# WeeFav/Visual-Odometry-GPU

Measured on AMD Instinct MI355X. Metric: ORB detect+describe frames/sec (1241x376, 8 lvls), higher is better.
Workload: dtype u8; 1 GPU; KITTI-shaped 1241x376 u8, 8 levels s=1.2, 1000 features, FAST-9 t=20, NMS 3x3, Harris top-N, blur5 all levels, BRIEF-256; batch=1024 frames/step/GPU resident in HBM (stream A); distinct_resident_batches=2, fast_early_exit=True, pyramid_blur_fused=True, pyramid_top_rows_first=True, pipelined_batches=True

## Files before the change

visual-odometry-gpu_amd/csrc/orbx_adapt.h:

```cpp
#pragma once
#include <cstdio>
#include <cstdlib>

#include "orbx_plan.h"

struct OrbxAdapt {
  int top_mode = 2;
  bool top_on = true;
  int top_single_batches = 0;
  uint32_t feedback_seen[2] = {0, 0};
  uint32_t need_cur[ORBX_MAX_LEVELS] = {}, need_prev[ORBX_MAX_LEVELS] = {};
  int tile_h_pref[ORBX_MAX_LEVELS] = {};
  int need_batches = 0, need_window = 2, retiles = 0, learn_w = 0, learn_h = 0;
  bool prefs_applied = false;
  uint32_t fill_cur[ORBX_MAX_LEVELS][ORBX_FILL_BUCKETS] = {}, fill_prev[ORBX_MAX_LEVELS][ORBX_FILL_BUCKETS] = {};
  int cut_pref[ORBX_MAX_LEVELS] = {}, cut_force[ORBX_MAX_LEVELS] = {};
  bool first_split = true, split_trace = false;
  uint32_t fill_last[ORBX_MAX_LEVELS][ORBX_FILL_BUCKETS] = {};
  int early_rows[ORBX_MAX_LEVELS] = {};
  bool early_band = true;
};

struct OrbxAdaptGeom {
  const OrbxPlan& plan;
  const OrbxBandMap& bm;
  int nms_radius, fast_impl, top_rows;
};

namespace orbx_adapt {

using namespace orbx_geom;

inline int fast_unit_rows_max(int fast_impl, int nms_radius) {
  return fast_impl == 4 ? ORBX_FAST_UNIT_ROWS_MAX : orbx_fast3_tile_h(nms_radius);
}

inline void first_split_fields(OrbxAdapt& a, const char* e) {
  e = e ? std::strchr(e, ':') : nullptr;
  while (e && *e == ':') {
    e++;
    if (!std::strncmp(e, "equal", 5)) {
      a.first_split = false;
    } else if (!std::strncmp(e, "trace", 5)) {
      a.split_trace = true;
    } else if (!std::strncmp(e, "late", 4)) {
      a.early_band = false;
    } else {
      for (int l = 0; l < ORBX_MAX_LEVELS; l++) {
        char* end = nullptr;
        const long v = std::strtol(e, &end, 10);
        if (end == e) break;
        a.cut_force[l] = (int)std::min<long>(std::max<long>(v, 0), 0xffff);
        e = end;
        if (*e != ',') break;
        e++;
      }
    }
    e = std::strchr(e, ':');
  }
}

inline void new_frame_size(OrbxAdapt& a, int w, int h, uint32_t* feedback) {
  a.learn_w = w;
  a.learn_h = h;
  for (int l = 0; l < ORBX_MAX_LEVELS; l++) a.need_cur[l] = a.need_prev[l] = 0, a.tile_h_pref[l] = a.cut_pref[l] = 0;
  std::memset(a.fill_cur, 0, sizeof(a.fill_cur));
  std::memset(a.fill_prev, 0, sizeof(a.fill_prev));
  std::memset(a.fill_last, 0, sizeof(a.fill_last));
  for (int i = 2; i < ORBX_FEEDBACK_WORDS; i++) feedback[i] = 0;
  a.need_batches = 0;
  a.need_window = 2;
  a.retiles = 0;
}

inline bool top_rows_wanted(const OrbxAdapt& a, int top_rows) {
  if (top_rows <= 0 || a.top_mode == 0) return false;
  return a.top_mode == 1 || a.top_on;
}
inline void top_rows_update(OrbxAdapt& a, uint64_t both) {
  if (a.top_mode != 2) return;
  const uint32_t sk = (uint32_t)both, pr = (uint32_t)(both >> 32);
  const uint32_t dsk = sk - a.feedback_seen[0], dpr = pr - a.feedback_seen[1];
  if (dsk + dpr > 0) {
    a.feedback_seen[0] = sk;
    a.feedback_seen[1] = pr;
    const bool pays = 4ull * dsk >= (unsigned long long)(dsk + dpr);
    if (!pays && a.top_on) a.top_single_batches = 0;
    a.top_on = pays;
  }
  if (!a.top_on && ++a.top_single_batches >= 128) {
    a.top_on = true;
    a.top_single_batches = 0;
  }
}

inline bool adapt_tile_rows(OrbxAdapt& a, const OrbxAdaptGeom& g, const uint32_t* words, bool prefs_apply,
                            long long batch_serial, FILE* trace) {
  if (!prefs_apply) return false;
  const int top = g.top_rows, nl = g.plan.nlevels;
  bool any = false;
  for (int l = 0; l < nl; l++) {
    const uint32_t v = words[2 + l];
    if (v) {
      a.need_cur[l] = std::max(a.need_cur[l], std::min<uint32_t>(v, (uint32_t)g.plan.L[l].h));
      any = true;
      for (int b = 0; b < ORBX_FILL_BUCKETS; b++) {
        const uint32_t cnt = words[ORBX_FEEDBACK_HIST + l * ORBX_FILL_BUCKETS + b];
        a.fill_cur[l][b] += std::min<uint32_t>(cnt, 1u << 20);
      }
    }
  }
  if (!any || ++a.need_batches < a.need_window) return false;
  a.need_batches = 0;
  a.need_window = std::min(2 * a.need_window, 32);
  bool change = false, grow = false;
  int want[ORBX_MAX_LEVELS] = {};
  for (int l = 0; l < nl; l++) {
    const uint32_t need = std::max(a.need_cur[l], a.need_prev[l]);
    a.need_prev[l] = a.need_cur[l];
    a.need_cur[l] = 0;
    if (need == 0) {
      want[l] = a.tile_h_pref[l];
      continue;
    }
    const int rows = (int)need + std::max(4, (int)need / 10);
    const int dflt = orbx_fast3_tile_h(g.nms_radius), lh = g.plan.L[l].h;
    const int bal = (lh + (lh + dflt - 1) / dflt - 1) / ((lh + dflt - 1) / dflt);
    int hh = (rows + top - 1) / top;
    if (g.fast_impl == 4) {
      const int over = (hh + 2 * g.nms_radius) % 7;
      if ((over == 1 || over == 2) && top * (hh - over) >= (int)need + 3) hh -= over;
    }
    if (hh >= bal || lh <= top * hh) hh = 0;
    const int eff = hh ? hh : bal, cur = g.bm.tile_h[l], asked = a.tile_h_pref[l] ? a.tile_h_pref[l] : bal;
    want[l] = ((eff > cur && (int)need > top * cur) || eff + 2 < std::min(cur, asked)) ? hh : a.tile_h_pref[l];
    if (eff > cur && (int)need > top * cur) grow = true;
    else if (eff + 2 < std::min(cur, asked)) change = true;
  }
  const bool heights_change = grow || change;
  const bool split = a.first_split && top == 2 && g.fast_impl == 4;
  const int R = g.nms_radius;
  int cut_want[ORBX_MAX_LEVELS] = {};
  bool cut_change = false;
  for (int l = 0; l < nl; l++) {
    uint32_t hist[ORBX_FILL_BUCKETS];
    uint64_t total = 0;
    for (int b = 0; b < ORBX_FILL_BUCKETS; b++) {
      hist[b] = a.fill_cur[l][b] + a.fill_prev[l][b];
      a.fill_last[l][b] = hist[b];
      a.fill_prev[l][b] = a.fill_cur[l][b];
      a.fill_cur[l][b] = 0;
      total += hist[b];
    }
    if (!split || a.cut_force[l] > 0 || g.bm.tiles_y[l] < 2) continue;
    const int dflt = orbx_fast3_tile_h(R), lh = g.plan.L[l].h;
    const int bal = (lh + (lh + dflt - 1) / dflt - 1) / ((lh + dflt - 1) / dflt);
    const int th_after = heights_change ? (want[l] ? want[l] : bal) : g.bm.tile_h[l];
    const int depth = 2 * th_after;
    const int in_force = !heights_change && g.bm.first_h[l][0] > 0 ? g.bm.first_h[l][0] : 0;
    int cost_new = 0;
    const int cut_new = total && lh > depth ? choose_first_cut(hist, depth, R, ORBX_FAST_UNIT_ROWS_MAX, &cost_new) : 0;
    const int cost_now = first_pass_cost_milli(hist, depth, in_force ? in_force : depth / 2, R);
    if (!total || lh <= depth) cost_new = cost_now;
    const bool pays = cost_now - cost_new >= 1000, stopped = in_force && !cut_new && cost_now > cost_new;
    cut_want[l] = heights_change || pays || stopped ? cut_new : a.cut_pref[l];
    if (cut_want[l] != in_force && (pays || stopped)) cut_change = true;
    if (trace) {
      fprintf(trace, "orbx split: batch %lld level %d need %u depth %d cut %d -> %d (%d -> %d milli-groups) fill rows:",
              batch_serial, l, a.need_prev[l], depth, in_force, cut_want[l], cost_now, cost_new);
      for (int b = 0; b < ORBX_FILL_BUCKETS; b++)
        if (hist[b]) fprintf(trace, " %d:%u", ORBX_FILL_BUCKET_ROWS * (b + 1), hist[b]);
      fprintf(trace, "\n");
    }
  }
  if (!grow && !change && !cut_change) return false;
  if (!grow && a.retiles >= 4 && a.need_window < 32) return false;
  for (int l = 0; l < nl; l++) a.tile_h_pref[l] = want[l], a.cut_pref[l] = cut_want[l];
  a.retiles++;
  if (trace) fprintf(trace, "orbx split: batch %lld re-tile %d\n", batch_serial, a.retiles);
  return true;
}

inline void forget_tile_rows(OrbxAdapt& a) {
  for (int l = 0; l < ORBX_MAX_LEVELS; l++) a.tile_h_pref[l] = 0;
  a.prefs_applied = false;
}

inline bool first_pass_heights(const OrbxAdapt& a, const OrbxAdaptGeom& g, int (*first)[2]) {
  bool any = false;
  if (a.prefs_applied && a.first_split && g.top_rows == 2) {
    for (int l = 0; l < g.plan.nlevels; l++) {
      int h0 = a.cut_force[l] > 0 ? a.cut_force[l] : a.cut_pref[l];
      if (h0 <= 0 || g.bm.tiles_y[l] < 2) continue;
      const int depth = 2 * g.bm.tile_h[l], umax = fast_unit_rows_max(g.fast_impl, g.nms_radius);
      if (a.cut_force[l] > 0)
        h0 = std::max(std::max(1, depth - umax), std::min(h0, std::min(umax, std::min(depth, g.plan.L[l].h) - 1)));
      first[l][0] = h0;
      first[l][1] = depth - h0;
      any = true;
    }
  }
  return any;
}

inline void choose_early_bands(OrbxAdapt& a, const OrbxAdaptGeom& g, FILE* trace) {
  const int top = g.top_rows;
  for (int l = 0; l < ORBX_MAX_LEVELS; l++) a.early_rows[l] = 0;
  for (int l = 0; l < g.plan.nlevels; l++) {
    const int late = pyrblur_first_pass_rows(g.plan, g.bm, l, top);
    const int P = a.early_band ? pyrblur_early_rows(g.plan, g.bm, l, top, g.nms_radius) : late;
    const bool forced = a.cut_force[l] > 0;
    const bool pays = P < late && (forced ? late - P >= ORBX_PYRBLUR_EARLY_MIN_ROWS
                                          : early_band_pays(a.fill_last[l], g.bm.first_h[l][0], late - P,
                                                            pyrblur_row_cost(l, g.plan.L[l].win8)));
    a.early_rows[l] = pays ? P : late;
    if (trace && g.bm.first_h[l][0] > 0)
      fprintf(trace, "orbx early band: level %d cut %d first pass ended at %d, now ends at %d, band %d rows: %s\n", l,
              g.bm.first_h[l][0], late, a.early_rows[l], late - P,
              pays ? (forced ? "split (forced cut)" : "split") : !a.early_band ? "late" : "kept");
  }
}

}
```

visual-odometry-gpu_amd/csrc/orbx_api.cpp:

```cpp
#include <algorithm>
#include <array>
#include <cmath>
#include <cstdlib>
#include <cstring>
#include <new>

#include "orbx_host.h"

using namespace orbx_host;
using namespace orbx_tables;

namespace {
thread_local std::string g_create_error;
}

namespace orbx_host {

int fail(orbx_ctx* c, int status, const std::string& msg) {
  if (c)
    c->err = msg;
  else
    g_create_error = msg;
  return status;
}

int ensure(orbx_ctx* c, DevBuf& b, size_t bytes) {
  if (b.bytes >= bytes && b.p) return ORBX_OK;
  if (b.p) {
    HIPCHK(c, hipStreamSynchronize(c->stream));
    for (const Lane& L : c->lanes)
      if (L.stream && L.stream != c->stream) HIPCHK(c, hipStreamSynchronize(L.stream));
    if (c->last_stream && c->last_stream != c->stream) HIPCHK(c, hipStreamSynchronize(c->last_stream));
    HIPCHK(c, hipFree(b.p));
    b.p = nullptr;
    b.bytes = 0;
  }
  bytes = align_up_sz(std::max<size_t>(bytes, 256), 256);
  HIPCHK(c, hipMalloc(&b.p, bytes));
  b.bytes = bytes;
  return ORBX_OK;
}

hipStream_t batch_stream(const orbx_ctx* c) { return c->last_stream ? c->last_stream : c->stream; }
const Lane& cur_lane(const orbx_ctx* c) { return c->lanes[c->lane]; }
const Block& last_block(const orbx_ctx* c) { return c->blocks[c->blk]; }
hipError_t lanes_sync(orbx_ctx* c) {
  for (const Lane& L : c->lanes)
    if (L.stream) {
      const hipError_t e = hipStreamSynchronize(L.stream);
      if (e != hipSuccess) return e;
    }
  return hipSuccess;
}

int check_image(orbx_ctx* c, const void* img, int w, int h, int stride) {
  if (!c) return ORBX_ERR_INVALID_ARG;
  if (!img) return fail(c, ORBX_ERR_INVALID_ARG, "image is NULL");
  if (w < 8 || h < 8 || w > c->p.max_width || h > c->p.max_height)
    return fail(c, ORBX_ERR_INVALID_ARG, "image size outside [8, max_width] x [8, max_height]");
  if (stride < w) return fail(c, ORBX_ERR_INVALID_ARG, "stride < width");
  return ORBX_OK;
}

bool finite_all(const double* v, int n) {
  for (int i = 0; i < n; i++)
    if (!std::isfinite(v[i])) return false;
  return true;
}

int gaussian_kernel(int K, float sigma, float* kernel) {
  if (K <= 0 || (K % 2) == 0 || !kernel) return ORBX_ERR_INVALID_ARG;
  if (sigma <= 0.0f) sigma = 0.3f * ((K - 1) * 0.5f) + 0.8f;
  const int half = K / 2;
  float sum = 0.0f;
  for (int y = -half; y <= half; ++y)
    for (int x = -half; x <= half; ++x) {
      const float value = std::exp(-(float)(x * x + y * y) / (2 * sigma * sigma));
      kernel[(y + half) * K + (x + half)] = value;
      sum += value;
    }
  for (int i = 0; i < K * K; ++i) kernel[i] /= sum;
  return ORBX_OK;
}

hipError_t launch_blur_auto(int impl, hipStream_t s, const OrbxPlan& P, const OrbxTileMap& tm1, const OrbxTileDesc* tiles2,
                            int ntiles2, int n, const uint8_t* src, uint8_t* dst, int first_level, int kind) {
  if (kind == ORBX_BLUR_SEP16 && impl == 3)
    return orbx_launch_blur4(s, tiles2, ntiles2, P.frame_bytes, n, src, dst, first_level);
  if (kind == ORBX_BLUR_SEP16 && impl != 1)
    return orbx_launch_blur3(s, tiles2, ntiles2, P.frame_bytes, n, src, dst, first_level);
  return orbx_launch_blur(s, P, tm1, n, src, dst, first_level, kind);
}

int SideWork::wait(orbx_ctx* c) {
  if (ev) HIPCHK(c, hipEventSynchronize(ev));
  return ORBX_OK;
}

int SideWork::enter(orbx_ctx* c, hipStream_t s) {
  if (!ev) HIPCHK(c, hipEventCreateWithFlags(&ev, hipEventDisableTiming));
  if (stream != s) {
    const int st = wait(c);
    if (st != ORBX_OK) return st;
  }
  stream = s;
  return ORBX_OK;
}

int SideWork::after(orbx_ctx* c, const SideWork& producer, hipStream_t s) {
  if (producer.ev && producer.stream != s) HIPCHK(c, hipStreamWaitEvent(s, producer.ev, 0));
  return ORBX_OK;
}

int SideWork::grow(orbx_ctx* c, DevBuf& b, size_t bytes) {
  if (b.p && b.bytes >= bytes) return ORBX_OK;
  const int st = wait(c);
  if (st != ORBX_OK) return st;
  bytes = align_up_sz(std::max<size_t>(bytes, 256), 256);
  void* p = nullptr;
  HIPCHK(c, hipMalloc(&p, bytes));
  if (b.p) (void)hipFree(b.p);
  b.p = p;
  b.bytes = bytes;
  return ORBX_OK;
}

int PinnedUpload::send(orbx_ctx* c, void* d_dst, const void* src, size_t n, hipStream_t s) {
  if (!ev) HIPCHK(c, hipEventCreateWithFlags(&ev, hipEventDisableTiming));
  HIPCHK(c, hipEventSynchronize(ev));
  if (bytes < n) {
    if (host) (void)hipHostFree(host);
    host = nullptr;
    bytes = 0;
    HIPCHK(c, hipHostMalloc(&host, align_up_sz(n, 4096), hipHostMallocDefault));
    bytes = align_up_sz(n, 4096);
  }
  std::memcpy(host, src, n);
  HIPCHK(c, hipMemcpyAsync(d_dst, host, n, hipMemcpyHostToDevice, s));
  HIPCHK(c, hipEventRecord(ev, s));
  return ORBX_OK;
}

int set_workspace_limit(orbx_ctx* c, SideWork& side, std::initializer_list<DevBuf*> ws, size_t* limit, size_t bytes,
                        size_t dflt) {
  const int st = side.wait(c);
  if (st != ORBX_OK) return st;
  for (DevBuf* b : ws)
    if (b->p) {
      HIPCHK(c, hipFree(b->p));
      *b = DevBuf{};
    }
  *limit = bytes ? bytes : dflt;
  return ORBX_OK;
}

int stage_tracks(orbx_ctx* c, SideWork& side, DevBuf& stage, const float* tracks_xy, const int32_t* seen, int n_slots,
                 int window_len, const float** d_tracks, const int32_t** d_seen) {
  int st = side.enter(c, c->stream);
  if (st != ORBX_OK) return st;
  const SideWork::Mark mark{side, c->stream};
  const size_t tb = sizeof(float) * 2 * (size_t)n_slots * window_len, sb = sizeof(int32_t) * (size_t)n_slots;
  const size_t o_seen = align_up_sz(tb, 256);
  if ((st = side.grow(c, stage, o_seen + sb)) != ORBX_OK) return st;
  uint8_t* d = (uint8_t*)stage.p;
  HIPCHK(c, hipMemcpyAsync(d, tracks_xy, tb, hipMemcpyHostToDevice, c->stream));
  HIPCHK(c, hipMemcpyAsync(d + o_seen, seen, sb, hipMemcpyHostToDevice, c->stream));
  *d_tracks = (const float*)d;
  *d_seen = (const int32_t*)(d + o_seen);
  return ORBX_OK;
}

int check_device_frames(orbx_ctx* c, const void* d_frames, int n, int n_min, int n_max, int w, int h, int row_stride,
                        size_t frame_stride, const FramesWhat& what) {
  if (!d_frames) return fail(c, ORBX_ERR_INVALID_ARG, what.null_msg);
  if (n < n_min || n > n_max) return fail(c, ORBX_ERR_INVALID_ARG, what.range_msg);
  if (w < 8 || h < 8 || w > c->p.max_width || h > c->p.max_height)
    return fail(c, ORBX_ERR_INVALID_ARG, "image size outside [8, max_width] x [8, max_height]");
  if (row_stride < w) return fail(c, ORBX_ERR_INVALID_ARG, "row_stride < width");
  if (frame_stride < (size_t)row_stride * (size_t)(h - 1) + (size_t)w)
    return fail(c, ORBX_ERR_INVALID_ARG, "frame_stride smaller than a frame");
  if ((unsigned long long)row_stride * (unsigned long long)(h - 1) + (unsigned long long)w > 0x7fffffffull)
    return fail(c, ORBX_ERR_INVALID_ARG, "row_stride * (height - 1) + width exceeds 2^31 - 1");
  return ORBX_OK;
}

}

namespace {

int env_int(const char* name, int dflt) {
  const char* e = getenv(name);
  return e ? atoi(e) : dflt;
}

int pyr_group_env() {
  static const int v = env_int("ORBX_PYR_GROUP", 32);
  return v;
}

int top_rows_env() {
  static const int v = std::max(env_int("ORBX_TOP_ROWS", 2), 0);
  return v;
}

int fast_impl_env() { return env_int("ORBX_FAST_IMPL", 4) == 3 ? 3 : 4; }

int blur_impl_env() {
  const int v = env_int("ORBX_BLUR_IMPL", 2);
  return v >= 1 && v <= 3 ? v : 2;
}

int fast_early_env() {
  static const int v = env_int("ORBX_FAST_EARLY", 1);
  return v;
}

int fuse_env() {
  static const int v = env_int("ORBX_FUSE", 1);
  return v;
}

int graph_env() {
  static const int v = env_int("ORBX_GRAPH", 1);
  return v;
}

int select_spread_env() {
  static const int v = env_int("ORBX_SELECT_SPREAD", -1);
  return v;
}

bool fused_pyrblur(const orbx_ctx* c) {
  return fuse_env() && c->fuse && c->p.blur_levels == ORBX_BLUR_ALL && c->p.blur_kind == ORBX_BLUR_SEP16;
}
bool fast_early_on(const orbx_ctx* c) { return fast_early_env() && c->fast_early; }
bool blur_enabled(const orbx_ctx* c) { return c->p.blur_levels != ORBX_BLUR_NONE; }
const uint8_t* final_pyr(const orbx_ctx* c) { return blur_enabled(c) ? cur_lane(c).d_pyr_blur : cur_lane(c).d_pyr; }

int slots_per_frame(const OrbxPlan& P) { return P.out_cap > 0 ? P.out_cap : 1; }

int validate_params(const orbx_params& p, std::string* why) {
  auto bad = [&](const char* m) {
    *why = m;
    return (int)ORBX_ERR_INVALID_ARG;
  };
  if (p.nfeatures < 0) return bad("nfeatures < 0");
  if (!(p.scale_factor > 1.0f) || !(p.scale_factor <= 4.0f)) return bad("scale_factor must be in (1, 4]");
  if (p.nlevels < 1 || p.nlevels > ORBX_MAX_LEVELS) return bad("nlevels must be in [1, 16]");
  if (p.n < 1 || p.n > 16) return bad("n must be in [1, 16]");
  if (p.threshold < 0 || p.threshold > 255) return bad("threshold must be in [0, 255]");
  if (p.nms_window < 0 || p.nms_window / 2 > 3) return bad("nms_window must be in [0, 7]");
  if (p.patch_size < 1 || p.patch_size / 2 > 20) return bad("patch_size must be in [1, 41]");
  if (p.harris_window < 1 || (p.harris_window % 2) == 0 || p.harris_window > 15)
    return bad("harris_window must be odd, in [1, 15]");
  if (p.select_mode != ORBX_SELECT_HARRIS && p.select_mode != ORBX_SELECT_ROWMAJOR) return bad("select_mode");
  if (p.blur_levels < 0 || p.blur_levels > 2) return bad("blur_levels");
  if (p.blur_kind < 0 || p.blur_kind > 1) return bad("blur_kind");
  if (p.max_width < 8 || p.max_height < 8 || p.max_width > 16384 || p.max_height > 16384)
    return bad("max_width/max_height must be in [8, 16384]");
  if (p.max_batch < 1 || p.max_batch > 65535) return bad("max_batch must be in [1, 65535]");
  return ORBX_OK;
}

struct PoolRef {
  void** p;
  size_t bytes;
  bool zero;
};
std::array<PoolRef, 11> lane_pools(const orbx_ctx* c, Lane& L) {
  const OrbxPlan& M = c->plan_max;
  const size_t B = (size_t)c->p.max_batch, nc = B * (size_t)std::max(M.cand_total, 1);
  const size_t frames = B * (size_t)M.frame_bytes, levels = B * ORBX_MAX_LEVELS * sizeof(int32_t);
  return {{
      {(void**)&L.d_pyr, frames, false},
      {(void**)&L.d_pyr_blur, c->p.blur_levels != ORBX_BLUR_NONE ? frames : 0, true},
      {(void**)&L.d_mask, B * (size_t)M.mask_words * 8, true},
      {(void**)&L.d_row_stat, B * ORBX_FAST_STAT_WORDS * 8, false},
      {(void**)&L.d_cand, nc * sizeof(orbx_keypoint), false},
      {(void**)&L.d_cand_count, levels, false},
      {(void**)&L.d_cand_total, levels, false},
      {(void**)&L.d_resp, nc * sizeof(float), false},
      {(void**)&L.d_lcand, nc * sizeof(uint32_t), false},
      {(void**)&L.d_lresp, nc * sizeof(float), false},
      {(void**)&L.d_lcount, levels, false},
  }};
}
hipError_t alloc_lane_pools(orbx_ctx* c, Lane& L) {
  for (const PoolRef& r : lane_pools(c, L)) {
    if (r.bytes == 0) continue;
    hipError_t e = hipMalloc(r.p, r.bytes + 256);
    if (e == hipSuccess && r.zero) e = hipMemset(*r.p, 0, r.bytes);
    if (e != hipSuccess) return e;
  }
  return hipSuccess;
}
void free_lane(orbx_ctx* c, Lane& L) {
  for (const PoolRef& r : lane_pools(c, L)) {
    if (*r.p) (void)hipFree(*r.p);
    *r.p = nullptr;
  }
  if (L.stream != c->stream) {
    if (L.stream) (void)hipStreamDestroy(L.stream);
    L.stream = nullptr;
  }
  L.pool_stream = nullptr;
}

bool tile_prefs_apply(const orbx_ctx* c) {
  return c->adapt.top_mode == 2 && top_rows_env() > 0 && fast_early_on(c) && fused_pyrblur(c);
}
OrbxAdaptGeom adapt_geom(const orbx_ctx* c) {
  return OrbxAdaptGeom{c->plan, c->bm_fast, c->p.nms_window / 2, c->fast_impl, top_rows_env()};
}
FILE* adapt_trace(const orbx_ctx* c) { return c->adapt.split_trace ? stderr : nullptr; }

int set_plan(orbx_ctx* c, int w, int h) {
  if (w == c->plan_w && h == c->plan_h) return ORBX_OK;
  if (w < 8 || h < 8 || w > c->p.max_width || h > c->p.max_height)
    return fail(c, ORBX_ERR_INVALID_ARG, "frame size outside [8, max_width] x [8, max_height]");
  OrbxPlan plan;
  std::string why;
  int st = plan_with_taps(c->p, w, h, c->fast_impl, &plan, &c->h_taps, &why);
  if (st != ORBX_OK) return fail(c, st, why);
  if (c->h_taps.size() > c->table_cap.taps) return fail(c, ORBX_ERR_UNSUPPORTED, "resize table exceeds pool");
  c->plan_w = c->plan_h = 0;
  OrbxPlanTables& T = c->scratch;
  const OrbxTableSwitches sw{c->fast_impl, c->blur_impl, top_rows_env(), pyr_group_env() > 0, tile_prefs_apply(c)};
  st = build_tile_tables(plan, c->p.nms_window / 2, sw, c->table_cap, c->adapt, adapt_trace(c), &T, &why);
  if (st != ORBX_OK) return fail(c, st, why);
  HIPCHK(c, hipStreamSynchronize(batch_stream(c)));
  HIPCHK(c, lanes_sync(c));
  HIPCHK(c, hipMemcpy(c->d_taps, c->h_taps.data(), c->h_taps.size() * sizeof(OrbxResizeTap),
                      hipMemcpyHostToDevice));
  for (const Lane& L : c->lanes)
    if (L.d_pyr_blur)
      HIPCHK(c, hipMemsetAsync(L.d_pyr_blur, 0, (size_t)c->p.max_batch * (size_t)c->plan_max.frame_bytes, c->stream));
  HIPCHK(c, hipStreamSynchronize(c->stream));
  for (int i = 0; i < kTileTables; i++) {
    const std::vector<OrbxTileDesc>& t = T.tiles[i];
    if (!t.empty())
      HIPCHK(c, hipMemcpy(c->tiles[i].d, t.data(), t.size() * sizeof(OrbxTileDesc), hipMemcpyHostToDevice));
    c->tiles[i].count = (int)t.size();
  }
  c->plan = plan;
  c->tm_blur = T.tm_blur;
  c->bm_fast = T.bm_fast;
  c->top_levels = T.top_levels;
  c->plan_serial++;
  c->plan_w = w;
  c->plan_h = h;
  return ORBX_OK;
}

hipError_t launch_pyramid_auto(orbx_ctx* c, hipStream_t s, int n, const uint8_t* d_in, int in_stride,
                               size_t in_frame_stride) {
  return orbx_launch_pyramid2(s, c->tiles[T_PYR2].d, c->tiles[T_PYR2].count, c->plan.frame_bytes, c->plan.w0, c->plan.h0, n,
                              d_in, in_stride, in_frame_stride, c->d_taps, cur_lane(c).d_pyr);
}

hipError_t launch_fast_tiles(orbx_ctx* c, hipStream_t s, int first, int count, int n, OrbxFastParams fp,
                             unsigned long long* stat, int chunk_scale = 1) {
  const OrbxTileDesc* tiles = c->tiles[T_FAST].d + first;
  unsigned long long* mask = cur_lane(c).d_mask;
  if (c->fast_impl == 4)
    return orbx_launch_fast4(s, tiles, count, n, final_pyr(c), c->plan.frame_bytes, c->plan.mask_words, fp, mask, stat);
  return orbx_launch_fast_nms(s, tiles, count, n, final_pyr(c), c->plan.frame_bytes, c->plan.mask_words, fp, mask, nullptr,
                              stat, chunk_scale);
}

hipError_t launch_fast_whole(orbx_ctx* c, hipStream_t s, int n, OrbxFastParams fp, bool stats_zeroed = false) {
  unsigned long long* stat = fast_early_on(c) ? cur_lane(c).d_row_stat : nullptr;
  if (stat && !stats_zeroed) {
    hipError_t e = hipMemsetAsync(stat, 0, (size_t)n * ORBX_FAST_STAT_WORDS * 8, s);
    if (e != hipSuccess) return e;
  }
  return launch_fast_tiles(c, s, 0, c->tiles[T_FAST].count, n, fp, stat);
}

int enqueue_batch(orbx_ctx* c, Block& B, const uint8_t* d_frames, int n, int row_stride, size_t frame_stride, hipStream_t s) {
  const OrbxPlan& P = c->plan;
  const Lane& L = cur_lane(c);
  const TileTable &whole = c->tiles[T_PYRBLUR], &shortb = c->tiles[T_PYRBLUR_SMALL], &top = c->tiles[T_PYRBLUR_TOP],
                  &rest = c->tiles[T_PYRBLUR_REST];
  const int tm = c->timing;
  TimingSet& ts = c->evr[c->ev_calls % ORBX_EVENT_SETS];
  auto mark = [&](int slot, bool roofline_edge) -> hipError_t {
    if (tm == 1 || (tm == 2 && roofline_edge)) return hipEventRecord(ts.ev[slot], s);
    return hipSuccess;
  };
  const bool fused = fused_pyrblur(c);
  const bool small = (long long)n * whole.count < 4096;
  const bool two_pass = fused && !small && fast_early_on(c) && top_rows_wanted(c->adapt, top_rows_env()) && rest.count > 0 &&
                        c->bm_fast.nbands > top_rows_env();
  if (!two_pass) HIPCHK(c, hipMemsetAsync(L.d_row_stat, 0, (size_t)n * ORBX_FAST_STAT_WORDS * 8, s));
  HIPCHK(c, mark(0, false));
  OrbxFastParams fp{c->p.threshold, c->p.n, c->p.nms_window / 2};
  if (fused) {
    HIPCHK(c, mark(1, true));
    if (!two_pass) {
      const TileTable& T = small ? shortb : whole;
      HIPCHK(c, orbx_launch_pyrblur(s, T.d, T.count, P.frame_bytes, P.w0, P.h0, n, d_frames, row_stride, frame_stride,
                                    c->d_taps, L.d_pyr_blur, small ? 0 : pyr_group_env()));
    } else {
      const int first_tiles = c->bm_fast.band_begin[top_rows_env()];
      HIPCHK(c, orbx_launch_pyrblur(s, top.d, top.count, P.frame_bytes, P.w0, P.h0, n, d_frames, row_stride, frame_stride,
                                    c->d_taps, L.d_pyr_blur, pyr_group_env(), nullptr, c->d_feedback, nullptr,
                                    L.d_row_stat));
      HIPCHK(c, mark(ORBX_NUM_STAGE_TIMES + 1, true));
      HIPCHK(c, launch_fast_tiles(c, s, 0, first_tiles, n, fp, L.d_row_stat));
      HIPCHK(c, mark(ORBX_NUM_STAGE_TIMES + 2, true));
      HIPCHK(c, orbx_launch_pyrblur(s, rest.d, rest.count, P.frame_bytes, P.w0, P.h0, n, d_frames, row_stride,
                                    frame_stride, c->d_taps, L.d_pyr_blur, pyr_group_env(), L.d_row_stat, c->d_feedback,
                                    &c->top_levels));
      HIPCHK(c, mark(2, true));
      HIPCHK(c, launch_fast_tiles(c, s, first_tiles, c->tiles[T_FAST].count - first_tiles, n, fp, L.d_row_stat, 4));
    }
  } else {
    HIPCHK(c, launch_pyramid_auto(c, s, n, d_frames, row_stride, frame_stride));
    HIPCHK(c, mark(1, true));
    if (blur_enabled(c))
      HIPCHK(c, launch_blur_auto(c->blur_impl, s, P, c->tm_blur, c->tiles[T_BLUR].d, c->tiles[T_BLUR].count, n, L.d_pyr,
                                 L.d_pyr_blur, c->p.blur_levels == ORBX_BLUR_UPPER ? 1 : 0, c->p.blur_kind));
  }
  if (!two_pass) {
    HIPCHK(c, mark(2, true));
    HIPCHK(c, launch_fast_whole(c, s, n, fp, true));
  }
  ts.split = two_pass;
  c->last_two_pass = two_pass;
  HIPCHK(c, mark(3, true));
  HIPCHK(c, mark(4, false));
  HIPCHK(c, mark(5, false));
  const OutLayout& o = B.layout;
  HIPCHK(c, orbx_launch_level_select_auto(s, P, n, c->p.select_mode, select_spread_env(), L.d_mask, final_pyr(c), c->d_gauss,
                                          c->p.harris_window, c->p.harris_k, L.d_lcand, L.d_lcount, L.d_lresp,
                                          L.d_cand, L.d_resp, L.d_cand_count, two_pass ? c->d_feedback + 2 : nullptr));
  HIPCHK(c, mark(6, false));
  if (P.out_cap <= 0)
    HIPCHK(c, hipMemsetAsync(B.d + o.counts, 0, sizeof(int32_t) * (size_t)n, s));
  OrbxHostRecord hr{};
  if (c->host_results && P.out_cap > 0 && B.h_dev)
    hr = OrbxHostRecord{(int32_t*)(B.h_dev + o.counts), (uint32_t*)(B.h_dev + o.kp16), (float*)(B.h_dev + o.angle),
                        (orbx_descriptor*)(B.h_dev + o.desc)};
  HIPCHK(c, orbx_launch_describe(s, P, n, final_pyr(c), c->p.patch_size, L.d_cand_count, L.d_cand, L.d_resp,
                                 (int32_t*)(B.d + o.counts), (orbx_keypoint*)(B.d + o.lkp),
                                 (float*)(B.d + o.resp), (int32_t*)(B.d + o.level),
                                 (orbx_keypoint*)(B.d + o.kp), (uint32_t*)(B.d + o.kp16),
                                 (float*)(B.d + o.angle),
                                 (orbx_descriptor*)(B.d + o.desc), two_pass ? c->d_feedback : nullptr,
                                 two_pass ? const_cast<uint32_t*>(c->h_feedback) : nullptr, &hr));
  HIPCHK(c, mark(7, false));
  return ORBX_OK;
}

void drop_graph(orbx_ctx* c, int i) {
  if (c->g_exec[i]) (void)hipGraphExecDestroy(c->g_exec[i]);
  c->g_exec[i] = nullptr;
}

int run_batch(orbx_ctx* c, const uint8_t* d_frames, int n, int w, int h, int row_stride, size_t frame_stride,
              hipStream_t s, bool may_pipeline = false) {
  OrbxAdapt& a = c->adapt;
  if (w != a.learn_w || h != a.learn_h) {
    new_frame_size(a, w, h, const_cast<uint32_t*>(c->h_feedback));
  } else if (w == c->plan_w && h == c->plan_h) {
    bool any_pref = false;
    for (int l = 0; l < ORBX_MAX_LEVELS; l++) any_pref |= a.tile_h_pref[l] != 0 || a.cut_pref[l] != 0 || a.cut_force[l] != 0;
    const bool apply = tile_prefs_apply(c);
    const int used = ORBX_FEEDBACK_HIST + c->plan.nlevels * ORBX_FILL_BUCKETS;
    uint32_t words[ORBX_FEEDBACK_WORDS];
    for (int i = 0; apply && i < used; i++) words[i] = c->h_feedback[i];
    if (adapt_tile_rows(a, adapt_geom(c), words, apply, c->batch_serial, adapt_trace(c)) || (any_pref && apply != a.prefs_applied))
      c->plan_w = 0;
  }
  const bool lanes = may_pipeline && c->pipelined && s == c->stream && w == c->plan_w && h == c->plan_h;
  c->lane = lanes ? c->next_lane : 0;
  Lane& L = c->lanes[c->lane];
  if (lanes) {
    s = L.stream;
  } else {
    if (c->lanes[1].stream) HIPCHK(c, lanes_sync(c));
    if (c->last_stream && c->last_stream != s) HIPCHK(c, hipStreamSynchronize(c->last_stream));
  }
  int st = set_plan(c, w, h);
  if (st != ORBX_OK) return st;
  top_rows_update(a, *reinterpret_cast<const volatile uint64_t*>(c->h_feedback));
  const int blk = (c->blk + 1) % orbx_ctx::kBlocks;
  Block& B = c->blocks[blk];
  if (B.copy_pending) HIPCHK(c, hipStreamWaitEvent(s, B.ev_copied, 0));
  if (L.pool_stream && L.pool_stream != s) HIPCHK(c, hipStreamWaitEvent(s, L.ev_pool, 0));
  if (B.stream && B.stream != s) HIPCHK(c, hipStreamWaitEvent(s, B.ev_done, 0));
  B.n = 0;
  B.copy_pending = false;
  B.copy_compact = false;
  B.cap = slots_per_frame(c->plan);
  B.layout = OutLayout(n, B.cap);
  const int tm = c->timing;
  if (graph_env() && tm == 0) {
    const OrbxGraphKey key{d_frames, frame_stride, n, w, h, row_stride, (fast_early_on(c) ? 1 : 0) | (fused_pyrblur(c) ? 2 : 0) | (top_rows_wanted(a, top_rows_env()) ? 4 : 0) | (lanes ? 8 : 0) | (c->lane << 4) | (c->host_results ? 64 : 0),
                           c->plan_serial, blk};
    int gi = -1;
    for (int i = 0; i < orbx_ctx::kGraphs; i++)
      if (c->g_exec[i] && key == c->g_key[i]) gi = i;
    if (gi < 0) {
      gi = c->g_next;
      c->g_next = (c->g_next + 1) % orbx_ctx::kGraphs;
      drop_graph(c, gi);
      hipGraph_t g = nullptr;
      const hipError_t be = hipStreamBeginCapture(s, hipStreamCaptureModeThreadLocal);
      if (be != hipSuccess) return fail(c, ORBX_ERR_HIP, std::string("hipStreamBeginCapture: ") + hipGetErrorString(be));
      st = enqueue_batch(c, B, d_frames, n, row_stride, frame_stride, s);
      const hipError_t ee = hipStreamEndCapture(s, &g);
      if (st != ORBX_OK) {
        if (g) (void)hipGraphDestroy(g);
        return st;
      }
      if (ee != hipSuccess) return fail(c, ORBX_ERR_HIP, std::string("hipStreamEndCapture: ") + hipGetErrorString(ee));
      const hipError_t ie = hipGraphInstantiate(&c->g_exec[gi], g, nullptr, nullptr, 0);
      (void)hipGraphDestroy(g);
      if (ie != hipSuccess) {
        c->g_exec[gi] = nullptr;
        return fail(c, ORBX_ERR_HIP, std::string("hipGraphInstantiate: ") + hipGetErrorString(ie));
      }
      c->g_key[gi] = key;
    }
    const hipError_t le = hipGraphLaunch(c->g_exec[gi], s);
    if (le != hipSuccess) return fail(c, ORBX_ERR_HIP, std::string("hipGraphLaunch: ") + hipGetErrorString(le));
  } else {
    if ((st = enqueue_batch(c, B, d_frames, n, row_stride, frame_stride, s)) != ORBX_OK) return st;
  }
  c->blk = blk;
  if (lanes) c->next_lane ^= 1;
  c->batch_serial++;
  c->last_stream = s;
  B.n = n;
  B.host_written = c->host_results && c->plan.out_cap > 0;
  HIPCHK(c, hipEventRecord(B.ev_done, s));
  if (B.host_written) {
    HIPCHK(c, hipEventRecord(B.ev_copied, s));
    B.copy_pending = true;
    B.copy_compact = true;
  }
  HIPCHK(c, hipEventRecord(L.ev_pool, s));
  L.pool_stream = s;
  B.stream = s;
  if (tm != 0) {
    c->evr[c->ev_calls % ORBX_EVENT_SETS].mode = tm;
    c->ev_calls++;
  }
  return ORBX_OK;
}


}

extern "C" {

int orbx_params_default_gpu(orbx_params* p) {
  if (!p) return ORBX_ERR_INVALID_ARG;
  std::memset(p, 0, sizeof(*p));
  p->nfeatures = 500;
  p->scale_factor = 1.2f;
  p->nlevels = 8;
  p->threshold = 20;
  p->n = 9;
  p->nms_window = 3;
  p->patch_size = 31;
  p->harris_window = 7;
  p->harris_k = 0.04f;
  p->select_mode = ORBX_SELECT_HARRIS;
  p->blur_levels = ORBX_BLUR_NONE;
  p->blur_kind = ORBX_BLUR_SEP16;
  p->max_width = 1920;
  p->max_height = 1080;
  p->max_batch = 1;
  p->device = -1;
  return ORBX_OK;
}

int orbx_params_default_cpu(orbx_params* p) {
  int st = orbx_params_default_gpu(p);
  if (st != ORBX_OK) return st;
  p->nfeatures = 3000;
  p->threshold = 50;
  p->n = 9;
  p->nms_window = 3;
  p->patch_size = 9;
  p->nlevels = 1;
  p->select_mode = ORBX_SELECT_ROWMAJOR;
  return ORBX_OK;
}

const char* orbx_status_string(int status) {
  switch (status) {
    case ORBX_OK:
      return "ok";
    case ORBX_ERR_INVALID_ARG:
      return "invalid argument";
    case ORBX_ERR_CAPACITY:
      return "output capacity exceeded";
    case ORBX_ERR_HIP:
      return "HIP runtime error";
    case ORBX_ERR_NO_DEVICE:
      return "no usable gfx950 device";
    case ORBX_ERR_UNSUPPORTED:
      return "unsupported parameter combination";
    default:
      return "unknown status";
  }
}

const char* orbx_version(void) { return "liborbx 0.1.0 gfx950"; }

const char* orbx_last_error_string(const orbx_ctx* ctx) { return ctx ? ctx->err.c_str() : g_create_error.c_str(); }

void orbx_destroy(orbx_ctx* c) {
  DeviceGuard _dg(c);
  if (!c) return;
  if (c->stream) (void)hipStreamSynchronize(c->stream);
  if (c->lanes[1].stream) (void)hipStreamSynchronize(c->lanes[1].stream);
  for (int i = 0; i < orbx_ctx::kGraphs; i++) drop_graph(c, i);
  for (Lane& L : c->lanes) {
    free_lane(c, L);
    if (L.ev_pool) (void)hipEventDestroy(L.ev_pool);
  }
  for (TileTable& T : c->tiles)
    if (T.d) (void)hipFree(T.d);
  void* bufs[] = {c->d_in, c->d_taps, c->d_gauss, c->d_feedback};
  for (void* b : bufs)
    if (b) (void)hipFree(b);
  if (c->h_feedback) (void)hipHostFree(const_cast<uint32_t*>(c->h_feedback));
  for (Block& B : c->blocks) {
    if (B.h) (void)hipHostFree(B.h);
    if (B.d) (void)hipFree(B.d);
    if (B.ev_done) (void)hipEventDestroy(B.ev_done);
    if (B.ev_copied) (void)hipEventDestroy(B.ev_copied);
  }
  if (c->cstream) {
    (void)hipStreamSynchronize(c->cstream);
    (void)hipStreamDestroy(c->cstream);
  }
  c->carry.release();
  c->reloc.release();
  c->pnp.release();
  c->st.release();
  c->wp.release();
  c->tp.release();
  c->lm.release();
  c->lkw.release();
  c->gf.release();
  c->s.release();
  c->m.release();
  c->lk.release();
  c->pose.release();
  c->scale.release();
  c->ba.release();
  for (auto& e : c->ev)
    if (e) (void)hipEventDestroy(e);
  for (TimingSet& set : c->evr)
    for (auto& e : set.ev)
      if (e) (void)hipEventDestroy(e);
  if (c->stream) (void)hipStreamDestroy(c->stream);
  delete c;
}

int orbx_create(const orbx_params* p, orbx_ctx** out) {
  if (!p || !out) return fail(nullptr, ORBX_ERR_INVALID_ARG, "params/out is NULL");
  *out = nullptr;
  std::string why;
  int st = validate_params(*p, &why);
  if (st != ORBX_OK) return fail(nullptr, st, why);

  int ndev = 0;
  if (hipGetDeviceCount(&ndev) != hipSuccess || ndev <= 0)
    return fail(nullptr, ORBX_ERR_NO_DEVICE, "hipGetDeviceCount found no device (liborbx has no CPU fallback)");
  int dev = p->device;
  if (dev < 0) {
    if (hipGetDevice(&dev) != hipSuccess) dev = 0;
  }
  if (dev >= ndev) return fail(nullptr, ORBX_ERR_INVALID_ARG, "device ordinal out of range");
  DeviceGuard dg(dev);
  {
    int cur = -1;
    if (hipGetDevice(&cur) != hipSuccess || cur != dev) return fail(nullptr, ORBX_ERR_NO_DEVICE, "hipSetDevice failed");
  }
  hipDeviceProp_t prop;
  if (hipGetDeviceProperties(&prop, dev) != hipSuccess)
    return fail(nullptr, ORBX_ERR_NO_DEVICE, "hipGetDeviceProperties failed");
  if (std::strncmp(prop.gcnArchName, "gfx950", 6) != 0)
    return fail(nullptr, ORBX_ERR_NO_DEVICE,
                std::string("device is ") + prop.gcnArchName + ", liborbx is built for gfx950 only");

  orbx_ctx* c = new (std::nothrow) orbx_ctx();
  if (!c) return fail(nullptr, ORBX_ERR_HIP, "out of host memory");
  c->p = *p;
  c->device = dev;

  c->fast_impl = fast_impl_env();
  c->blur_impl = blur_impl_env();
  first_split_fields(c->adapt, getenv("ORBX_TOP_ROWS"));
  st = build_plan(c->p, p->max_width, p->max_height, &c->plan_max, &why, c->fast_impl);
  if (st != ORBX_OK) {
    delete c;
    return fail(nullptr, st, why);
  }
  const OrbxPlan& M = c->plan_max;
  const size_t B = (size_t)p->max_batch;

#define CREATE_CHK(expr)                                                                     \
  do {                                                                                       \
    hipError_t _e = (expr);                                                                  \
    if (_e != hipSuccess) {                                                                  \
      std::string m = std::string(#expr) + ": " + hipGetErrorString(_e);                     \
      orbx_destroy(c);                                                                       \
      return fail(nullptr, ORBX_ERR_HIP, m);                                                 \
    }                                                                                        \
  } while (0)

  CREATE_CHK(hipStreamCreateWithFlags(&c->stream, hipStreamNonBlocking));
  c->lanes[0].stream = c->stream;
  for (auto& e : c->ev) CREATE_CHK(hipEventCreate(&e));
  for (TimingSet& set : c->evr)
    for (auto& e : set.ev) CREATE_CHK(hipEventCreate(&e));
  CREATE_CHK(hipMalloc((void**)&c->d_in, B * (size_t)p->max_width * p->max_height + 256));
  CREATE_CHK(alloc_lane_pools(c, c->lanes[0]));
  CREATE_CHK(hipMalloc((void**)&c->d_feedback, ORBX_FEEDBACK_WORDS * 4));
  CREATE_CHK(hipMemset(c->d_feedback, 0, ORBX_FEEDBACK_WORDS * 4));
  CREATE_CHK(hipHostMalloc((void**)&c->h_feedback, ORBX_FEEDBACK_WORDS * 4, hipHostMallocDefault));
  for (int i = 0; i < ORBX_FEEDBACK_WORDS; i++) c->h_feedback[i] = 0;
  OrbxTableCapacity tcap{};
  if ((st = table_capacity(*p, M, c->fast_impl, c->blur_impl, &tcap, &why)) != ORBX_OK) {
    orbx_destroy(c);
    return fail(nullptr, st, why);
  }
  c->table_cap = tcap;
  for (int i = 0; i < kTileTables; i++)
    CREATE_CHK(hipMalloc((void**)&c->tiles[i].d, std::max<size_t>(tile_table_capacity(tcap, i), 1) * sizeof(OrbxTileDesc)));
  CREATE_CHK(hipMalloc((void**)&c->d_taps, tcap.taps * sizeof(OrbxResizeTap)));
  {
    const int K = p->harris_window;
    std::vector<float> g((size_t)K * K);
    gaussian_kernel(K, -1.0f, g.data());
    CREATE_CHK(hipMalloc((void**)&c->d_gauss, g.size() * sizeof(float)));
    CREATE_CHK(hipMemcpy(c->d_gauss, g.data(), g.size() * sizeof(float), hipMemcpyHostToDevice));
  }
  {
    const OutLayout o((int)B, slots_per_frame(M));
    {
      int least = 0, greatest = 0;
      CREATE_CHK(hipDeviceGetStreamPriorityRange(&least, &greatest));
      CREATE_CHK(hipStreamCreateWithPriority(&c->cstream, hipStreamNonBlocking, greatest));
    }
    for (Block& blk : c->blocks) {
      CREATE_CHK(hipMalloc((void**)&blk.d, o.total));
      CREATE_CHK(hipHostMalloc((void**)&blk.h, o.total, hipHostMallocDefault));
      CREATE_CHK(hipHostGetDevicePointer((void**)&blk.h_dev, blk.h, 0));
      CREATE_CHK(hipEventCreateWithFlags(&blk.ev_done, hipEventDisableTiming));
      CREATE_CHK(hipEventCreateWithFlags(&blk.ev_copied, hipEventDisableTiming));
    }
    for (Lane& L : c->lanes) CREATE_CHK(hipEventCreateWithFlags(&L.ev_pool, hipEventDisableTiming));
  }
#undef CREATE_CHK
  *out = c;
  return ORBX_OK;
}

int orbx_get_plan(orbx_ctx* c, int width, int height, int32_t* level_w, int32_t* level_h, int32_t* quota,
                  int32_t* fast_cap, float* level_scale_out, int32_t* out_capacity) {
  DeviceGuard _dg(c);
  if (!c) return ORBX_ERR_INVALID_ARG;
  OrbxPlan plan;
  std::string why;
  int st = build_plan(c->p, width, height, &plan, &why, c->fast_impl);
  if (st != ORBX_OK) return fail(c, st, why);
  for (int l = 0; l < plan.nlevels; l++) {
    if (level_w) level_w[l] = plan.L[l].w;
    if (level_h) level_h[l] = plan.L[l].h;
    if (quota) quota[l] = plan.L[l].quota;
    if (fast_cap) fast_cap[l] = plan.L[l].cap;
    if (level_scale_out) level_scale_out[l] = plan.L[l].scale;
  }
  if (out_capacity) *out_capacity = plan.out_cap;
  return ORBX_OK;
}

int orbx_detect_and_compute_batch_device(orbx_ctx* c, const void* d_frames, int n, int width, int height,
                                         int row_stride, size_t frame_stride, void* stream) {
  DeviceGuard _dg(c);
  if (!c) return ORBX_ERR_INVALID_ARG;
  if (!d_frames) return fail(c, ORBX_ERR_INVALID_ARG, "d_frames is NULL");
  if (n < 1 || n > c->p.max_batch) return fail(c, ORBX_ERR_INVALID_ARG, "n outside [1, max_batch]");
  if (row_stride < width) return fail(c, ORBX_ERR_INVALID_ARG, "row_stride < width");
  if (frame_stride < (size_t)row_stride * (size_t)(height - 1) + (size_t)width)
    return fail(c, ORBX_ERR_INVALID_ARG, "frame_stride smaller than a frame");
  if ((unsigned long long)row_stride * (unsigned long long)(height - 1) + (unsigned long long)width > 0x7fffffffull)
    return fail(c, ORBX_ERR_INVALID_ARG, "row_stride * (height - 1) + width exceeds 2^31 - 1");
  return run_batch(c, (const uint8_t*)d_frames, n, width, height, row_stride, frame_stride, stream_of(c, stream), true);
}

int orbx_detect_and_compute_batch_host(orbx_ctx* c, const uint8_t* frames, int n, int width, int height,
                                       int row_stride, size_t frame_stride) {
  DeviceGuard _dg(c);
  if (!c) return ORBX_ERR_INVALID_ARG;
  if (n < 1 || n > c->p.max_batch) return fail(c, ORBX_ERR_INVALID_ARG, "n outside [1, max_batch]");
  int st = check_image(c, frames, width, height, row_stride);
  if (st != ORBX_OK) return st;
  if (n > 1 && frame_stride < (size_t)row_stride * (size_t)(height - 1) + (size_t)width)
    return fail(c, ORBX_ERR_INVALID_ARG, "frame_stride smaller than a frame");
  const size_t tight = (size_t)width * height;
  if (row_stride == width && (n == 1 || frame_stride == tight)) {
    HIPCHK(c, hipMemcpyAsync(c->d_in, frames, tight * n, hipMemcpyHostToDevice, c->stream));
  } else {
    for (int i = 0; i < n; i++)
      HIPCHK(c, hipMemcpy2DAsync(c->d_in + tight * i, width, frames + frame_stride * i, row_stride, width, height,
                                 hipMemcpyHostToDevice, c->stream));
  }
  return run_batch(c, c->d_in, n, width, height, width, tight, c->stream);
}

int orbx_wait(orbx_ctx* c) {
  DeviceGuard _dg(c);
  if (!c) return ORBX_ERR_INVALID_ARG;
  HIPCHK(c, hipStreamSynchronize(batch_stream(c)));
  HIPCHK(c, lanes_sync(c));
  return ORBX_OK;
}

int orbx_set_host_results(orbx_ctx* c, int enable) {
  DeviceGuard _dg(c);
  if (!c) return ORBX_ERR_INVALID_ARG;
  c->host_results = enable ? 1 : 0;
  return ORBX_OK;
}

int orbx_set_pipelined_batches(orbx_ctx* c, int enable) {
  DeviceGuard _dg(c);
  if (!c) return ORBX_ERR_INVALID_ARG;
  if (c->last_stream) HIPCHK(c, hipStreamSynchronize(c->last_stream));
  HIPCHK(c, lanes_sync(c));
  Lane& L = c->lanes[1];
  if (enable && !L.stream) {
    hipError_t e = alloc_lane_pools(c, L);
    if (e == hipSuccess) e = hipStreamCreateWithFlags(&L.stream, hipStreamNonBlocking);
    if (e != hipSuccess) {
      free_lane(c, L);
      c->pipelined = false;
      return fail(c, ORBX_ERR_HIP, std::string("second lane of the pipelined mode: ") + hipGetErrorString(e));
    }
  }
  c->pipelined = enable != 0;
  return ORBX_OK;
}

int orbx_debug_fill_pools(orbx_ctx* c, int byte) {
  DeviceGuard _dg(c);
  if (!c) return ORBX_ERR_INVALID_ARG;
  if (byte < 0 || byte > 255) return fail(c, ORBX_ERR_INVALID_ARG, "byte must be in [0, 255]");
  if (c->last_stream) HIPCHK(c, hipStreamSynchronize(c->last_stream));
  HIPCHK(c, hipStreamSynchronize(c->stream));
  HIPCHK(c, lanes_sync(c));
  for (Lane& L : c->lanes) {
    if (!L.d_mask) continue;
    for (const PoolRef& r : lane_pools(c, L))
      if (*r.p && *r.p != L.d_pyr_blur) HIPCHK(c, hipMemsetAsync(*r.p, byte, r.bytes, c->stream));
    if (L.d_pyr_blur && c->plan_w > 0)
      for (size_t f = 0; f < (size_t)c->p.max_batch; f++)
        for (int l = 0; l < c->plan.nlevels; l++) {
          const OrbxLevel& V = c->plan.L[l];
          HIPCHK(c, hipMemset2DAsync(L.d_pyr_blur + f * (size_t)c->plan.frame_bytes + (size_t)V.img_off, (size_t)V.pitch, byte,
                                     (size_t)V.w, (size_t)V.h, c->stream));
        }
  }
  HIPCHK(c, hipStreamSynchronize(c->stream));
  return ORBX_OK;
}

int orbx_debug_read_pyramid_level(orbx_ctx* c, int frame, int level, uint8_t* out, size_t out_bytes) {
  DeviceGuard _dg(c);
  if (!c || !out) return ORBX_ERR_INVALID_ARG;
  if (c->plan_w == 0 || !cur_lane(c).d_pyr_blur) return fail(c, ORBX_ERR_INVALID_ARG, "run a batch first");
  if (frame < 0 || frame >= c->p.max_batch || level < 0 || level >= c->plan.nlevels)
    return fail(c, ORBX_ERR_INVALID_ARG, "frame or level out of range");
  const OrbxLevel& V = c->plan.L[level];
  if (out_bytes < (size_t)V.w * (size_t)V.h) return fail(c, ORBX_ERR_INVALID_ARG, "out_bytes below level_w * level_h");
  if (c->last_stream) HIPCHK(c, hipStreamSynchronize(c->last_stream));
  HIPCHK(c, hipStreamSynchronize(c->stream));
  HIPCHK(c, lanes_sync(c));
  HIPCHK(c, hipMemcpy2D(out, (size_t)V.w, cur_lane(c).d_pyr_blur + (size_t)frame * (size_t)c->plan.frame_bytes + (size_t)V.img_off,
                        (size_t)V.pitch, (size_t)V.w, (size_t)V.h, hipMemcpyDeviceToHost));
  return ORBX_OK;
}

int orbx_set_fast_early_exit(orbx_ctx* c, int enable) {
  DeviceGuard _dg(c);
  if (!c) return ORBX_ERR_INVALID_ARG;
  c->fast_early = enable != 0;
  return ORBX_OK;
}

int orbx_set_fused_pyramid_blur(orbx_ctx* c, int enable) {
  DeviceGuard _dg(c);
  if (!c) return ORBX_ERR_INVALID_ARG;
  c->fuse = enable != 0;
  return ORBX_OK;
}

int orbx_set_top_rows_first(orbx_ctx* c, int mode) {
  DeviceGuard _dg(c);
  if (!c || mode < 0 || mode > 2) return ORBX_ERR_INVALID_ARG;
  c->adapt.top_mode = mode;
  c->adapt.top_on = true;
  c->adapt.top_single_batches = 0;
  return ORBX_OK;
}

int orbx_fast_tile_counts(orbx_ctx* c, long long* worked, long long* total) {
  DeviceGuard _dg(c);
  if (!c || !worked || !total) return ORBX_ERR_INVALID_ARG;
  if (c->plan_w == 0 || last_block(c).n < 1) return fail(c, ORBX_ERR_INVALID_ARG, "run a batch first");
  const int n = last_block(c).n;
  std::vector<unsigned long long> h((size_t)n * ORBX_FAST_STAT_WORDS);
  HIPCHK(c, hipStreamSynchronize(c->last_stream));
  HIPCHK(c, hipMemcpy(h.data(), cur_lane(c).d_row_stat, h.size() * 8, hipMemcpyDeviceToHost));
  long long w = 0;
  for (int f = 0; f < n; f++)
    for (int l = 0; l < c->plan.nlevels; l++)
      for (int b = 0; b < c->bm_fast.tiles_y[l]; b++)
        w += (long long)(h[(size_t)f * ORBX_FAST_STAT_WORDS + (size_t)l * ORBX_MAX_BANDS + b] >> 32);
  *total = (long long)c->bm_fast.band_begin[c->bm_fast.nbands] * n;
  *worked = fast_early_on(c) ? w : *total;
  return ORBX_OK;
}

int orbx_pyramid_pixel_counts(orbx_ctx* c, long long* produced, long long* total) {
  DeviceGuard _dg(c);
  if (!c || !produced || !total) return ORBX_ERR_INVALID_ARG;
  if (c->plan_w == 0 || last_block(c).n < 1) return fail(c, ORBX_ERR_INVALID_ARG, "run a batch first");
  const int n = last_block(c).n, top = top_rows_env();
  long long per_frame = 0;
  for (int l = 0; l < c->plan.nlevels; l++) per_frame += (long long)c->plan.L[l].w * c->plan.L[l].h;
  *total = per_frame * n;
  *produced = *total;
  if (!c->last_two_pass) return ORBX_OK;
  std::vector<unsigned long long> h((size_t)n * ORBX_FAST_STAT_WORDS);
  HIPCHK(c, hipStreamSynchronize(c->last_stream));
  HIPCHK(c, hipMemcpy(h.data(), cur_lane(c).d_row_stat, h.size() * 8, hipMemcpyDeviceToHost));
  long long done = 0;
  for (int f = 0; f < n; f++)
    for (int l = 0; l < c->plan.nlevels; l++) {
      const OrbxLevel& L = c->plan.L[l];
      const int first = pyrblur_first_pass_rows(c->plan, c->bm_fast, l, top);
      long long surv = 0, surv0 = 0;
      for (int b = 0; b < std::min(top, c->bm_fast.tiles_y[l]); b++) {
        surv += (long long)(uint32_t)h[(size_t)f * ORBX_FAST_STAT_WORDS + (size_t)l * ORBX_MAX_BANDS + b];
        if (b == 0) surv0 = surv;
      }
      const int early_l = c->adapt.early_rows[l], early = early_l > 0 && early_l < first ? early_l : first;
      const int band = surv0 >= L.cap ? 0 : first - early;
      done += (long long)L.w * (first < L.h && surv >= L.cap ? early + band : L.h);
    }
  *produced = done;
  return ORBX_OK;
}

int orbx_enable_stage_timing(orbx_ctx* c, int enable) {
  DeviceGuard _dg(c);
  if (!c) return ORBX_ERR_INVALID_ARG;
  c->timing = enable < 0 || enable > 2 ? 1 : enable;
  return ORBX_OK;
}

int orbx_stage_times_history(orbx_ctx* c, int back, float* ms) {
  DeviceGuard _dg(c);
  if (!c || !ms) return ORBX_ERR_INVALID_ARG;
  if (back < 0 || back >= ORBX_EVENT_SETS || back >= c->ev_calls)
    return fail(c, ORBX_ERR_INVALID_ARG, "no timed batched call that far back");
  const long long call = c->ev_calls - 1 - back;
  const TimingSet& ts = c->evr[call % ORBX_EVENT_SETS];
  const hipEvent_t* evs = ts.ev;
  const int mode = ts.mode;
  std::memset(ms, 0, sizeof(float) * ORBX_NUM_STAGE_TIMES);
  if (mode == 1) {
    for (int i = 0; i < ORBX_NUM_STAGE_TIMES - 1; i++) HIPCHK(c, hipEventElapsedTime(&ms[i], evs[i], evs[i + 1]));
    HIPCHK(c, hipEventElapsedTime(&ms[ORBX_NUM_STAGE_TIMES - 1], evs[0], evs[ORBX_NUM_STAGE_TIMES - 1]));
  } else {
    HIPCHK(c, hipEventElapsedTime(&ms[1], evs[1], evs[2]));
    HIPCHK(c, hipEventElapsedTime(&ms[2], evs[2], evs[3]));
  }
  if (ts.split) {
    float a = 0, b = 0, d = 0, e = 0;
    HIPCHK(c, hipEventElapsedTime(&a, evs[1], evs[ORBX_NUM_STAGE_TIMES + 1]));
    HIPCHK(c, hipEventElapsedTime(&b, evs[ORBX_NUM_STAGE_TIMES + 1], evs[ORBX_NUM_STAGE_TIMES + 2]));
    HIPCHK(c, hipEventElapsedTime(&d, evs[ORBX_NUM_STAGE_TIMES + 2], evs[2]));
    HIPCHK(c, hipEventElapsedTime(&e, evs[2], evs[3]));
    ms[1] = a + d;
    ms[2] = b + e;
  }
  return ORBX_OK;
}

int orbx_last_stage_times(orbx_ctx* c, float* ms) { return orbx_stage_times_history(c, 0, ms); }

int orbx_batch_results_device(orbx_ctx* c, orbx_batch_view* v) {
  DeviceGuard _dg(c);
  if (!c || !v) return ORBX_ERR_INVALID_ARG;
  const Block& B = last_block(c);
  if (B.n <= 0) return fail(c, ORBX_ERR_INVALID_ARG, "no batch has been run");
  const OutLayout& o = B.layout;
  v->counts = (const int32_t*)(B.d + o.counts);
  v->keypoints = (const orbx_keypoint*)(B.d + o.kp);
  v->keypoints16 = (const uint32_t*)(B.d + o.kp16);
  v->level_kps = (const orbx_keypoint*)(B.d + o.lkp);
  v->orientations = (const float*)(B.d + o.angle);
  v->responses = (const float*)(B.d + o.resp);
  v->levels = (const int32_t*)(B.d + o.level);
  v->descriptors = (const orbx_descriptor*)(B.d + o.desc);
  v->slot_capacity = B.cap;
  v->n = B.n;
  return ORBX_OK;
}

namespace {
int fetch_block(orbx_ctx* c, int b, int first, int n, int32_t* counts, orbx_keypoint* keypoints, float* orientations,
                orbx_descriptor* descriptors, float* responses, int32_t* levels, orbx_keypoint* level_kps,
                int capacity) {
  Block& B = c->blocks[b];
  if (!counts) return fail(c, ORBX_ERR_INVALID_ARG, "counts is NULL");
  if (first < 0 || n < 1 || first + n > B.n) return fail(c, ORBX_ERR_INVALID_ARG, "frame range outside batch");
  if (capacity < 0) return fail(c, ORBX_ERR_INVALID_ARG, "capacity < 0");
  const OutLayout& o = B.layout;
  const int cap = B.cap;
  const uint8_t* h = B.h;
  if (B.copy_pending && B.copy_compact && (responses || levels || level_kps)) {
    HIPCHK(c, hipEventSynchronize(B.ev_copied));
    HIPCHK(c, hipMemcpyAsync(B.h + o.compact, B.d + o.compact, o.total - o.compact, hipMemcpyDeviceToHost,
                             c->cstream));
    HIPCHK(c, hipStreamSynchronize(c->cstream));
    B.copy_compact = false;
  } else if (B.copy_pending) {
    HIPCHK(c, hipEventSynchronize(B.ev_copied));
  } else if (b == c->blk) {
    hipStream_t s = batch_stream(c);
    HIPCHK(c, hipMemcpyAsync(B.h, B.d, o.total, hipMemcpyDeviceToHost, s));
    HIPCHK(c, hipStreamSynchronize(s));
  } else {
    HIPCHK(c, hipStreamWaitEvent(c->cstream, B.ev_done, 0));
    HIPCHK(c, hipMemcpyAsync(B.h, B.d, o.total, hipMemcpyDeviceToHost, c->cstream));
    HIPCHK(c, hipStreamSynchronize(c->cstream));
  }
  const int32_t* hc = (const int32_t*)(h + o.counts);
  bool truncated = false;
  for (int i = 0; i < n; i++) {
    const int f = first + i;
    const int cnt = hc[f];
    counts[i] = cnt;
    const int m = std::min(cnt, capacity);
    if (cnt > capacity) truncated = true;
    const size_t so = (size_t)f * cap, dst = (size_t)i * capacity;
    if (keypoints) {
      const uint32_t* k16 = (const uint32_t*)(h + o.kp16) + so;
      for (int j = 0; j < m; j++) keypoints[dst + j] = orbx_keypoint{(int32_t)(k16[j] & 0xffffu), (int32_t)(k16[j] >> 16)};
    }
    if (level_kps) std::memcpy(level_kps + dst, (const orbx_keypoint*)(h + o.lkp) + so, sizeof(orbx_keypoint) * m);
    if (orientations) std::memcpy(orientations + dst, (const float*)(h + o.angle) + so, sizeof(float) * m);
    if (responses) std::memcpy(responses + dst, (const float*)(h + o.resp) + so, sizeof(float) * m);
    if (levels) std::memcpy(levels + dst, (const int32_t*)(h + o.level) + so, sizeof(int32_t) * m);
    if (descriptors)
      std::memcpy(descriptors + dst, (const orbx_descriptor*)(h + o.desc) + so, sizeof(orbx_descriptor) * m);
  }
  if (truncated) return fail(c, ORBX_ERR_CAPACITY, "capacity smaller than keypoint count");
  return ORBX_OK;
}
}

int orbx_batch_fetch(orbx_ctx* c, int first, int n, int32_t* counts, orbx_keypoint* keypoints,
                     float* orientations, orbx_descriptor* descriptors, float* responses, int32_t* levels,
                     orbx_keypoint* level_kps, int capacity) {
  DeviceGuard _dg(c);
  if (!c) return ORBX_ERR_INVALID_ARG;
  return fetch_block(c, c->blk, first, n, counts, keypoints, orientations, descriptors, responses, levels, level_kps,
                     capacity);
}

int orbx_batch_results_host(orbx_ctx* c, int previous, orbx_batch_view* v) {
  DeviceGuard _dg(c);
  if (!c || !v) return ORBX_ERR_INVALID_ARG;
  if (previous < 0 || previous >= orbx_ctx::kBlocks) return fail(c, ORBX_ERR_INVALID_ARG, "previous must be 0..3 (a ring of four result blocks)");
  Block& B = c->blocks[(c->blk + orbx_ctx::kBlocks - previous) % orbx_ctx::kBlocks];
  if (B.n <= 0) return fail(c, ORBX_ERR_INVALID_ARG, previous ? "there is no batch that far back" : "no batch has been run");
  const OutLayout& o = B.layout;
  if (B.copy_pending) {
    HIPCHK(c, hipEventSynchronize(B.ev_copied));
  } else {
    HIPCHK(c, hipStreamWaitEvent(c->cstream, B.ev_done, 0));
    HIPCHK(c, hipMemcpyAsync(B.h, B.d, o.total, hipMemcpyDeviceToHost, c->cstream));
    HIPCHK(c, hipEventRecord(B.ev_copied, c->cstream));
    B.copy_pending = true;
    HIPCHK(c, hipEventSynchronize(B.ev_copied));
  }
  const uint8_t* h = B.h;
  const bool compact = B.copy_compact;
  v->counts = (const int32_t*)(h + o.counts);
  v->keypoints = compact ? nullptr : (const orbx_keypoint*)(h + o.kp);
  v->keypoints16 = (const uint32_t*)(h + o.kp16);
  v->level_kps = compact ? nullptr : (const orbx_keypoint*)(h + o.lkp);
  v->orientations = (const float*)(h + o.angle);
  v->responses = compact ? nullptr : (const float*)(h + o.resp);
  v->levels = compact ? nullptr : (const int32_t*)(h + o.level);
  v->descriptors = (const orbx_descriptor*)(h + o.desc);
  v->slot_capacity = B.cap;
  v->n = B.n;
  return ORBX_OK;
}

namespace {
int prefetch_block(orbx_ctx* c, bool compact) {
  Block& B = c->blocks[c->blk];
  if (B.n <= 0) return fail(c, ORBX_ERR_INVALID_ARG, "no batch has been run");
  const OutLayout& o = B.layout;
  if (B.copy_pending) {
    if (compact || !B.copy_compact) return ORBX_OK;
    HIPCHK(c, hipStreamWaitEvent(c->cstream, B.ev_done, 0));
    HIPCHK(c, hipMemcpyAsync(B.h + o.compact, B.d + o.compact, o.total - o.compact, hipMemcpyDeviceToHost,
                             c->cstream));
    HIPCHK(c, hipEventRecord(B.ev_copied, c->cstream));
    B.copy_compact = false;
    return ORBX_OK;
  }
  HIPCHK(c, hipStreamWaitEvent(c->cstream, B.ev_done, 0));
  HIPCHK(c, hipMemcpyAsync(B.h, B.d, compact ? o.compact : o.total, hipMemcpyDeviceToHost, c->cstream));
  HIPCHK(c, hipEventRecord(B.ev_copied, c->cstream));
  B.copy_pending = true;
  B.copy_compact = compact;
  return ORBX_OK;
}
}

int orbx_batch_prefetch(orbx_ctx* c) {
  DeviceGuard _dg(c);
  if (!c) return ORBX_ERR_INVALID_ARG;
  return prefetch_block(c, false);
}

int orbx_batch_prefetch_compact(orbx_ctx* c) {
  DeviceGuard _dg(c);
  if (!c) return ORBX_ERR_INVALID_ARG;
  return prefetch_block(c, true);
}

int orbx_batch_fetch_previous(orbx_ctx* c, int first, int n, int32_t* counts, orbx_keypoint* keypoints,
                              float* orientations, orbx_descriptor* descriptors, float* responses, int32_t* levels,
                              orbx_keypoint* level_kps, int capacity) {
  DeviceGuard _dg(c);
  if (!c) return ORBX_ERR_INVALID_ARG;
  const int b = (c->blk + orbx_ctx::kBlocks - 1) % orbx_ctx::kBlocks;
  if (c->blocks[b].n <= 0) return fail(c, ORBX_ERR_INVALID_ARG, "there is no batch before the last one");
  return fetch_block(c, b, first, n, counts, keypoints, orientations, descriptors, responses, levels, level_kps,
                     capacity);
}

int orbx_detect_and_compute(orbx_ctx* c, const uint8_t* image, int width, int height, int stride,
                            orbx_keypoint* keypoints, float* orientations, orbx_descriptor* descriptors,
                            float* responses, int32_t* levels, orbx_keypoint* level_kps, int capacity,
                            int* count) {
  DeviceGuard _dg(c);
  if (!c) return ORBX_ERR_INVALID_ARG;
  if (!count) return fail(c, ORBX_ERR_INVALID_ARG, "count is NULL");
  int st = orbx_detect_and_compute_batch_host(c, image, 1, width, height, stride, (size_t)stride * height);
  if (st != ORBX_OK) return st;
  int32_t cnt = 0;
  st = orbx_batch_fetch(c, 0, 1, &cnt, keypoints, orientations, descriptors, responses, levels, level_kps,
                        capacity);
  *count = cnt;
  return st;
}

int orbx_bench_stage(orbx_ctx* c, int n_frames, int stage, int reps, float* avg_ms) {
  DeviceGuard _dg(c);
  if (!c || !avg_ms) return ORBX_ERR_INVALID_ARG;
  if (c->plan_w == 0) return fail(c, ORBX_ERR_INVALID_ARG, "run a batch first (no pyramid built)");
  if (n_frames < 1 || n_frames > last_block(c).n || reps < 1) return fail(c, ORBX_ERR_INVALID_ARG, "n_frames/reps");
  const OrbxPlan& P = c->plan;
  const Lane& L = cur_lane(c);
  hipStream_t s = c->stream;
  OrbxFastParams fp{c->p.threshold, c->p.n, c->p.nms_window / 2};
  HIPCHK(c, hipStreamSynchronize(s));
  HIPCHK(c, lanes_sync(c));
  HIPCHK(c, hipEventRecord(c->ev[0], s));
  for (int i = 0; i < reps; i++) {
    switch (stage) {
      case ORBX_STAGE_BLUR:
        if (!blur_enabled(c)) return fail(c, ORBX_ERR_INVALID_ARG, "blur is disabled in this context");
        HIPCHK(c, launch_blur_auto(c->blur_impl, s, P, c->tm_blur, c->tiles[T_BLUR].d, c->tiles[T_BLUR].count, n_frames,
                                   L.d_pyr, L.d_pyr_blur, c->p.blur_levels == ORBX_BLUR_UPPER ? 1 : 0, c->p.blur_kind));
        break;
      case ORBX_STAGE_FAST:
        HIPCHK(c, launch_fast_whole(c, s, n_frames, fp));
        break;
      case ORBX_STAGE_COMPACT:
        HIPCHK(c, orbx_launch_compact(s, P, n_frames, L.d_mask, L.d_cand, L.d_cand_count, L.d_cand_total, 0));
        break;
      default:
        return fail(c, ORBX_ERR_INVALID_ARG, "stage not benchmarkable in isolation");
    }
  }
  HIPCHK(c, hipEventRecord(c->ev[1], s));
  HIPCHK(c, hipEventSynchronize(c->ev[1]));
  float ms = 0;
  HIPCHK(c, hipEventElapsedTime(&ms, c->ev[0], c->ev[1]));
  *avg_ms = ms / reps;
  return ORBX_OK;
}

int orbx_build_pyramid_level(orbx_ctx* c, const uint8_t* image, int width, int height, int stride, int level,
                             uint8_t* dst, int* level_w, int* level_h) {
  DeviceGuard _dg(c);
  int st = check_image(c, image, width, height, stride);
  if (st != ORBX_OK) return st;
  if (level < 0 || level >= c->p.nlevels || !dst) return fail(c, ORBX_ERR_INVALID_ARG, "level out of range / dst NULL");
  if ((st = set_plan(c, width, height)) != ORBX_OK) return st;
  const OrbxPlan& P = c->plan;
  HIPCHK(c, lanes_sync(c));
  HIPCHK(c, hipMemcpy2DAsync(c->d_in, width, image, stride, width, height, hipMemcpyHostToDevice, c->stream));
  HIPCHK(c, launch_pyramid_auto(c, c->stream, 1, c->d_in, width, (size_t)width * height));
  if (blur_enabled(c))
    HIPCHK(c, launch_blur_auto(c->blur_impl, c->stream, P, c->tm_blur, c->tiles[T_BLUR].d, c->tiles[T_BLUR].count, 1,
                               cur_lane(c).d_pyr, cur_lane(c).d_pyr_blur, c->p.blur_levels == ORBX_BLUR_UPPER ? 1 : 0,
                               c->p.blur_kind));
  const OrbxLevel& L = P.L[level];
  HIPCHK(c, hipMemcpy2DAsync(dst, L.w, final_pyr(c) + L.img_off, L.pitch, L.w, L.h, hipMemcpyDeviceToHost,
                             c->stream));
  HIPCHK(c, hipStreamSynchronize(c->stream));
  if (level_w) *level_w = L.w;
  if (level_h) *level_h = L.h;
  return ORBX_OK;
}

}
```

visual-odometry-gpu_amd/csrc/orbx_fast4.hip:

```cpp
#include <hip/hip_runtime.h>

#include <algorithm>

#include "orbx_fast_common.h"
#include "orbx_internal.h"
#include "orbx_wave.h"

namespace {

template <int R>
struct F4 {
  static constexpr int HD = orbx_fast4_halo(R);
  static constexpr int S = 64 - 2 * HD;
  static constexpr int G = 7;
  static constexpr int IMG_SLOTS = 2 * G + 6;
  static constexpr int IMG_PITCH = 256;
  static constexpr int NS = R > 0 ? G + 2 * R : 1;
  static constexpr int SC_PITCH = 256;
  static constexpr int QCAP = 256;
};

__device__ __forceinline__ uint32_t f4_colmask(int x0, int lo, int hi) {
  const int a = min(max(lo - x0, 0), 4), b = min(max(hi - x0, 0), 4);
  if (b <= a) return 0u;
  const uint32_t upto_b = b >= 4 ? 0xffffffffu : ((1u << (8 * b)) - 1u);
  const uint32_t below_a = a >= 4 ? 0xffffffffu : ((1u << (8 * a)) - 1u);
  return (upto_b & ~below_a) & 0x7f7f7f7fu;
}
__device__ __forceinline__ uint32_t f4_rowmask(int y0, int lo, int hi) {
  const int a = min(max(lo - y0, 0), 7), b = min(max(hi - y0, 0), 7);
  if (b <= a) return 0u;
  return (((1u << b) - 1u) & ~((1u << a) - 1u)) * 0x01010101u;
}

template <int R, bool ZT>
__global__ __launch_bounds__(64) void k_fast4(const OrbxTileDesc* __restrict__ tiles, int n_tiles, int n_frames,
                                              const uint8_t* __restrict__ pyr, int frame_bytes, int mask_words,
                                              OrbxFastParams fp, u64* __restrict__ mask, u64* __restrict__ row_stat) {
  typedef F4<R> C;
  typedef F3Ring<C::IMG_PITCH> RG;
  __shared__ __attribute__((aligned(16))) uint32_t s_img32[C::IMG_SLOTS * 64];
  __shared__ __attribute__((aligned(16))) uint16_t s_sc[C::NS * C::SC_PITCH];
  __shared__ __attribute__((aligned(16))) uint16_t s_queue[C::QCAP];
  __shared__ __attribute__((aligned(16))) uint32_t s_cflag[64];
  __shared__ __attribute__((aligned(16))) uint32_t s_mask32[C::G * 8];
  __shared__ __attribute__((aligned(16))) uint32_t s_lut32[128];
  __shared__ int s_qn;
  const uint8_t* s_img = reinterpret_cast<const uint8_t*>(s_img32);
  const uint8_t* s_lut = reinterpret_cast<const uint8_t*>(s_lut32);

  const int lane = threadIdx.x;
  const int lin = blockIdx.x;
  const int tile = lin / n_frames, f = lin - tile * n_frames;
  const OrbxTileDesc d = f3_tile(tiles, tile);
  if (row_stat && d.ty > 0) {
    u64* st = row_stat + (size_t)f * ORBX_FAST_STAT_WORDS;
    u64* dead = st + ORBX_MAX_LEVELS * ORBX_MAX_BANDS + d.l;
    const u64 pv = f3_probe_issue(st + d.stat_index, dead, d.ty, lane);
    if (f3_probe_decide(pv, dead, d.ty, d.u2, d.u0, lane)) return;
  }
  const int w = d.w, h = d.h, pitch = d.pitch, th = (int)(d.pad >> 16);
  const int y0 = (int)(d.pad & 0xffffu), y1 = min(y0 + th, h);
  const int thr = fp.threshold, narc_any = fp.n;
  const bool first = d.tx == 0, last = d.tx + 1 == d.u2;
  const int dw0 = d.tx * C::S;
  const int x_lane = 4 * (dw0 + lane);
  const int P0 = first ? 0 : 4 * (dw0 + C::HD), P1 = last ? 4 * (dw0 + 64) : 4 * (dw0 + 64 - C::HD);
  const uint32_t scol = f4_colmask(x_lane, max(P0 - R, 3), min(P1 + R, w - 3));
  const uint32_t pcol = f4_colmask(x_lane, max(P0, 3), min(P1, w - 3));
  const int sy_lo = max(y0 - R, 3), sy_hi = min(y1 + R, h - 3);

  const __amdgpu_buffer_rsrc_t rsrc = __builtin_amdgcn_make_buffer_rsrc(
      const_cast<uint8_t*>(pyr) + ((size_t)f * (size_t)frame_bytes + d.img_off), 0, pitch * h, 0x00020000);
  const uint32_t voff = x_lane < pitch ? (uint32_t)x_lane : 0xffffffffu;
  const int rbase = y0 - R - 3;
  auto issue = [&](int t, uint32_t& r) {
    const int ry = min(max(rbase + t, 0), h - 1);
    r = __builtin_amdgcn_raw_buffer_load_b32(rsrc, voff, ry * pitch, 0);
  };

  {
    uint32_t wlo = 0, whi = 0;
#pragma unroll
    for (int b = 0; b < 4; b++) {
      const int d0 = 8 * lane + b - 255, d1 = d0 + 4;
      wlo |= (uint32_t)((d0 >= thr ? 1 : 0) | (d0 <= -thr ? 2 : 0)) << (8 * b);
      whi |= (uint32_t)((d1 >= thr ? 1 : 0) | (d1 <= -thr ? 2 : 0)) << (8 * b);
    }
    reinterpret_cast<uint2*>(s_lut32)[lane] = make_uint2(wlo, whi);
    if (lane == 0) s_qn = 0;
  }
  if (R > 0) {
    for (int i = lane; i < C::NS * C::SC_PITCH / 8; i += 64) reinterpret_cast<uint4*>(s_sc)[i] = make_uint4(0u, 0u, 0u, 0u);
    s_cflag[lane] = 0u;
  }
  if (lane < C::G * 8) s_mask32[lane] = 0u;

  uint32_t E[7], O[7], raw[7];
#pragma unroll
  for (int k = 0; k < 7; k++) issue(k, raw[k]);
  int slot = 0;
  const uint32_t lds_lane = (uint32_t)lane * 4u;
  auto store_row = [&](uint32_t c) {
    s_img32[slot * 64 + lane] = c;
    if (slot < 6) s_img32[(14 + slot) * 64 + lane] = c;
    slot = slot == 13 ? 0 : slot + 1;
  };
  (void)lds_lane;
#pragma unroll
  for (int k = 0; k < 6; k++) {
    const uint32_t c = raw[k];
    issue(7 + k, raw[k]);
    store_row(c);
    E[k] = __builtin_amdgcn_perm(c, c, 0x0c020c00u);
    O[k] = __builtin_amdgcn_perm(c, c, 0x0c030c01u);
  }

  const uint32_t T = (uint32_t)thr * 0x00010001u;
  const int ngroups = (y1 - y0 + 2 * R + C::G - 1) / C::G;
  uint32_t prev_c = 0u;
  int sm0 = 0;
  int surv = 0;
  u64* const mask_base = mask + ((size_t)f * (size_t)mask_words + d.mask_off) + (size_t)(4 * d.tx);
  const int wpr = d.u1;

  for (int g = 0; g < ngroups; g++) {
    const int gpar = (g & 1) * 7;
    const int cy0 = y0 - R + 7 * g;
    uint32_t acc = 0u;
#pragma unroll
    for (int k = 0; k < 7; k++) {
      const int jn = (6 + k) % 7, jc = (3 + k) % 7, jo = k;
      const uint32_t c = raw[jn];
      issue(7 * g + 13 + k, raw[jn]);
      store_row(c);
      E[jn] = __builtin_amdgcn_perm(c, c, 0x0c020c00u);
      O[jn] = __builtin_amdgcn_perm(c, c, 0x0c030c01u);
      const uint32_t Ec = E[jc], Oc = O[jc];
      const uint32_t En = __builtin_amdgcn_update_dpp(0u, Ec, 0x130, 0xf, 0xf, true);
      const uint32_t On = __builtin_amdgcn_update_dpp(0u, Oc, 0x130, 0xf, 0xf, true);
      const uint32_t Ep = __builtin_amdgcn_update_dpp(0u, Ec, 0x138, 0xf, 0xf, true);
      const uint32_t Op = __builtin_amdgcn_update_dpp(0u, Oc, 0x138, 0xf, 0xf, true);
      const uint32_t ee = __builtin_amdgcn_alignbit(On, Oc, 16), eo = En;
      const uint32_t we = Op, wo = __builtin_amdgcn_alignbit(Ec, Ep, 16);
      const uint32_t ze = f3_pretest<ZT>(Ec, E[jo], ee, E[jn], we, T);
      const uint32_t zo = f3_pretest<ZT>(Oc, O[jo], eo, O[jn], wo, T);
      const uint32_t F = __builtin_amdgcn_perm(zo, ze, 0x07030501u);
      acc = (F & 0x80808080u) | (acc >> 1);
    }
    uint32_t cand = (~acc >> 1) & scol & f4_rowmask(cy0, sy_lo, sy_hi);
    if (R == 0) cand &= pcol & f4_rowmask(cy0, y0, y1);

    auto for_each = [&](uint32_t bits, auto&& fn) {
      if (__ballot(bits != 0u) == 0ull) return;
      const uint32_t ebase = (uint32_t)lane << 5;
      auto pass = [&](uint32_t b) -> int {
        const int cnt = __popc(b);
        int pos = 0;
        if (cnt) pos = atomicAdd(&s_qn, cnt);
        wave_lds_sync();
        const int total = __builtin_amdgcn_readfirstlane(s_qn);
        wave_lds_sync();
        if (lane == 0) s_qn = 0;
        if (total <= C::QCAP) {
          while (b) {
            const int bp = __ffs(b) - 1;
            b &= b - 1;
            s_queue[pos++] = (uint16_t)(ebase | (uint32_t)bp);
          }
        }
        return total;
      };
      auto drain = [&](int n) {
        wave_lds_sync();
        for (int q0 = 0; q0 < n; q0 += 64) {
          const int q = q0 + lane;
          const bool active = q < n;
          fn(active, active ? (uint32_t)s_queue[q] : 0u);
        }
        wave_lds_sync();
      };
      const int total = pass(bits);
      if (total <= C::QCAP) {
        drain(total);
      } else {
        for (int r = 0; r < C::G; r++) {
          const uint32_t rb = bits & (0x01010101u << r);
          if (__ballot(rb != 0u) == 0ull) continue;
          drain(pass(rb));
        }
      }
    };

    auto eval = [&](bool active, uint32_t e) {
      const int xs = (int)(e >> 3), k = (int)(e & 7u);
      const uint8_t* p0 = s_img + (gpar + k) * C::IMG_PITCH + xs - 3;
      if (!active) p0 = s_img + 3 * C::IMG_PITCH;
      const int Ip = p0[3 * C::IMG_PITCH + 3];
      int v[16];
#pragma unroll
      for (int i = 0; i < 16; i++) v[i] = p0[RG::off(i)];
      const uint8_t* lut = s_lut + (255 - Ip);
      uint32_t M = 0;
#pragma unroll
      for (int i = 0; i < 16; i++) M = (M << 2) | (uint32_t)lut[v[i]];
      auto rot = [](uint32_t x, int sh) { return __builtin_amdgcn_alignbit(x, x, sh); };
      uint32_t a = M;
      if (narc_any == 9) {
        a &= rot(a, 2);
        a &= rot(a, 4);
        a &= rot(a, 8);
        a &= rot(a, 2);
      } else if (narc_any == 12) {
        a &= rot(a, 2);
        a &= rot(a, 4);
        a &= rot(a, 8);
        a &= rot(a, 8);
      } else {
        int kk = 1;
        while (2 * kk <= narc_any) {
          a &= rot(a, 2 * kk);
          kk *= 2;
        }
        if (kk < narc_any) a &= rot(a, 2 * (narc_any - kk));
      }
      const bool corner = a != 0u;
      uint32_t score = 0;
#pragma unroll
      for (int i = 0; i < 16; i++) score = __builtin_amdgcn_sad_u16((uint32_t)Ip, (uint32_t)v[i], score);
      if (active && corner && score > 0u) {
        if (R > 0) {
          int s = sm0 + k;
          s = s >= C::NS ? s - C::NS : s;
          s_sc[s * C::SC_PITCH + xs] = (uint16_t)(score | ((uint32_t)((7 * g + k) & 15) << 12));
          atomicOr(&s_cflag[e >> 5], 1u << (e & 31u));
        } else {
          atomicOr(&s_mask32[k * 8 + (xs >> 5)], 1u << (xs & 31));
        }
      }
    };
    for_each(cand, eval);

    if (R > 0) {
      const uint32_t cur_c = s_cflag[lane];
      s_cflag[lane] = 0u;
      constexpr uint32_t LOWR = ((1u << R) - 1u) * 0x01010101u;
      uint32_t nbits = ((prev_c >> (7 - R)) & LOWR) | ((cur_c << R) & (0x7f7f7f7fu & ~LOWR));
      prev_c = cur_c;
      nbits &= pcol & f4_rowmask(cy0 - R, y0, y1);
      auto nms = [&](bool active, uint32_t e) {
        const int xs = (int)(e >> 3), n = (int)(e & 7u);
        int sr = sm0 - R + n;
        sr = sr < 0 ? sr + C::NS : sr;
        sr = sr >= C::NS ? sr - C::NS : sr;
        const int xq = active ? xs : R;
        const int mrow = 7 * g - R + n;
        const uint32_t s = (uint32_t)s_sc[sr * C::SC_PITCH + xq] & 0xfffu;
        bool keep = true;
#pragma unroll
        for (int dy = -R; dy <= R; dy++) {
          int rr = sr + dy;
          rr = rr < 0 ? rr + C::NS : rr;
          rr = rr >= C::NS ? rr - C::NS : rr;
          const uint16_t* row = s_sc + rr * C::SC_PITCH + xq - R;
          const uint32_t base = ((uint32_t)((mrow + dy) & 15) << 12) + s + 1u, lim = 4095u - s;
#pragma unroll
          for (int dx = 0; dx <= 2 * R; dx++)
            if (dy != 0 || dx != R) keep = keep & !((uint32_t)row[dx] - base < lim);
        }
        if (active && keep) atomicOr(&s_mask32[n * 8 + (xs >> 5)], 1u << (xs & 31));
      };
      for_each(nbits, nms);
    }

    wave_lds_sync();
    {
      const int r = lane >> 2, wq = lane & 3;
      const int y = cy0 - R + r;
      if (lane < C::G * 4) {
        const uint2 m = reinterpret_cast<const uint2*>(s_mask32)[lane];
        reinterpret_cast<uint2*>(s_mask32)[lane] = make_uint2(0u, 0u);
        if (y >= y0 && y < y1) {
          mask_base[(size_t)y * wpr + wq] = (u64)m.x | ((u64)m.y << 32);
          surv += __popc(m.x) + __popc(m.y);
        }
      }
    }
    wave_lds_sync();
    sm0 += C::G;
    sm0 = sm0 >= C::NS ? sm0 - C::NS : sm0;
  }
  if (row_stat) {
    const int ws = wave_sum(surv);
    if (lane == 0)
      __hip_atomic_fetch_add(row_stat + (size_t)f * ORBX_FAST_STAT_WORDS + d.stat_index + d.ty,
                             (1ull << 32) | (u64)(uint32_t)ws, __ATOMIC_RELAXED, __HIP_MEMORY_SCOPE_AGENT);
  }
}

template <int R>
void launch_fast4(unsigned wgs, hipStream_t s, const OrbxTileDesc* d_tiles, int n_tiles, int n_frames, const uint8_t* d_pyr,
                  int frame_bytes, int mask_words, OrbxFastParams fp, unsigned long long* d_mask,
                  unsigned long long* d_row_stat) {
  if (fp.threshold == 0)
    hipLaunchKernelGGL((k_fast4<R, true>), dim3(wgs), dim3(64), 0, s, d_tiles, n_tiles, n_frames, d_pyr, frame_bytes,
                       mask_words, fp, d_mask, d_row_stat);
  else
    hipLaunchKernelGGL((k_fast4<R, false>), dim3(wgs), dim3(64), 0, s, d_tiles, n_tiles, n_frames, d_pyr, frame_bytes,
                       mask_words, fp, d_mask, d_row_stat);
}

}

hipError_t orbx_launch_fast4(hipStream_t s, const OrbxTileDesc* d_tiles, int n_tiles, int n_frames, const uint8_t* d_pyr,
                             int frame_bytes, int mask_words, OrbxFastParams fp, unsigned long long* d_mask,
                             unsigned long long* d_row_stat) {
  if (n_tiles <= 0 || n_frames <= 0) return hipSuccess;
  const long long total = (long long)n_tiles * n_frames;
  if (total > 0x7fffffffll) return hipErrorInvalidValue;
  switch (fp.nms_radius) {
    case 0:
      launch_fast4<0>((unsigned)total, s, d_tiles, n_tiles, n_frames, d_pyr, frame_bytes, mask_words, fp, d_mask, d_row_stat);
      break;
    case 1:
      launch_fast4<1>((unsigned)total, s, d_tiles, n_tiles, n_frames, d_pyr, frame_bytes, mask_words, fp, d_mask, d_row_stat);
      break;
    case 2:
      launch_fast4<2>((unsigned)total, s, d_tiles, n_tiles, n_frames, d_pyr, frame_bytes, mask_words, fp, d_mask, d_row_stat);
      break;
    default:
      launch_fast4<3>((unsigned)total, s, d_tiles, n_tiles, n_frames, d_pyr, frame_bytes, mask_words, fp, d_mask, d_row_stat);
      break;
  }
  return hipGetLastError();
}
```

visual-odometry-gpu_amd/csrc/orbx_host.h:

```cpp
#pragma once
#include <hip/hip_runtime.h>

#include <cmath>
#include <cstring>
#include <initializer_list>
#include <string>
#include <vector>

#include "../../include/orbx_reloc.h"
#include "orbx_internal.h"
#include "orbx_layout.h"
#include "orbx_tables.h"

namespace orbx_host {

using namespace orbx_geom;
using namespace orbx_layout;

struct DevBuf {
  void* p = nullptr;
  size_t bytes = 0;
};
template <class T>
T* at(const DevBuf& b, size_t off) { return reinterpret_cast<T*>(static_cast<uint8_t*>(b.p) + off); }
inline void free_bufs(std::initializer_list<DevBuf*> bufs) {
  for (DevBuf* b : bufs)
    if (b->p) (void)hipFree(b->p);
}

struct Block {
  uint8_t* d = nullptr;
  uint8_t* h = nullptr;
  uint8_t* h_dev = nullptr;
  OutLayout layout{};
  int n = 0;
  int cap = 1;
  bool copy_pending = false;
  bool copy_compact = false;
  bool host_written = false;
  hipEvent_t ev_done = nullptr, ev_copied = nullptr;
  hipStream_t stream = nullptr;
};

struct Lane {
  uint8_t *d_pyr = nullptr, *d_pyr_blur = nullptr;
  unsigned long long *d_mask = nullptr, *d_row_stat = nullptr;
  orbx_keypoint* d_cand = nullptr;
  int32_t *d_cand_count = nullptr, *d_cand_total = nullptr;
  float* d_resp = nullptr;
  uint32_t* d_lcand = nullptr;
  float* d_lresp = nullptr;
  int32_t* d_lcount = nullptr;
  hipStream_t stream = nullptr;
  hipEvent_t ev_pool = nullptr;
  hipStream_t pool_stream = nullptr;
};

struct TileTable {
  OrbxTileDesc* d = nullptr;
  int count = 0;
};

struct TimingSet {
  hipEvent_t ev[ORBX_NUM_STAGE_TIMES + 3] = {};
  int mode = 0;
  bool split = false;
};

int fail(orbx_ctx* c, int status, const std::string& msg);

#define HIPCHK(c, expr)                                                                              \
  do {                                                                                               \
    hipError_t _e = (expr);                                                                          \
    if (_e != hipSuccess)                                                                            \
      return fail((c), ORBX_ERR_HIP, std::string(#expr) + ": " + hipGetErrorString(_e));             \
  } while (0)

struct SideWork {
  hipStream_t stream = nullptr;
  hipEvent_t ev = nullptr;
  int wait(orbx_ctx* c);
  int enter(orbx_ctx* c, hipStream_t s);
  int after(orbx_ctx* c, const SideWork& producer, hipStream_t s);
  int grow(orbx_ctx* c, DevBuf& b, size_t bytes);
  struct Mark {
    SideWork& w;
    hipStream_t s;
    ~Mark() {
      if (w.ev) (void)hipEventRecord(w.ev, s);
    }
  };
  void release() {
    if (!ev) return;
    (void)hipEventSynchronize(ev);
    (void)hipEventDestroy(ev);
  }
};

struct PinnedUpload {
  void* host = nullptr;
  size_t bytes = 0;
  hipEvent_t ev = nullptr;
  int send(orbx_ctx* c, void* d_dst, const void* src, size_t n, hipStream_t s);
  void release() {
    if (ev) (void)hipEventDestroy(ev);
    if (host) (void)hipHostFree(host);
  }
};


struct StageScratch {
  DevBuf img_a, img_b, f32, u16, mask, kps, f32b, desc, i32, kern;
  DevBuf tiles;
  void release() { free_bufs({&img_a, &img_b, &f32, &u16, &mask, &kps, &f32b, &desc, &i32, &kern, &tiles}); }
};

struct Matcher {
  DevBuf res, in;
  int pairs = 0, cap = 0;
  long long serial = -1;
  long long gen = 0;
  void release() { free_bufs({&res, &in}); }
};

struct LkPair {
  DevBuf img[2], deriv, io;
  void* host = nullptr;
  size_t host_bytes = 0;
  int w = 0, h = 0, top = -1, win = 0, last = -1;
  void release() {
    if (host) (void)hipHostFree(host);
    free_bufs({&img[0], &img[1], &deriv, &io});
  }
};

struct LkWindows {
  DevBuf ws, first, img, pts, res, fbres;
  size_t ws_limit = ORBX_LK_WORKSPACE_DEFAULT;
  int n = 0, cap = 0, len = 0;
  bool fb = false;
  SideWork side;
  PinnedUpload first_up;
  void release() {
    side.release();
    first_up.release();
    free_bufs({&ws, &first, &img, &pts, &res, &fbres});
  }
};

struct Pose {
  DevBuf blk, hblk, hin;
  int pairs = 0, cap = 0;
  hipStream_t stream = nullptr;
  long long serial = -1;
  long long match_gen = -1;
  void release() { free_bufs({&blk, &hblk, &hin}); }
};

struct Scale {
  DevBuf blk, host;
  int pairs = 0, cap = 0;
  hipStream_t stream = nullptr;
  void release() { free_bufs({&blk, &host}); }
};

struct BundleAdjust {
  DevBuf stage, ws;
  void release() { free_bufs({&stage, &ws}); }
};

struct Landmarks {
  DevBuf scr, blk, sol, ws, stage, views;
  double K[9] = {};
  int n = 0, cap = 0, len = 0;
  bool has_views = false;
  bool solved = false;
  long long gen = 0;
  SideWork side;
  PinnedUpload poses_up;
  void release() {
    side.release();
    poses_up.release();
    free_bufs({&scr, &blk, &sol, &ws, &stage, &views});
  }
};

struct TracksPose {
  DevBuf scr, blk, stage;
  int n = 0, cap = 0, len = 0;
  SideWork side;
  void release() {
    side.release();
    free_bufs({&scr, &blk, &stage});
  }
};

struct WindowPoses {
  DevBuf in, blk, wb, stage;
  int n = 0, len = 0;
  int wb_n = 0, wb_len = 0;
  SideWork side;
  PinnedUpload up;
  void release() {
    side.release();
    up.release();
    free_bufs({&in, &blk, &wb, &stage});
  }
};

struct StreamStitch {
  DevBuf in, blk, stage;
  int n = 0, len = 0, stride = 0;
  SideWork side;
  PinnedUpload up;
  void release() {
    side.release();
    up.release();
    free_bufs({&in, &blk, &stage});
  }
};

struct Pnp {
  DevBuf scr, blk, hscr, hblk;
  int n = 0, cap = 0, len = 0;
  long long lm_gen = -1;
  SideWork side;
  void release() {
    side.release();
    free_bufs({&scr, &blk, &hscr, &hblk});
  }
};

struct Carry {
  DevBuf blk, pscr, pblk, stage;
  int n = 0, cap = 0;
  int pn = 0, pcap = 0, plen = 0;
  SideWork side;
  void release() {
    side.release();
    free_bufs({&blk, &pscr, &pblk, &stage});
  }
};

struct Reloc {
  DevBuf ws, list, bank[2], stage, best, rblk, rstage;
  size_t ws_limit = ORBX_PD_WORKSPACE_DEFAULT;
  int n[2] = {0, 0}, cap[2] = {0, 0};
  int rn = 0, rq = 0, rt = 0;
  SideWork side;
  void release() {
    side.release();
    free_bufs({&ws, &list, &bank[0], &bank[1], &stage, &best, &rblk, &rstage});
  }
};

struct GoodFeatures {
  DevBuf ws, img, res, bm, stage, tres;
  size_t ws_limit = ORBX_GFTT_WORKSPACE_DEFAULT;
  int n = 0, cap = 0;
  int tn = 0, tcap = 0;
  SideWork side;
  void release() {
    side.release();
    free_bufs({&ws, &img, &res, &bm, &stage, &tres});
  }
};

}

struct OrbxGraphKey {
  const uint8_t* d_frames;
  size_t frame_stride;
  int n, w, h, row_stride, early, plan_serial, block;
  bool operator==(const OrbxGraphKey& o) const {
    return d_frames == o.d_frames && frame_stride == o.frame_stride && n == o.n && w == o.w && h == o.h &&
           row_stride == o.row_stride && early == o.early && plan_serial == o.plan_serial && block == o.block;
  }
};

struct orbx_ctx {
  orbx_params p{};
  int device = 0;
  hipStream_t stream = nullptr;
  std::string err;

  OrbxPlan plan{};
  OrbxPlan plan_max{};
  OrbxTileMap tm_blur{};
  OrbxBandMap bm_fast{};
  orbx_host::TileTable tiles[kTileTables];
  OrbxTopLevels top_levels{};
  std::vector<OrbxResizeTap> h_taps;
  OrbxPlanTables scratch;
  orbx_geom::OrbxTableCapacity table_cap{};
  int plan_w = 0, plan_h = 0;

  uint8_t* d_in = nullptr;
  static constexpr int kGraphs = 16;
  hipGraphExec_t g_exec[kGraphs] = {};
  OrbxGraphKey g_key[kGraphs] = {};
  int g_next = 0;
  int plan_serial = 0;
  OrbxResizeTap* d_taps = nullptr;
  float* d_gauss = nullptr;
  static constexpr int kBlocks = 4;
  orbx_host::Block blocks[kBlocks];
  int blk = 0;
  int host_results = 0;
  int next_lane = 1;
  hipStream_t cstream = nullptr;
  orbx_host::Lane lanes[2];
  int lane = 0;
  bool pipelined = false;
  bool last_two_pass = false;
  hipStream_t last_stream = nullptr;

  long long batch_serial = 0;
  orbx_host::StageScratch s;
  orbx_host::Matcher m;
  orbx_host::LkPair lk;
  orbx_host::LkWindows lkw;
  orbx_host::Pose pose;
  orbx_host::Scale scale;
  orbx_host::BundleAdjust ba;
  orbx_host::GoodFeatures gf;
  orbx_host::Landmarks lm;
  orbx_host::TracksPose tp;
  orbx_host::WindowPoses wp;
  orbx_host::StreamStitch st;
  orbx_host::Pnp pnp;
  orbx_host::Carry carry;
  orbx_host::Reloc reloc;

  int timing = 0;
  int fast_early = 1;
  int blur_impl = 2;
  int fast_impl = 4;
  int fuse = 1;
  OrbxAdapt adapt;
  uint32_t* d_feedback = nullptr;
  volatile uint32_t* h_feedback = nullptr;
  orbx_host::TimingSet evr[ORBX_EVENT_SETS];
  long long ev_calls = 0;
  hipEvent_t ev[2] = {};
};

namespace orbx_host {

struct DeviceGuard {
  int prev = -1;
  bool switched = false;
  explicit DeviceGuard(const orbx_ctx* c) {
    if (!c) return;
    enter(c->device);
  }
  explicit DeviceGuard(int dev) { enter(dev); }
  void enter(int dev) {
    if (hipGetDevice(&prev) == hipSuccess && prev != dev) switched = hipSetDevice(dev) == hipSuccess;
  }
  ~DeviceGuard() {
    if (switched) (void)hipSetDevice(prev);
  }
  DeviceGuard(const DeviceGuard&) = delete;
  DeviceGuard& operator=(const DeviceGuard&) = delete;
};

int ensure(orbx_ctx* c, DevBuf& b, size_t bytes);
#define ENSURE(c, buf, bytes)                        \
  do {                                               \
    const int _st = ensure((c), (buf), (bytes));     \
    if (_st != ORBX_OK) return _st;                  \
  } while (0)

hipStream_t batch_stream(const orbx_ctx* c);
const Lane& cur_lane(const orbx_ctx* c);
const Block& last_block(const orbx_ctx* c);
hipError_t lanes_sync(orbx_ctx* c);

int check_image(orbx_ctx* c, const void* img, int w, int h, int stride);
struct FramesWhat {
  const char* null_msg;
  std::string range_msg;
};
int check_device_frames(orbx_ctx* c, const void* d_frames, int n, int n_min, int n_max, int w, int h, int row_stride,
                        size_t frame_stride, const FramesWhat& what);
bool finite_all(const double* v, int n);
inline bool pose_args_ok(const double* K, double prob, double threshold, int max_iters) {
  return K && K[0] > 0 && K[4] > 0 && std::isfinite(K[0]) && std::isfinite(K[4]) && std::isfinite(K[2]) &&
         std::isfinite(K[5]) && std::isfinite(prob) && std::isfinite(threshold) && threshold >= 0 && max_iters >= 0 &&
         max_iters <= ORBX_POSE_MAX_ITERS;
}
inline void pose_unpack(const OrbxPoseOut& r, double* E, double* R, double* t, int32_t* inliers, int32_t* good,
                        int32_t* iters) {
  if (E) memcpy(E, r.E, sizeof r.E);
  if (R) memcpy(R, r.R, sizeof r.R);
  if (t) memcpy(t, r.t, sizeof r.t);
  if (inliers) *inliers = r.inliers;
  if (good) *good = r.good;
  if (iters) *iters = r.iters;
}
int gaussian_kernel(int K, float sigma, float* kernel);
hipError_t launch_blur_auto(int impl, hipStream_t s, const OrbxPlan& P, const OrbxTileMap& tm1, const OrbxTileDesc* tiles2,
                            int ntiles2, int n, const uint8_t* src, uint8_t* dst, int first_level, int kind);
int set_workspace_limit(orbx_ctx* c, SideWork& side, std::initializer_list<DevBuf*> ws, size_t* limit, size_t bytes,
                        size_t dflt);
inline hipStream_t stream_of(const orbx_ctx* c, void* stream) { return stream ? (hipStream_t)stream : c->stream; }
inline bool range_ok(int first, int n, int total, int n_min = 1) {
  return first >= 0 && n >= n_min && n <= total - first;
}
int stage_tracks(orbx_ctx* c, SideWork& side, DevBuf& stage, const float* tracks_xy, const int32_t* seen, int n_slots,
                 int window_len, const float** d_tracks, const int32_t** d_seen);
struct LmViewsOptions {
  int tri_mode;
  double max_reproj_px;
};
bool lm_views_ok(const LmViewsOptions& o);
bool ba_params_ok(double huber_delta, int max_iters);
int lm_check_build(orbx_ctx* c, const double* K, const void* tracks, const void* seen, int n, int cap, int len,
                   const double* poses6);
int lm_run(orbx_ctx* c, const double* K, const float* d_tracks, const int32_t* d_seen, int n, int cap, int len,
           const double* poses6, const double* d_poses6, const int32_t* d_pose_status, hipStream_t s,
           const LmViewsOptions* views = nullptr, const SideWork* producer = nullptr);
int tp_check(orbx_ctx* c, const double* K, const void* tracks, const void* seen, int n, int cap, int len, double prob,
             double threshold, int max_iters);
struct WpStreamOptions {
  int stride;
  double scale0_first;
};
int wp_check(orbx_ctx* c, const double* T0, const double* scale0, const WpStreamOptions* stream_of_windows);
int wp_run(orbx_ctx* c, const double* T0, const double* scale0, hipStream_t s,
           const WpStreamOptions* stream_of_windows = nullptr);
bool gate_params_ok(double max_rot, double max_trans);
int lm_solve(orbx_ctx* c, double huber_delta, int max_iters, hipStream_t s, const double* d_poses6,
             const SideWork* producer);

}
```

visual-odometry-gpu_amd/csrc/orbx_internal.h:

```cpp
#pragma once
#include <hip/hip_runtime.h>
#include <stdint.h>

#include "../../include/orbx.h"

#include "orbx_plan.h"

__host__ __device__ inline int orbx_mask_x(const OrbxLevel& L, int xw, int b) {
  return L.mask_strip_px ? (xw >> 2) * L.mask_strip_px + (xw & 3) * 64 + b : xw * 64 + b;
}

#define ORBX_FAST_STAT_WORDS (ORBX_MAX_LEVELS * ORBX_MAX_BANDS + ORBX_MAX_LEVELS)
struct OrbxFastParams {
  int32_t threshold, n, nms_radius;
};

#define ORBX_LK_MAX_LEVELS 8
struct OrbxLkLevel {
  const uint8_t* img;
  const int16_t* deriv;
  int32_t w, h, pitch, pad;
};
struct OrbxLkPyr {
  OrbxLkLevel L[ORBX_LK_MAX_LEVELS];
  int32_t top;
  int32_t pad;
};
hipError_t orbx_launch_lk_pyrdown(hipStream_t s, const uint8_t* d_src, int sw, int sh, int spitch, uint8_t* d_dst,
                                  int dw, int dh, int dpitch);
hipError_t orbx_launch_lk_scharr(hipStream_t s, const uint8_t* d_img, int w, int h, int pitch, int16_t* d_deriv);
hipError_t orbx_launch_lk_track(hipStream_t s, const OrbxLkPyr& prev, const OrbxLkPyr& next, int n,
                                const float* d_prev_pts, float* d_next_pts, uint8_t* d_status, float* d_err, int win,
                                int max_iters, double eps2);
struct OrbxLkFrames {
  OrbxLkLevel L[ORBX_LK_MAX_LEVELS];
  size_t frame_stride, img_stride, der_stride;
  int32_t top, first;
};
hipError_t orbx_launch_lk_pyrdown_frames(hipStream_t s, int frames, const uint8_t* d_src, int sw, int sh, int spitch,
                                         size_t src_frame_stride, uint8_t* d_dst, int dw, int dh, int dpitch,
                                         size_t dst_frame_stride);
hipError_t orbx_launch_lk_scharr_frames(hipStream_t s, int frames, const uint8_t* d_img, int w, int h, int pitch,
                                        size_t img_frame_stride, int16_t* d_deriv, size_t deriv_frame_bytes);
hipError_t orbx_launch_lk_track_windows(hipStream_t s, const OrbxLkFrames& frames, const int32_t* d_window_first,
                                        int n_windows, int window_len, const float* d_points, const int32_t* d_counts,
                                        int slot_capacity, float* d_tracks, int32_t* d_seen, float* d_err, int win,
                                        int max_iters, double eps2);
hipError_t orbx_launch_lk_track_windows_fb(hipStream_t s, const OrbxLkFrames& frames, const int32_t* d_window_first,
                                           int n_windows, int window_len, const float* d_points,
                                           const int32_t* d_counts, int slot_capacity, float* d_tracks, int32_t* d_seen,
                                           float* d_err, float* d_fb_d2, int32_t* d_lost, int win, int max_iters,
                                           double eps2, double thr2);

hipError_t orbx_launch_pyramid2(hipStream_t s, const OrbxTileDesc* d_tiles, int n_tiles, int frame_bytes, int w0,
                                int h0, int n_frames, const uint8_t* d_in, int in_stride, size_t in_frame_stride,
                                const OrbxResizeTap* d_taps, uint8_t* d_pyr);
hipError_t orbx_launch_blur(hipStream_t s, const OrbxPlan& plan, const OrbxTileMap& tm, int n_frames,
                            const uint8_t* d_src, uint8_t* d_dst, int first_level, int kind);
hipError_t orbx_launch_blur3(hipStream_t s, const OrbxTileDesc* d_tiles, int n_tiles, int frame_bytes, int n_frames,
                             const uint8_t* d_src, uint8_t* d_dst, int first_level);
hipError_t orbx_launch_blur4(hipStream_t s, const OrbxTileDesc* d_tiles, int n_tiles, int frame_bytes, int n_frames,
                             const uint8_t* d_src, uint8_t* d_dst, int first_level);
hipError_t orbx_launch_pyrblur(hipStream_t s, const OrbxTileDesc* d_tiles, int n_tiles, int frame_bytes, int w0, int h0,
                               int n_frames, const uint8_t* d_in, int in_stride, size_t in_frame_stride,
                               const OrbxResizeTap* d_taps, uint8_t* d_dst, int group = 0,
                               const unsigned long long* d_row_stat = nullptr, uint32_t* d_feedback = nullptr,
                               const OrbxTopLevels* top = nullptr, unsigned long long* d_zero_stat = nullptr);
hipError_t orbx_launch_fast_nms(hipStream_t s, const OrbxTileDesc* d_tiles, int n_tiles, int n_frames,
                                const uint8_t* d_pyr, int frame_bytes, int mask_words, OrbxFastParams fp,
                                unsigned long long* d_mask, uint16_t* d_scores,
                                unsigned long long* d_row_stat, int chunk_scale = 1);
hipError_t orbx_launch_fast4(hipStream_t s, const OrbxTileDesc* d_tiles, int n_tiles, int n_frames, const uint8_t* d_pyr,
                             int frame_bytes, int mask_words, OrbxFastParams fp, unsigned long long* d_mask,
                             unsigned long long* d_row_stat);
hipError_t orbx_launch_compact(hipStream_t s, const OrbxPlan& plan, int n_frames,
                               const unsigned long long* d_mask, orbx_keypoint* d_cand, int32_t* d_cand_count,
                               int32_t* d_cand_total, int need_total);
hipError_t orbx_launch_harris_flat(hipStream_t s, const uint8_t* d_img, int w, int h, int pitch,
                                   const orbx_keypoint* d_kps, int nkp, const float* d_gauss, int K, float kk,
                                   float* d_resp);
hipError_t orbx_launch_level_select(hipStream_t s, const OrbxPlan& plan, int n_frames, int mode,
                                    const unsigned long long* d_mask, const uint8_t* d_pyr, const float* d_gauss,
                                    int window, float k, orbx_keypoint* d_sel_lkp, float* d_sel_resp,
                                    int32_t* d_sel_count, uint32_t* d_need = nullptr);
hipError_t orbx_launch_level_select_auto(hipStream_t s, const OrbxPlan& plan, int n_frames, int mode, int force,
                                         const unsigned long long* d_mask, const uint8_t* d_pyr,
                                         const float* d_gauss, int window, float k, uint32_t* d_cand,
                                         int32_t* d_ncand, float* d_cresp, orbx_keypoint* d_sel_lkp,
                                         float* d_sel_resp, int32_t* d_sel_count, uint32_t* d_need = nullptr);
struct OrbxHostRecord {
  int32_t* counts;
  uint32_t* kp16;
  float* angle;
  orbx_descriptor* desc;
};
hipError_t orbx_launch_describe(hipStream_t s, const OrbxPlan& plan, int n_frames, const uint8_t* d_pyr,
                                int patch_size, const int32_t* d_sel_count, const orbx_keypoint* d_sel_lkp,
                                const float* d_sel_resp, int32_t* d_out_count, orbx_keypoint* d_out_lkp,
                                float* d_out_resp, int32_t* d_out_level, orbx_keypoint* d_out_kp, uint32_t* d_out_kp16,
                                float* d_out_angle, orbx_descriptor* d_out_desc, const uint32_t* d_feedback = nullptr,
                                uint32_t* h_feedback = nullptr, const OrbxHostRecord* host_record = nullptr);

hipError_t orbx_launch_describe_flat(hipStream_t s, const uint8_t* d_img, int w, int h, int pitch,
                                     const orbx_keypoint* d_kps, int nkp, int patch_size, int use_given_angles,
                                     int do_brief, float* d_angles, orbx_descriptor* d_desc);
hipError_t orbx_launch_nms_f32(hipStream_t s, const float* d_scores, int w, int h, int radius, float threshold,
                               unsigned long long* d_mask, int mask_wpr);
hipError_t orbx_launch_conv2d(hipStream_t s, const uint8_t* d_img, int w, int h, int pitch, const float* d_kernel,
                              int K, int reflect_pad, uint8_t* d_dst, int dst_pitch);
hipError_t orbx_launch_select_flat(hipStream_t s, const float* d_resp, int n, int keep, int32_t* d_idx);

hipError_t orbx_launch_knn2(hipStream_t s, int npairs, int max_nq, const orbx_descriptor* d_q, const int32_t* d_qcount,
                            size_t qstride, const orbx_descriptor* d_t, const int32_t* d_tcount, size_t tstride,
                            double ratio, int32_t* d_idx, int32_t* d_dist, int32_t* d_match, size_t ostride);

struct OrbxPosePt {
  double x1, y1, x2, y2;
};
struct OrbxPoseOut {
  double E[9], R[9], t[3];
  int32_t inliers, good, iters, pad;
};
hipError_t orbx_launch_pose_prep_batch(hipStream_t s, int npairs, int cap, const int32_t* d_counts,
                                       const orbx_keypoint* d_kp, const int32_t* d_match, const double* K,
                                       OrbxPosePt* d_pts, int32_t* d_npts);
hipError_t orbx_launch_pose_prep_host(hipStream_t s, int n, const float* d_p1, const float* d_p2, const double* K,
                                      OrbxPosePt* d_pts, int32_t* d_npts);
hipError_t orbx_launch_pose_ransac(hipStream_t s, int npairs, int cap, const OrbxPosePt* d_pts, const int32_t* d_npts,
                                   const double* K, double prob, double threshold, int max_iters, uint64_t seed,
                                   OrbxPoseOut* d_out, uint8_t* d_mask);

struct OrbxScaleOut {
  double scale;
  int32_t triplets, ratios_used;
};
#define ORBX_SCALE_LDS_MAX (160 * 1024 - 256)
hipError_t orbx_launch_triangulate_batch(hipStream_t s, int npairs, int cap, const int32_t* d_counts,
                                         const orbx_keypoint* d_kp, const int32_t* d_match, const OrbxPoseOut* d_pose,
                                         const double* K, float* d_xyz, uint8_t* d_valid, int32_t* d_mq, int32_t* d_mt,
                                         int32_t* d_npts);
hipError_t orbx_launch_triangulate_host(hipStream_t s, int n, const float* d_p1, const float* d_p2, const double* K,
                                        const double* R, const double* t, float* d_xyz, uint8_t* d_valid);
hipError_t orbx_launch_scale_join(hipStream_t s, int npairs, int chain, int cap, const int32_t* d_npts, const int32_t* d_mq,
                                  const int32_t* d_mt, const float* d_xyz, const uint8_t* d_valid,
                                  const OrbxPoseOut* d_pose, OrbxScaleOut* d_out);
hipError_t orbx_launch_scale_aligned(hipStream_t s, int n_prev, int n_cur, const float* d_prev,
                                     const uint8_t* d_prev_valid, const float* d_cur, const uint8_t* d_cur_valid,
                                     OrbxScaleOut* d_out);

#define ORBX_BA_WS_POINT 30
#define ORBX_BA_WS_OBS 18
#define ORBX_BA_MAX_POINTS 65536
#define ORBX_BA_MAX_GROUPS 512
#define ORBX_BA_WS_BUDGET ((size_t)2 << 30)
hipError_t orbx_launch_ba(hipStream_t s, int n_windows, int groups, int max_iters, const double* K4, double delta,
                          const int32_t* d_pose_off, const int32_t* d_pt_off, const int32_t* d_obs_off,
                          double* d_poses, double* d_points, const int32_t* d_rows, const uint8_t* d_obs_pose,
                          const double* d_obs_xy, int cap, int ocap, double* d_ws_pt, double* d_ws_obs,
                          unsigned long long* d_ws_slot, void* d_out);

#define ORBX_LM_THREADS 256
struct OrbxLmBlock {
  int32_t *status, *pose_off, *pt_off, *obs_off;
  double* points3;
  int32_t* rows;
  uint8_t* opose;
  double* oxy;
  int32_t* slot_of_point;
};
inline int orbx_lm_blocks(int cap) { return (cap + ORBX_LM_THREADS - 1) / ORBX_LM_THREADS; }
hipError_t orbx_launch_landmarks(hipStream_t s, const double* K9, const double* d_poses, const float* d_tracks,
                                 const int32_t* d_seen, int n_windows, int cap, int window_len, double* d_cand,
                                 uint8_t* d_keep, int32_t* d_partial, int32_t* d_gate, const OrbxLmBlock& out,
                                 const int32_t* d_pose_status = nullptr);
hipError_t orbx_launch_landmarks_views(hipStream_t s, const double* K9, const double* d_poses, const float* d_tracks,
                                       const int32_t* d_seen, int n_windows, int cap, int window_len, int tri_mode,
                                       double max_reproj_px, double* d_table, uint8_t* d_reason, float* d_reproj_px,
                                       double* d_cand, uint8_t* d_keep, int32_t* d_partial, int32_t* d_gate,
                                       const OrbxLmBlock& out, const int32_t* d_pose_status = nullptr);

hipError_t orbx_launch_window_poses(hipStream_t s, int n_windows, int window_len, const OrbxPoseOut* d_pose,
                                    const OrbxScaleOut* d_scale, const double* d_T0, const double* d_scale0,
                                    double* d_poses6, double* d_poses4x4, int32_t* d_status);
hipError_t orbx_launch_ba_write_back(hipStream_t s, int n_windows, int window_len, const double* d_solved6,
                                     const double* d_built6, const void* d_summaries, double max_rot,
                                     double max_trans, double* d_poses4x4, uint8_t* d_updated);

struct OrbxPnpCorr {
  double X[3], x, y;
};
struct OrbxPnpRecord {
  double pose6[6];
  int32_t inliers, iters, n_corr, status;
  double rms_px;
};
struct OrbxPnpIn {
  const int32_t *status, *pt_off, *obs_off, *rows;
  const double *points3, *oxy, *built6;
};
hipError_t orbx_launch_pnp(hipStream_t s, int n_windows, int window_len, int cap, const OrbxPnpIn& in, int n_pre,
                           const double* K4, double prob, double threshold_px, int max_iters, uint64_t seed,
                           int refine_iters, int min_inliers, OrbxPnpCorr* d_corr, int32_t* d_cidx,
                           OrbxPnpRecord* d_rec, double* d_seeded6, uint8_t* d_mask,
                           const int32_t* d_ncorr = nullptr);

enum { CARRY_OK = 0, CARRY_LOST = 1 };
struct OrbxCarryIn {
  const int32_t *status, *pt_off, *slot;
  const double* src;
  int old_cap;
};
hipError_t orbx_launch_carry_join(hipStream_t s, const OrbxCarryIn& in, const int32_t* d_origin, int n_windows, int cap,
                                  double* d_xyz, int32_t* d_point, int32_t* d_count);
hipError_t orbx_launch_carry_gather(hipStream_t s, const double* d_xyz, const int32_t* d_point, const int32_t* d_count,
                                    const float* d_tracks, const int32_t* d_seen, int n_windows, int cap, int window_len,
                                    OrbxPnpCorr* d_corr, int32_t* d_cidx, int32_t* d_ncorr);
hipError_t orbx_launch_carry_fill(hipStream_t s, const OrbxPnpRecord* d_rec, int n_windows, int window_len,
                                  double* d_poses6, int32_t* d_wstatus);

enum { PD_NONE = 0, PD_BORDER = 1, PD_OK = 2 };
#define PD_R_MIN 20
#define PD_LEVEL0_COPY 2
hipError_t orbx_launch_pd_level0(hipStream_t s, const uint8_t* d_frames, int n, int w, int h, int row_stride,
                                 size_t frame_stride, int kind, uint8_t* d_level0, int pitch, size_t img_stride);
hipError_t orbx_launch_pd_describe(hipStream_t s, const uint8_t* d_level0, int n, int w, int h, int pitch,
                                   size_t img_stride, const float* d_xy, size_t point_stride, size_t xy_frame_stride,
                                   const int32_t* d_seen, int seen_min, const int32_t* d_counts, int cap, int patch_size,
                                   int32_t* d_state, float* d_angle, orbx_descriptor* d_desc, int32_t* d_n_ok,
                                   int32_t* d_list);
hipError_t orbx_launch_reassociate(hipStream_t s, int n_windows, const orbx_descriptor* d_qdesc,
                                   const int32_t* d_qstate, int qcap, const orbx_descriptor* d_tdesc,
                                   const int32_t* d_tstate, int tcap, double ratio, int max_distance, int unique,
                                   uint32_t* d_best, int32_t* d_origin, int32_t* d_dist, int32_t* d_count);

hipError_t orbx_launch_st_scale0(hipStream_t s, int n_windows, int window_len, int stride, double scale0_first,
                                 const OrbxScaleOut* d_scale, double* d_scale0);
hipError_t orbx_launch_stitch(hipStream_t s, int n_windows, int window_len, int stride, const double* d_poses4x4,
                              const double* d_T_start, int align_scale, double* d_links, int32_t* d_broken,
                              double* d_trajectory4x4, int32_t* d_owner, double* d_anchors4x4, double* d_lambda,
                              int32_t* d_status);

hipError_t orbx_launch_tracks_prep(hipStream_t s, int n_windows, int cap, int window_len, const float* d_tracks,
                                   const int32_t* d_seen, const double* K, OrbxPosePt* d_pts, int32_t* d_npts,
                                   int32_t* d_slot_of, uint8_t* d_mask, float* d_xyz, uint8_t* d_valid);
hipError_t orbx_launch_tracks_triangulate(hipStream_t s, int n_windows, int cap, int window_len, const float* d_tracks,
                                          const int32_t* d_npts, const int32_t* d_slot_of, const OrbxPoseOut* d_pose,
                                          const double* K, float* d_xyz, uint8_t* d_valid);

hipError_t orbx_launch_gftt_response(hipStream_t s, const uint8_t* d_frames, int n, int w, int h, int row_stride,
                                     size_t frame_stride, float* d_map, uint32_t* d_max);
hipError_t orbx_launch_gftt_candidates(hipStream_t s, const float* d_map, int n, int w, int h, const uint32_t* d_max,
                                       double quality, unsigned long long* d_keys, size_t pool, int32_t* d_ncand);
hipError_t orbx_launch_gftt_select(hipStream_t s, int n, int w, unsigned long long* d_keys, size_t pool,
                                   const int32_t* d_ncand, double min_distance, int cell, int gw, int gh, int slots,
                                   uint32_t* d_grid, size_t grid_stride, int cap, int32_t* d_counts,
                                   float* d_corners);
hipError_t orbx_launch_gftt_seeds(hipStream_t s, int n, const float* d_seed_xy, size_t point_stride,
                                  size_t frame_stride, const int32_t* d_seed_seen, int seen_min, int seed_cap, int w,
                                  int h, int slot_cap, int32_t* d_carried, float* d_points, int32_t* d_origin);
hipError_t orbx_launch_gftt_block(hipStream_t s, int n, const float* d_points, const int32_t* d_carried, int slot_cap,
                                  int max_seeds, int w, int h, double min_distance, uint32_t* d_bits);
hipError_t orbx_launch_gftt_mask_bits(hipStream_t s, const uint8_t* d_mask, int w, int h, int mask_stride,
                                      uint32_t* d_bits);
hipError_t orbx_launch_gftt_masked_max(hipStream_t s, const float* d_map, int n, int w, int h, const uint32_t* d_bits,
                                       uint32_t* d_mmax);
hipError_t orbx_launch_gftt_candidates_blocked(hipStream_t s, const float* d_map, int n, int w, int h,
                                               const uint32_t* d_mmax, double quality, unsigned long long* d_keys,
                                               size_t pool, int32_t* d_ncand, const uint32_t* d_bits);
hipError_t orbx_launch_gftt_select_topup(hipStream_t s, int n, int w, unsigned long long* d_keys, size_t pool,
                                         const int32_t* d_ncand, double min_distance, int cell, int gw, int gh,
                                         int slots, uint32_t* d_grid, size_t grid_stride, int slot_cap,
                                         const int32_t* d_carried, int32_t* d_counts, float* d_points);
```

visual-odometry-gpu_amd/csrc/orbx_plan.h:

```cpp
#pragma once
#include <stddef.h>
#include <stdint.h>

#include <algorithm>
#include <cmath>
#include <cstring>
#include <string>
#include <vector>

#include "../../include/orbx.h"

struct OrbxLevel {
  int32_t w, h, pitch;
  int32_t img_off;
  int32_t mask_wpr;
  int32_t mask_off;
  int32_t cap;
  int32_t quota;
  int32_t cand_off;
  int32_t xtab_off;
  int32_t ytab_off;
  float scale;
  int32_t out_off;
  int32_t win8;
  int32_t mask_strip_px;
};

struct OrbxPlan {
  int32_t nlevels;
  int32_t w0, h0;
  int32_t frame_bytes;
  int32_t mask_words;
  int32_t cand_total;
  int32_t out_cap;
  OrbxLevel L[ORBX_MAX_LEVELS];
};

struct OrbxTileMap {
  int32_t begin[ORBX_MAX_LEVELS + 1];
  int32_t tiles_x[ORBX_MAX_LEVELS];
};

#define ORBX_MAX_BANDS 64
#define ORBX_MIN_TILE_H 16
#define ORBX_FAST_UNIT_ROWS_MAX 128
struct OrbxBandMap {
  int32_t nbands;
  int32_t band_begin[ORBX_MAX_BANDS + 1];
  int32_t tiles_x[ORBX_MAX_LEVELS];
  int32_t tiles_y[ORBX_MAX_LEVELS];
  int32_t tile_h[ORBX_MAX_LEVELS];
  int32_t xprefix[ORBX_MAX_LEVELS + 1];
  int32_t first_h[ORBX_MAX_LEVELS][2];
};

struct OrbxTileDesc {
  int32_t l, tx, ty, f;
  int32_t w, h, pitch;
  int32_t u0;
  int32_t u1;
  int32_t u2;
  uint32_t stat_index;
  uint32_t pad;
  uint64_t img_off;
  uint64_t mask_off;
};
static_assert(sizeof(OrbxTileDesc) == 64, "one 64-byte scalar load per workgroup");

struct OrbxResizeTap {
  int32_t ofs;
  int16_t c0, c1;
};

struct OrbxTopLevels {
  int32_t n;
  int32_t stat_index[ORBX_MAX_LEVELS];
  int32_t rows[ORBX_MAX_LEVELS];
  int32_t cap[ORBX_MAX_LEVELS];
};

#define ORBX_FAST3_TW 128
#define ORBX_FAST3_K 7
constexpr int orbx_fast3_tile_h(int nms_radius) {
  return (256 / (ORBX_FAST3_TW / 4 + 2)) * ORBX_FAST3_K - 2 * nms_radius;
}
constexpr int orbx_fast4_halo(int nms_radius) { return (nms_radius + 3 + 3) / 4; }
constexpr int orbx_fast4_strip_lanes(int nms_radius) { return 64 - 2 * orbx_fast4_halo(nms_radius); }
constexpr int orbx_fast4_strips(int w, int nms_radius) {
  const int ndw = (w + 3) / 4, s = orbx_fast4_strip_lanes(nms_radius), n = (ndw - 2 * orbx_fast4_halo(nms_radius) + s - 1) / s;
  return n < 1 ? 1 : n;
}
#define ORBX_BLUR_TW 64
#define ORBX_BLUR_TH 16
#define ORBX_BLUR3_TW 256
#define ORBX_BLUR3_RH 64
#define ORBX_BLUR4_TW 256
#define ORBX_BLUR4_RH 96
#define ORBX_PYRBLUR_TW 248
#define ORBX_PYR_STAGE_BYTES 832
#define ORBX_PYRBLUR_RH 58
#define ORBX_PYRBLUR_RH_SMALL 12
#define ORBX_PYR2_TW 256
#define ORBX_PYR2_TH 16

#define ORBX_MAX_SELECT 4096

#define ORBX_TOP_MARGIN 21

namespace orbx_geom {

inline int align_up(int v, int a) { return (v + a - 1) / a * a; }
inline size_t align_up_sz(size_t v, size_t a) { return (v + a - 1) / a * a; }


inline float level_scale(float sf, int l) { return (float)std::pow((double)sf, (double)l); }

inline void level_size(int w0, int h0, float sf, int l, int* wl, int* hl) {
  if (l == 0) {
    *wl = w0;
    *hl = h0;
    return;
  }
  const float scale = level_scale(sf, l);
  *wl = (int)std::round((double)((float)w0 / scale));
  *hl = (int)std::round((double)((float)h0 / scale));
}

inline int level_quota(int nfeatures, float sf, int nlevels, int l) {
  const float inv = 1 / sf;
  const float num = 1 - inv;
  const double den = 1 - std::pow((double)inv, (double)nlevels);
  return (int)(nfeatures * ((double)num / den) * std::pow((double)inv, (double)l));
}

inline void make_tilemap(const OrbxPlan& plan, int tw, int th, bool use_pitch, OrbxTileMap* tm) {
  int acc = 0;
  for (int l = 0; l < plan.nlevels; l++) {
    const int wcols = use_pitch ? plan.L[l].pitch : plan.L[l].w;
    const int tx = (wcols + tw - 1) / tw, ty = (plan.L[l].h + th - 1) / th;
    tm->begin[l] = acc;
    tm->tiles_x[l] = tx;
    acc += tx * ty;
  }
  for (int l = plan.nlevels; l <= ORBX_MAX_LEVELS; l++) tm->begin[l] = acc;
}

inline int fast_tiles_x(int w, int nms_radius, bool strips) {
  return strips ? orbx_fast4_strips(w, nms_radius) : (w + ORBX_FAST3_TW - 1) / ORBX_FAST3_TW;
}

inline int make_bandmap(const OrbxPlan& plan, int nms_radius, OrbxBandMap* bm, std::string* why, bool strips = false,
                        const int* pref_h = nullptr, const int (*first_h)[2] = nullptr) {
  std::memset(bm, 0, sizeof(*bm));
  const int th = orbx_fast3_tile_h(nms_radius);
  int nb = 0;
  for (int l = 0; l < plan.nlevels; l++) {
    bm->tiles_x[l] = fast_tiles_x(plan.L[l].w, nms_radius, strips);
    bm->tiles_y[l] = (plan.L[l].h + th - 1) / th;
    bm->tile_h[l] = (plan.L[l].h + bm->tiles_y[l] - 1) / bm->tiles_y[l];
    if (pref_h && pref_h[l] > 0 && pref_h[l] < bm->tile_h[l]) {
      int hh = std::max(pref_h[l], ORBX_MIN_TILE_H);
      const int most = l > 0 ? std::min(bm->tiles_y[l - 1], ORBX_MAX_BANDS) : ORBX_MAX_BANDS;
      while ((plan.L[l].h + hh - 1) / hh > most) hh++;
      if (hh < bm->tile_h[l]) {
        bm->tile_h[l] = hh;
        bm->tiles_y[l] = (plan.L[l].h + hh - 1) / hh;
      }
    }
    if (first_h && first_h[l][0] > 0 && first_h[l][1] > 0) {
      const int a = first_h[l][0], b = first_h[l][1];
      const int unit_max = strips ? ORBX_FAST_UNIT_ROWS_MAX : th;
      if (a + b == 2 * bm->tile_h[l] && bm->tiles_y[l] >= 2 && a < plan.L[l].h && a <= unit_max && b <= unit_max) {
        bm->first_h[l][0] = a;
        bm->first_h[l][1] = b;
      }
    }
    bm->xprefix[l + 1] = bm->xprefix[l] + bm->tiles_x[l];
    if (l > 0 && bm->tiles_y[l] > bm->tiles_y[l - 1]) {
      *why = "pyramid levels must not grow with the level index";
      return ORBX_ERR_UNSUPPORTED;
    }
    nb = std::max(nb, bm->tiles_y[l]);
  }
  if (nb > ORBX_MAX_BANDS) {
    *why = "image taller than ORBX_MAX_BANDS FAST tile rows";
    return ORBX_ERR_UNSUPPORTED;
  }
  bm->nbands = nb;
  int acc = 0;
  for (int b = 0; b < nb; b++) {
    bm->band_begin[b] = acc;
    for (int l = 0; l < plan.nlevels; l++)
      if (bm->tiles_y[l] > b) acc += bm->tiles_x[l];
  }
  for (int b = nb; b <= ORBX_MAX_BANDS; b++) bm->band_begin[b] = acc;
  return ORBX_OK;
}

inline void fast_band_rows(const OrbxBandMap& bm, int l, int b, int* y0, int* rows) {
  const bool cut = bm.first_h[l][0] > 0 && b < 2;
  *y0 = cut ? (b == 0 ? 0 : bm.first_h[l][0]) : b * bm.tile_h[l];
  *rows = cut ? bm.first_h[l][b] : bm.tile_h[l];
}


inline size_t build_fast_tiles(const OrbxPlan& plan, const OrbxBandMap& bm, int first_band, int strip,
                               std::vector<OrbxTileDesc>* out) {
  size_t cnt = 0;
  if (out) out->clear();
  for (int b = first_band; b < bm.nbands; b++)
    for (int l = 0; l < plan.nlevels; l++) {
      if (bm.tiles_y[l] <= b) continue;
      const OrbxLevel& L = plan.L[l];
      int y0, rows;
      fast_band_rows(bm, l, b, &y0, &rows);
      for (int tx = 0; tx < bm.tiles_x[l]; tx += strip) {
        OrbxTileDesc d{};
        d.l = l;
        d.tx = tx;
        d.ty = b;
        d.f = bm.tile_h[l];
        d.pad = (uint32_t)y0 | ((uint32_t)rows << 16);
        d.w = L.w;
        d.h = L.h;
        d.pitch = L.pitch;
        d.u0 = L.cap;
        d.u1 = L.mask_wpr;
        d.u2 = bm.tiles_x[l];
        d.stat_index = (uint32_t)(l * ORBX_MAX_BANDS);
        d.img_off = (uint64_t)L.img_off;
        d.mask_off = (uint64_t)L.mask_off;
        if (out) out->push_back(d);
        cnt++;
      }
    }
  return cnt;
}

inline size_t build_frame_tiles(const OrbxPlan& plan, int tw, int th, bool pyramid_fields, std::vector<OrbxTileDesc>* out) {
  size_t cnt = 0;
  if (out) out->clear();
  for (int l = 0; l < plan.nlevels; l++) {
    const OrbxLevel& L = plan.L[l];
    const int rpw = pyramid_fields ? ((l == 0 || L.win8 == 1) ? 8 : 4) : 0;
    if (pyramid_fields) th = 4 * rpw;
    const int ntx = (L.pitch + tw - 1) / tw, nty = (L.h + th - 1) / th;
    for (int ty = 0; ty < nty; ty++)
      for (int tx = 0; tx < ntx; tx++) {
        OrbxTileDesc d{};
        d.l = l;
        d.tx = tx;
        d.ty = ty;
        d.f = rpw;
        d.w = L.w;
        d.h = L.h;
        d.pitch = L.pitch;
        if (pyramid_fields) {
          d.u0 = L.xtab_off;
          d.u1 = L.ytab_off;
          d.u2 = L.win8 == 1;
        }
        d.img_off = (uint64_t)L.img_off;
        if (out) out->push_back(d);
        cnt++;
      }
  }
  return cnt;
}

inline size_t build_blur_tiles(const OrbxPlan& plan, std::vector<OrbxTileDesc>* out) {
  size_t cnt = 0;
  if (out) out->clear();
  for (int l = 0; l < plan.nlevels; l++) {
    const OrbxLevel& L = plan.L[l];
    const int ntx = (L.pitch + ORBX_BLUR3_TW - 1) / ORBX_BLUR3_TW;
    const int nb = (L.h + ORBX_BLUR3_RH - 1) / ORBX_BLUR3_RH, rows = (L.h + nb - 1) / nb;
    for (int b = 0; b < nb; b++)
      for (int tx = 0; tx < ntx; tx++) {
        OrbxTileDesc d{};
        d.l = l;
        d.tx = tx;
        d.ty = b * rows;
        d.f = std::min(rows, L.h - b * rows);
        d.w = L.w;
        d.h = L.h;
        d.pitch = L.pitch;
        d.img_off = (uint64_t)L.img_off;
        if (d.f > 0) {
          if (out) out->push_back(d);
          cnt++;
        }
      }
  }
  return cnt;
}

inline size_t build_blur4_tiles(const OrbxPlan& plan, std::vector<OrbxTileDesc>* out) {
  size_t cnt = 0;
  if (out) out->clear();
  for (int l = 0; l < plan.nlevels; l++) {
    const OrbxLevel& L = plan.L[l];
    const int ntx = (L.pitch + ORBX_BLUR4_TW - 1) / ORBX_BLUR4_TW;
    const int nwv = (L.h + 4 * ORBX_BLUR4_RH - 1) / (4 * ORBX_BLUR4_RH), rows = (L.h + 4 * nwv - 1) / (4 * nwv);
    for (int wv = 0; wv < nwv; wv++)
      for (int tx = 0; tx < ntx; tx++) {
        OrbxTileDesc d{};
        d.l = l;
        d.tx = tx;
        d.ty = wv * 4 * rows;
        d.f = rows;
        d.w = L.w;
        d.h = L.h;
        d.pitch = L.pitch;
        d.img_off = (uint64_t)L.img_off;
        if (d.ty < L.h) {
          if (out) out->push_back(d);
          cnt++;
        }
      }
  }
  return cnt;
}

inline size_t blur_tiles_for_impl(int impl, const OrbxPlan& plan, std::vector<OrbxTileDesc>* out) {
  return impl == 3 ? build_blur4_tiles(plan, out) : build_blur_tiles(plan, out);
}

inline int pyrblur_first_pass_rows(const OrbxPlan& plan, const OrbxBandMap& bm, int l, int top_rows) {
  if (top_rows <= 0 || bm.tiles_y[l] <= top_rows) return plan.L[l].h;
  int y0, rows;
  fast_band_rows(bm, l, top_rows - 1, &y0, &rows);
  return std::min(plan.L[l].h, y0 + rows + ORBX_TOP_MARGIN);
}
inline int pyrblur_early_rows(const OrbxPlan& plan, const OrbxBandMap& bm, int l, int top_rows, int nms_radius) {
  const int late = pyrblur_first_pass_rows(plan, bm, l, top_rows);
  if (top_rows != 2 || bm.tiles_y[l] <= top_rows || bm.first_h[l][0] <= 0 || late >= plan.L[l].h) return late;
  const int h0 = bm.first_h[l][0], D = h0 + bm.first_h[l][1];
  return std::min(late, std::max(h0 + ORBX_TOP_MARGIN, D + nms_radius + 3));
}
inline int pyrblur_strips_x(int w) {
  const int dw = (w + 3) / 4;
  return dw <= 64 ? 1 : (dw - 2 + 61) / 62;
}
inline int pyrblur_row_cost(int l, int win8) { return l == 0 ? 35 : win8 == 1 ? 80 : 90; }
#define ORBX_PYRBLUR_WARMUP_ROWS 4
inline size_t build_pyrblur_tiles(const OrbxPlan& plan, int max_rows, std::vector<OrbxTileDesc>* out,
                                  bool heavy_first = false, int part = 0, const OrbxBandMap* bm = nullptr,
                                  int top_rows = 0, const int* early_rows = nullptr) {
  size_t cnt = 0;
  if (out) out->clear();
  bool have_reporter = false;
  for (int l = 0; l < plan.nlevels; l++) {
    const OrbxLevel& L = plan.L[l];
    const int ntx = pyrblur_strips_x(L.w);
    const int split = part == 0 ? L.h : pyrblur_first_pass_rows(plan, *bm, l, top_rows);
    const int early = part != 0 && early_rows && early_rows[l] > 0 && early_rows[l] < split ? early_rows[l] : split;
    const int seg[2][3] = {{part == 2 ? early : 0, part == 1 ? early : part == 2 ? split : L.h, 1},
                           {split, part == 2 ? L.h : split, std::min(top_rows, bm ? bm->tiles_y[l] : 0)}};
    for (int s = 0; s < 2; s++) {
      const int r0 = seg[s][0], r1 = seg[s][1];
      if (r1 <= r0) continue;
      const int nb = (r1 - r0 + max_rows - 1) / max_rows, rows = (r1 - r0 + nb - 1) / nb;
      for (int b = 0; b < nb; b++)
        for (int tx = 0; tx < ntx; tx++) {
          OrbxTileDesc d{};
          d.l = l;
          d.tx = tx;
          d.ty = r0 + b * rows;
          d.f = std::min(rows, r1 - d.ty);
          d.w = L.w;
          d.h = L.h;
          d.pitch = L.pitch;
          d.u0 = L.xtab_off;
          d.u1 = L.ytab_off;
          d.u2 = L.win8;
          d.pad = (uint32_t)ntx;
          d.img_off = (uint64_t)L.img_off;
          if (part == 2) {
            d.stat_index = (uint32_t)(l * ORBX_MAX_BANDS);
            d.mask_off = ((uint64_t)(uint32_t)seg[s][2] << 32) | (uint32_t)L.cap;
            if (s == 1 && b == 0 && tx == 0 && !have_reporter) {
              d.mask_off |= 1ull << 62;
              have_reporter = true;
            }
          }
          if (d.f > 0) {
            if (out) out->push_back(d);
            cnt++;
          }
        }
    }
  }
  if (heavy_first && out) {
    auto cost = [](const OrbxTileDesc& d) { return (d.f + ORBX_PYRBLUR_WARMUP_ROWS) * pyrblur_row_cost(d.l, d.u2); };
    std::stable_sort(out->begin(), out->end(),
                     [&](const OrbxTileDesc& a, const OrbxTileDesc& b) { return cost(a) > cost(b); });
  }
  return cnt;
}

inline int build_plan(const orbx_params& p, int w0, int h0, OrbxPlan* plan, std::string* why, int fast_impl = 3) {
  std::memset(plan, 0, sizeof(*plan));
  plan->nlevels = p.nlevels;
  plan->w0 = w0;
  plan->h0 = h0;
  size_t img_off = 0, mask_off = 0;
  int cand_off = 0, out_cap = 0, xt = 0;
  for (int l = 0; l < p.nlevels; l++) {
    OrbxLevel& L = plan->L[l];
    level_size(w0, h0, p.scale_factor, l, &L.w, &L.h);
    if (L.w < 8 || L.h < 8) {
      *why = "pyramid level " + std::to_string(l) + " is smaller than 8x8 (" + std::to_string(L.w) + "x" +
             std::to_string(L.h) + ")";
      return ORBX_ERR_UNSUPPORTED;
    }
    L.pitch = align_up(L.w, 64);
    L.img_off = (int32_t)img_off;
    img_off = align_up_sz(img_off + (size_t)L.pitch * L.h, 256);
    if (fast_impl == 4) {
      L.mask_strip_px = 4 * orbx_fast4_strip_lanes(p.nms_window / 2);
      L.mask_wpr = 4 * orbx_fast4_strips(L.w, p.nms_window / 2);
    } else {
      L.mask_wpr = (L.w + 63) / 64;
    }
    L.mask_off = (int32_t)mask_off;
    mask_off += (size_t)L.mask_wpr * L.h;
    int quota;
    if (p.select_mode == ORBX_SELECT_ROWMAJOR && p.nlevels == 1)
      quota = p.nfeatures;
    else
      quota = level_quota(p.nfeatures, p.scale_factor, p.nlevels, l);
    if (quota < 0) quota = 0;
    L.quota = quota;
    L.cap = p.select_mode == ORBX_SELECT_HARRIS ? 2 * quota : quota;
    if (L.cap > ORBX_MAX_SELECT) {
      *why = "per-level FAST cap " + std::to_string(L.cap) + " exceeds ORBX_MAX_SELECT";
      return ORBX_ERR_UNSUPPORTED;
    }
    L.cand_off = cand_off;
    cand_off += L.cap;
    L.out_off = out_cap;
    out_cap += quota;
    L.scale = level_scale(p.scale_factor, l);
    L.xtab_off = xt;
    L.ytab_off = xt + (l == 0 ? 0 : align_up(L.w, 4));
    xt += (l == 0 ? 0 : align_up(L.w, 4) + align_up(L.h, 4));
    if (img_off > 0x7fffffffull) {
      *why = "pyramid frame exceeds 2 GiB";
      return ORBX_ERR_UNSUPPORTED;
    }
  }
  plan->frame_bytes = (int32_t)img_off;
  plan->mask_words = (int32_t)mask_off;
  plan->cand_total = std::max(cand_off, (out_cap + 15) & ~15);
  plan->out_cap = (out_cap + 15) & ~15;
  return ORBX_OK;
}

inline size_t taps_count(const OrbxPlan& plan) {
  size_t total = 0;
  for (int l = 1; l < plan.nlevels; l++) total += (size_t)align_up(plan.L[l].w, 4) + align_up(plan.L[l].h, 4);
  return total ? total : 1;
}

inline void make_taps(OrbxPlan& plan, std::vector<OrbxResizeTap>* taps) {
  taps->assign(taps_count(plan), OrbxResizeTap{0, 0, 0});
  for (int l = 1; l < plan.nlevels; l++) {
    const OrbxLevel& L = plan.L[l];
    const double scale_x = 1. / ((double)L.w / plan.w0), scale_y = 1. / ((double)L.h / plan.h0);
    for (int dx = 0; dx < L.w; dx++) {
      float fx = (float)((dx + 0.5) * scale_x - 0.5);
      int sx = (int)std::floor(fx);
      fx -= (float)sx;
      if (sx < 0) {
        fx = 0;
        sx = 0;
      }
      if (sx >= plan.w0 - 1) {
        fx = 0;
        sx = plan.w0 - 1;
      }
      OrbxResizeTap& t = (*taps)[L.xtab_off + dx];
      t.ofs = sx;
      t.c0 = (int16_t)std::lrintf((1.f - fx) * 2048.f);
      t.c1 = (int16_t)std::lrintf(fx * 2048.f);
      if (sx == plan.w0 - 1) {
        t.ofs = plan.w0 - 2;
        t.c1 = t.c0;
        t.c0 = 0;
      }
    }
    {
      bool ok = plan.w0 >= 8;
      for (int dx = 0; dx + 3 < L.w && ok; dx += 4)
        ok = (*taps)[L.xtab_off + dx + 3].ofs + 1 - (*taps)[L.xtab_off + dx].ofs <= 7;
      for (int dx = L.w & ~3; dx < L.w && ok; dx++)
        ok = (*taps)[L.xtab_off + dx].ofs + 1 - (*taps)[L.xtab_off + (L.w & ~3)].ofs <= 7;
      plan.L[l].win8 = ok ? 1 : 0;
      if (!ok && plan.w0 >= 8) {
        bool ok3 = true;
        for (int x0 = 0; x0 < L.w && ok3; x0 += ORBX_PYRBLUR_TW) {
          const int ofs_first = (*taps)[L.xtab_off + x0].ofs, ofs_last = (*taps)[L.xtab_off + std::min(x0 + 255, L.w - 1)].ofs;
          const int want = ofs_first - ((ofs_first - plan.w0) & 3), span0 = std::max(want, 0);
          ok3 = ofs_last + 2 - span0 <= ORBX_PYR_STAGE_BYTES;
          if (want < 0 && (plan.w0 & 3) && ofs_last + 2 > (plan.w0 & ~3)) ok3 = false;
        }
        if (ok3) plan.L[l].win8 = 3;
      }
    }
    for (int dy = 0; dy < L.h; dy++) {
      float fy = (float)((dy + 0.5) * scale_y - 0.5);
      int sy = (int)std::floor(fy);
      fy -= (float)sy;
      OrbxResizeTap& t = (*taps)[L.ytab_off + dy];
      t.ofs = sy;
      t.c0 = (int16_t)std::lrintf((1.f - fy) * 2048.f);
      t.c1 = (int16_t)std::lrintf(fy * 2048.f);
    }
  }
}

struct OrbxTableCapacity {
  size_t fast;
  size_t frame;
  size_t small;
  size_t taps;
};
static_assert(ORBX_TOP_MARGIN <= ORBX_PYRBLUR_RH, "an early band is one band");
inline size_t pyrblur_early_strips_bound(const OrbxPlan& M) {
  size_t n = 0;
  for (int l = 0; l < M.nlevels; l++) n += (size_t)pyrblur_strips_x(M.L[l].w);
  return n;
}
inline size_t fast_tiles_upper_bound(const OrbxPlan& M, int nms_radius, bool strips) {
  size_t cap = 0;
  for (int l = 0; l < M.nlevels; l++) {
    const int rows = std::min(ORBX_MAX_BANDS, (M.L[l].h + ORBX_MIN_TILE_H - 1) / ORBX_MIN_TILE_H);
    cap += (size_t)fast_tiles_x(M.L[l].w, nms_radius, strips) * (size_t)rows;
  }
  return cap;
}
inline int table_capacity(const orbx_params& p, const OrbxPlan& M, int fast_impl, int blur_impl, OrbxTableCapacity* cap,
                          std::string* why) {
  OrbxBandMap bm;
  const int st = make_bandmap(M, p.nms_window / 2, &bm, why, fast_impl == 4, nullptr);
  if (st != ORBX_OK) return st;
  cap->fast = fast_tiles_upper_bound(M, p.nms_window / 2, fast_impl == 4);
  const size_t t1 = blur_tiles_for_impl(blur_impl, M, nullptr);
  const size_t t2 = build_frame_tiles(M, ORBX_PYR2_TW, ORBX_PYR2_TH, true, nullptr);
  const size_t t3 = build_pyrblur_tiles(M, ORBX_PYRBLUR_RH, nullptr);
  cap->frame = std::max(std::max(t1, t2), t3) + 256 + pyrblur_early_strips_bound(M);
  cap->small = build_pyrblur_tiles(M, ORBX_PYRBLUR_RH_SMALL, nullptr) + 64;
  cap->taps = taps_count(M) + 16;
  return ORBX_OK;
}

#define ORBX_FILL_BUCKETS 32
#define ORBX_FILL_BUCKET_ROWS 4
inline int fill_bucket(int fill_row) { return std::min(std::max(fill_row - 1, 0) / ORBX_FILL_BUCKET_ROWS, ORBX_FILL_BUCKETS - 1); }
#define ORBX_FEEDBACK_HIST (2 + ORBX_MAX_LEVELS)
#define ORBX_FEEDBACK_WORDS (ORBX_FEEDBACK_HIST + ORBX_MAX_LEVELS * ORBX_FILL_BUCKETS)
inline uint32_t fill_exits(const uint32_t* hist, int cut) {
  uint32_t n = 0;
  for (int b = 0; b < ORBX_FILL_BUCKETS - 1 && ORBX_FILL_BUCKET_ROWS * (b + 1) <= cut; b++) n += hist[b];
  return n;
}
#define ORBX_FAST4_UNIT_SETUP_MILLI 1200
#define ORBX_FAST4_UNIT_EXIT_MILLI 280
struct OrbxUnitCost {
  int setup_milli, exit_milli;
};
inline int fast4_unit_cost_milli(int rows, int nms_radius, const OrbxUnitCost& uc) {
  return uc.setup_milli + 1000 * ((rows + 2 * nms_radius + 6) / 7);
}
inline int first_pass_cost_milli(const uint32_t* hist, int depth, int cut, int nms_radius,
                                 const OrbxUnitCost& uc = OrbxUnitCost{ORBX_FAST4_UNIT_SETUP_MILLI, ORBX_FAST4_UNIT_EXIT_MILLI}) {
  uint64_t total = 0;
  for (int b = 0; b < ORBX_FILL_BUCKETS; b++) total += hist[b];
  const uint64_t out = total ? fill_exits(hist, cut) : 0, on = total ? total - out : 1;
  const uint64_t second = (on * (uint64_t)fast4_unit_cost_milli(depth - cut, nms_radius, uc) + out * (uint64_t)uc.exit_milli) /
                          (total ? total : 1);
  return fast4_unit_cost_milli(cut, nms_radius, uc) + (int)second;
}
inline int choose_first_cut(const uint32_t* hist, int depth, int nms_radius, int unit_max, int* cost_milli,
                            const OrbxUnitCost& uc = OrbxUnitCost{ORBX_FAST4_UNIT_SETUP_MILLI, ORBX_FAST4_UNIT_EXIT_MILLI}) {
  uint64_t total = 0;
  for (int b = 0; b < ORBX_FILL_BUCKETS; b++) total += hist[b];
  int best = 0, best_cost = first_pass_cost_milli(hist, depth, depth / 2, nms_radius, uc);
  if (total)
    for (int cut = 7 - (2 * nms_radius) % 7; cut < depth; cut += 7) {
      if (cut > unit_max || depth - cut > unit_max || cut == depth / 2) continue;
      if (fill_exits(hist, cut) == 0) continue;
      const int c = first_pass_cost_milli(hist, depth, cut, nms_radius, uc);
      if (c < best_cost) {
        best = cut;
        best_cost = c;
      }
    }
  if (cost_milli) *cost_milli = best_cost;
  return best;
}

#define ORBX_PYRBLUR_SKIP_EXIT 100
#define ORBX_PYRBLUR_EARLY_MIN_ROWS 3
inline bool early_band_pays(const uint32_t* hist, int h0, int rows, int row_cost, int exit_cost = ORBX_PYRBLUR_SKIP_EXIT) {
  uint64_t total = 0;
  for (int b = 0; b < ORBX_FILL_BUCKETS; b++) total += hist[b];
  if (!total || rows < ORBX_PYRBLUR_EARLY_MIN_ROWS) return false;
  const uint64_t out = fill_exits(hist, h0), stay = total - out;
  return out * (uint64_t)rows * (uint64_t)row_cost >
         stay * (uint64_t)(ORBX_PYRBLUR_WARMUP_ROWS * row_cost) + out * (uint64_t)exit_cost;
}

}
```

visual-odometry-gpu_amd/csrc/orbx_tables.h:

```cpp
#pragma once
#include <cstdio>
#include <string>
#include <vector>

#include "orbx_adapt.h"

enum {
  T_FAST,
  T_BLUR,
  T_PYR2,
  T_PYRBLUR,
  T_PYRBLUR_SMALL,
  T_PYRBLUR_TOP,
  T_PYRBLUR_REST,
  kTileTables
};

struct OrbxTableSwitches {
  int fast_impl, blur_impl;
  int top_rows;
  bool grouped;
  bool prefs_apply;
};

struct OrbxPlanTables {
  OrbxTileMap tm_blur{};
  OrbxBandMap bm_fast{};
  std::vector<OrbxTileDesc> tiles[kTileTables];
  OrbxTopLevels top_levels{};
};

namespace orbx_tables {

using namespace orbx_adapt;

inline size_t tile_table_capacity(const OrbxTableCapacity& cap, int table) {
  return table == T_FAST ? cap.fast : table == T_PYRBLUR_SMALL ? cap.small : cap.frame;
}

inline int plan_with_taps(const orbx_params& p, int w, int h, int fast_impl, OrbxPlan* plan,
                          std::vector<OrbxResizeTap>* taps, std::string* why) {
  const int st = build_plan(p, w, h, plan, why, fast_impl);
  if (st != ORBX_OK) return st;
  make_taps(*plan, taps);
  return ORBX_OK;
}

inline int build_tile_tables(const OrbxPlan& plan, int nms_radius, const OrbxTableSwitches& sw,
                             const OrbxTableCapacity& cap, OrbxAdapt& a, FILE* trace, OrbxPlanTables* out,
                             std::string* why) {
  OrbxBandMap& bm = out->bm_fast;
  const OrbxAdaptGeom geom{plan, bm, nms_radius, sw.fast_impl, sw.top_rows};
  auto too_large = [&](int table, const char* msg) {
    if (out->tiles[table].size() <= tile_table_capacity(cap, table)) return false;
    *why = msg;
    return true;
  };
  make_tilemap(plan, ORBX_BLUR_TW, ORBX_BLUR_TH, true, &out->tm_blur);
  a.prefs_applied = sw.prefs_apply;
  int st = make_bandmap(plan, nms_radius, &bm, why, sw.fast_impl == 4, a.prefs_applied ? a.tile_h_pref : nullptr);
  if (a.prefs_applied && (st != ORBX_OK || (size_t)bm.band_begin[bm.nbands] > cap.fast)) {
    forget_tile_rows(a);
    st = make_bandmap(plan, nms_radius, &bm, why, sw.fast_impl == 4, nullptr);
  }
  if (st != ORBX_OK) return st;
  int first[ORBX_MAX_LEVELS][2] = {};
  if (first_pass_heights(a, geom, first))
    (void)make_bandmap(plan, nms_radius, &bm, why, sw.fast_impl == 4, a.prefs_applied ? a.tile_h_pref : nullptr, first);
  const bool grouped = sw.grouped;
  const int top = sw.top_rows;
  blur_tiles_for_impl(sw.blur_impl, plan, &out->tiles[T_BLUR]);
  if (too_large(T_BLUR, "blur tile table exceeds pool")) return ORBX_ERR_UNSUPPORTED;
  build_pyrblur_tiles(plan, ORBX_PYRBLUR_RH, &out->tiles[T_PYRBLUR], grouped);
  if (too_large(T_PYRBLUR, "strip table exceeds pool")) return ORBX_ERR_UNSUPPORTED;
  choose_early_bands(a, geom, trace);
  build_pyrblur_tiles(plan, ORBX_PYRBLUR_RH, &out->tiles[T_PYRBLUR_TOP], grouped, 1, &bm, top, a.early_rows);
  if (too_large(T_PYRBLUR_TOP, "strip table exceeds pool")) return ORBX_ERR_UNSUPPORTED;
  build_pyrblur_tiles(plan, ORBX_PYRBLUR_RH, &out->tiles[T_PYRBLUR_REST], grouped, 2, &bm, top, a.early_rows);
  if (too_large(T_PYRBLUR_REST, "strip table exceeds pool")) return ORBX_ERR_UNSUPPORTED;
  out->top_levels = OrbxTopLevels{};
  for (int l = 0; l < plan.nlevels; l++)
    if (pyrblur_first_pass_rows(plan, bm, l, top) < plan.L[l].h) {
      const int i = out->top_levels.n++;
      out->top_levels.stat_index[i] = l * ORBX_MAX_BANDS;
      out->top_levels.rows[i] = std::min(top, bm.tiles_y[l]);
      out->top_levels.cap[i] = plan.L[l].cap;
    }
  build_pyrblur_tiles(plan, ORBX_PYRBLUR_RH_SMALL, &out->tiles[T_PYRBLUR_SMALL]);
  if (too_large(T_PYRBLUR_SMALL, "strip table exceeds pool")) return ORBX_ERR_UNSUPPORTED;
  build_frame_tiles(plan, ORBX_PYR2_TW, ORBX_PYR2_TH, true, &out->tiles[T_PYR2]);
  if (too_large(T_PYR2, "pyramid tile table exceeds pool")) return ORBX_ERR_UNSUPPORTED;
  build_fast_tiles(plan, bm, 0, 1, &out->tiles[T_FAST]);
  if (too_large(T_FAST, "FAST tile table exceeds pool")) return ORBX_ERR_UNSUPPORTED;
  return ORBX_OK;
}

}
```

Baseline: 699,000 frames/s.

## Pack narrow FAST tail strips of several frames into one wave

In the first FAST pass, the last column strip of each level often fills only a few of the 64 lanes. This change packs 2 or 4 frames' tail strips into a single 64-lane workgroup, using a per-frame buffer offset and per-quarter mask and stat writes. A separate pack tile table and a grid prefix are passed to the kernel, and the adaptive first-cut cost model now weights row-0 cost by the packed share. It cuts wasted lanes and workgroup count on narrow levels, but adds lane-index arithmetic, extra LDS syncs and a serialized per-frame stats reduction.

```diff
diff --git a/visual-odometry-gpu_amd/csrc/orbx_adapt.h b/visual-odometry-gpu_amd/csrc/orbx_adapt.h
--- a/visual-odometry-gpu_amd/csrc/orbx_adapt.h
+++ b/visual-odometry-gpu_amd/csrc/orbx_adapt.h
@@ -2,6 +2,7 @@
 #include <cstdio>
 #include <cstdlib>
 
+#include "orbx_pack.h"
 #include "orbx_plan.h"
 
 struct OrbxAdapt {
@@ -19,12 +20,14 @@
   uint32_t fill_last[ORBX_MAX_LEVELS][ORBX_FILL_BUCKETS] = {};
   int early_rows[ORBX_MAX_LEVELS] = {};
   bool early_band = true;
+  bool tail_pack = true, two_pass_small = false;
 };
 
 struct OrbxAdaptGeom {
   const OrbxPlan& plan;
   const OrbxBandMap& bm;
   int nms_radius, fast_impl, top_rows;
+  bool tail_pack = false;
 };
 
 namespace orbx_adapt {
@@ -45,6 +48,10 @@
       a.split_trace = true;
     } else if (!std::strncmp(e, "late", 4)) {
       a.early_band = false;
+    } else if (!std::strncmp(e, "nopack", 6)) {
+      a.tail_pack = false;
+    } else if (!std::strncmp(e, "small", 5)) {
+      a.two_pass_small = true;
     } else {
       for (int l = 0; l < ORBX_MAX_LEVELS; l++) {
         char* end = nullptr;
@@ -159,8 +166,10 @@
     const int depth = 2 * th_after;
     const int in_force = !heights_change && g.bm.first_h[l][0] > 0 ? g.bm.first_h[l][0] : 0;
     int cost_new = 0;
-    const int cut_new = total && lh > depth ? choose_first_cut(hist, depth, R, ORBX_FAST_UNIT_ROWS_MAX, &cost_new) : 0;
-    const int cost_now = first_pass_cost_milli(hist, depth, in_force ? in_force : depth / 2, R);
+    const OrbxUnitCost uc{ORBX_FAST4_UNIT_SETUP_MILLI, ORBX_FAST4_UNIT_EXIT_MILLI};
+    const int share = orbx_pack::fast4_row0_share_milli(g.plan, l, R, g.tail_pack && g.fast_impl == 4);
+    const int cut_new = total && lh > depth ? choose_first_cut(hist, depth, R, ORBX_FAST_UNIT_ROWS_MAX, &cost_new, uc, share) : 0;
+    const int cost_now = first_pass_cost_milli(hist, depth, in_force ? in_force : depth / 2, R, uc, share);
     if (!total || lh <= depth) cost_new = cost_now;
     const bool pays = cost_now - cost_new >= 1000, stopped = in_force && !cut_new && cost_now > cost_new;
     cut_want[l] = heights_change || pays || stopped ? cut_new : a.cut_pref[l];
diff --git a/visual-odometry-gpu_amd/csrc/orbx_api.cpp b/visual-odometry-gpu_amd/csrc/orbx_api.cpp
--- a/visual-odometry-gpu_amd/csrc/orbx_api.cpp
+++ b/visual-odometry-gpu_amd/csrc/orbx_api.cpp
@@ -310,7 +310,7 @@
   return c->adapt.top_mode == 2 && top_rows_env() > 0 && fast_early_on(c) && fused_pyrblur(c);
 }
 OrbxAdaptGeom adapt_geom(const orbx_ctx* c) {
-  return OrbxAdaptGeom{c->plan, c->bm_fast, c->p.nms_window / 2, c->fast_impl, top_rows_env()};
+  return OrbxAdaptGeom{c->plan, c->bm_fast, c->p.nms_window / 2, c->fast_impl, top_rows_env(), c->adapt.tail_pack};
 }
 FILE* adapt_trace(const orbx_ctx* c) { return c->adapt.split_trace ? stderr : nullptr; }
 
@@ -325,7 +325,7 @@
   if (c->h_taps.size() > c->table_cap.taps) return fail(c, ORBX_ERR_UNSUPPORTED, "resize table exceeds pool");
   c->plan_w = c->plan_h = 0;
   OrbxPlanTables& T = c->scratch;
-  const OrbxTableSwitches sw{c->fast_impl, c->blur_impl, top_rows_env(), pyr_group_env() > 0, tile_prefs_apply(c)};
+  const OrbxTableSwitches sw{c->fast_impl, c->blur_impl, top_rows_env(), pyr_group_env() > 0, tile_prefs_apply(c), c->adapt.tail_pack};
   st = build_tile_tables(plan, c->p.nms_window / 2, sw, c->table_cap, c->adapt, adapt_trace(c), &T, &why);
   if (st != ORBX_OK) return fail(c, st, why);
   HIPCHK(c, hipStreamSynchronize(batch_stream(c)));
@@ -342,6 +342,11 @@
       HIPCHK(c, hipMemcpy(c->tiles[i].d, t.data(), t.size() * sizeof(OrbxTileDesc), hipMemcpyHostToDevice));
     c->tiles[i].count = (int)t.size();
   }
+  if (!T.fast_pack.empty())
+    HIPCHK(c, hipMemcpy(c->fast_pack.d, T.fast_pack.data(), T.fast_pack.size() * sizeof(OrbxTileDesc), hipMemcpyHostToDevice));
+  c->fast_pack.count = (int)T.fast_pack.size();
+  c->fast_pack_units = std::min(T.fast_pack_units, ORBX_MAX_LEVELS);
+  for (int i = 0; i < c->fast_pack_units; i++) c->fast_pack_head[i] = T.fast_pack[i];
   c->plan = plan;
   c->tm_blur = T.tm_blur;
   c->bm_fast = T.bm_fast;
@@ -366,6 +371,18 @@
     return orbx_launch_fast4(s, tiles, count, n, final_pyr(c), c->plan.frame_bytes, c->plan.mask_words, fp, mask, stat);
   return orbx_launch_fast_nms(s, tiles, count, n, final_pyr(c), c->plan.frame_bytes, c->plan.mask_words, fp, mask, nullptr,
                               stat, chunk_scale);
+}
+
+hipError_t launch_fast_first(orbx_ctx* c, hipStream_t s, int first_tiles, int n, OrbxFastParams fp, unsigned long long* stat) {
+  OrbxPackGrid pg;
+  c->last_pack_units = c->last_pack_waves = 0;
+  if (c->fast_impl != 4 || c->fast_pack_units <= 0 || c->fast_pack.count != first_tiles ||
+      !orbx_pack::fast4_pack_grid(c->fast_pack_head, c->fast_pack_units, n, &pg))
+    return launch_fast_tiles(c, s, 0, first_tiles, n, fp, stat);
+  c->last_pack_units = pg.n_units;
+  c->last_pack_waves = pg.blocks;
+  return orbx_launch_fast4(s, c->fast_pack.d, c->fast_pack.count, n, final_pyr(c), c->plan.frame_bytes, c->plan.mask_words, fp,
+                           cur_lane(c).d_mask, stat, &pg);
 }
 
 hipError_t launch_fast_whole(orbx_ctx* c, hipStream_t s, int n, OrbxFastParams fp, bool stats_zeroed = false) {
@@ -389,8 +406,10 @@
     return hipSuccess;
   };
   const bool fused = fused_pyrblur(c);
+  c->last_pack_units = c->last_pack_waves = 0;
   const bool small = (long long)n * whole.count < 4096;
-  const bool two_pass = fused && !small && fast_early_on(c) && top_rows_wanted(c->adapt, top_rows_env()) && rest.count > 0 &&
+  const bool few = small && !c->adapt.two_pass_small;
+  const bool two_pass = fused && !few && fast_early_on(c) && top_rows_wanted(c->adapt, top_rows_env()) && rest.count > 0 &&
                         c->bm_fast.nbands > top_rows_env();
   if (!two_pass) HIPCHK(c, hipMemsetAsync(L.d_row_stat, 0, (size_t)n * ORBX_FAST_STAT_WORDS * 8, s));
   HIPCHK(c, mark(0, false));
@@ -407,7 +426,7 @@
                                     c->d_taps, L.d_pyr_blur, pyr_group_env(), nullptr, c->d_feedback, nullptr,
                                     L.d_row_stat));
       HIPCHK(c, mark(ORBX_NUM_STAGE_TIMES + 1, true));
-      HIPCHK(c, launch_fast_tiles(c, s, 0, first_tiles, n, fp, L.d_row_stat));
+      HIPCHK(c, launch_fast_first(c, s, first_tiles, n, fp, L.d_row_stat));
       HIPCHK(c, mark(ORBX_NUM_STAGE_TIMES + 2, true));
       HIPCHK(c, orbx_launch_pyrblur(s, rest.d, rest.count, P.frame_bytes, P.w0, P.h0, n, d_frames, row_stride,
                                     frame_stride, c->d_taps, L.d_pyr_blur, pyr_group_env(), L.d_row_stat, c->d_feedback,
@@ -626,6 +645,7 @@
   }
   for (TileTable& T : c->tiles)
     if (T.d) (void)hipFree(T.d);
+  if (c->fast_pack.d) (void)hipFree(c->fast_pack.d);
   void* bufs[] = {c->d_in, c->d_taps, c->d_gauss, c->d_feedback};
   for (void* b : bufs)
     if (b) (void)hipFree(b);
@@ -736,6 +756,7 @@
   c->table_cap = tcap;
   for (int i = 0; i < kTileTables; i++)
     CREATE_CHK(hipMalloc((void**)&c->tiles[i].d, std::max<size_t>(tile_table_capacity(tcap, i), 1) * sizeof(OrbxTileDesc)));
+  CREATE_CHK(hipMalloc((void**)&c->fast_pack.d, std::max<size_t>(tcap.fast, 1) * sizeof(OrbxTileDesc)));
   CREATE_CHK(hipMalloc((void**)&c->d_taps, tcap.taps * sizeof(OrbxResizeTap)));
   {
     const int K = p->harris_window;
@@ -929,6 +950,15 @@
         w += (long long)(h[(size_t)f * ORBX_FAST_STAT_WORDS + (size_t)l * ORBX_MAX_BANDS + b] >> 32);
   *total = (long long)c->bm_fast.band_begin[c->bm_fast.nbands] * n;
   *worked = fast_early_on(c) ? w : *total;
+  return ORBX_OK;
+}
+
+int orbx_debug_tail_packs(orbx_ctx* c, int* units, int* waves) {
+  DeviceGuard _dg(c);
+  if (!c || !units || !waves) return ORBX_ERR_INVALID_ARG;
+  if (c->plan_w == 0 || last_block(c).n < 1) return fail(c, ORBX_ERR_INVALID_ARG, "run a batch first");
+  *units = c->last_pack_units;
+  *waves = c->last_pack_waves;
   return ORBX_OK;
 }
 
diff --git a/visual-odometry-gpu_amd/csrc/orbx_fast4.hip b/visual-odometry-gpu_amd/csrc/orbx_fast4.hip
--- a/visual-odometry-gpu_amd/csrc/orbx_fast4.hip
+++ b/visual-odometry-gpu_amd/csrc/orbx_fast4.hip
@@ -33,46 +33,54 @@
   return (((1u << b) - 1u) & ~((1u << a) - 1u)) * 0x01010101u;
 }
 
-template <int R, bool ZT>
-__global__ __launch_bounds__(64) void k_fast4(const OrbxTileDesc* __restrict__ tiles, int n_tiles, int n_frames,
-                                              const uint8_t* __restrict__ pyr, int frame_bytes, int mask_words,
-                                              OrbxFastParams fp, u64* __restrict__ mask, u64* __restrict__ row_stat) {
+template <int R>
+struct F4Lds {
+  uint32_t* img32;
+  uint16_t* sc;
+  uint16_t* queue;
+  uint32_t* cflag;
+  uint32_t* mask32;
+  uint32_t* lut32;
+  int* qn;
+};
+
+template <int R, bool ZT, bool PK>
+__device__ __forceinline__ void f4_unit(const F4Lds<R>& S, const OrbxTileDesc& d, int f0, int n_frames,
+                                        const uint8_t* __restrict__ pyr, int frame_bytes, int mask_words,
+                                        OrbxFastParams fp, u64* __restrict__ mask, u64* __restrict__ row_stat) {
   typedef F4<R> C;
   typedef F3Ring<C::IMG_PITCH> RG;
-  __shared__ __attribute__((aligned(16))) uint32_t s_img32[C::IMG_SLOTS * 64];
-  __shared__ __attribute__((aligned(16))) uint16_t s_sc[C::NS * C::SC_PITCH];
-  __shared__ __attribute__((aligned(16))) uint16_t s_queue[C::QCAP];
-  __shared__ __attribute__((aligned(16))) uint32_t s_cflag[64];
-  __shared__ __attribute__((aligned(16))) uint32_t s_mask32[C::G * 8];
-  __shared__ __attribute__((aligned(16))) uint32_t s_lut32[128];
-  __shared__ int s_qn;
+  uint32_t* const s_img32 = S.img32;
+  uint16_t* const s_sc = S.sc;
+  uint16_t* const s_queue = S.queue;
+  uint32_t* const s_cflag = S.cflag;
+  uint32_t* const s_mask32 = S.mask32;
+  uint32_t* const s_lut32 = S.lut32;
+  int& s_qn = *S.qn;
   const uint8_t* s_img = reinterpret_cast<const uint8_t*>(s_img32);
   const uint8_t* s_lut = reinterpret_cast<const uint8_t*>(s_lut32);
 
   const int lane = threadIdx.x;
-  const int lin = blockIdx.x;
-  const int tile = lin / n_frames, f = lin - tile * n_frames;
-  const OrbxTileDesc d = f3_tile(tiles, tile);
-  if (row_stat && d.ty > 0) {
-    u64* st = row_stat + (size_t)f * ORBX_FAST_STAT_WORDS;
-    u64* dead = st + ORBX_MAX_LEVELS * ORBX_MAX_BANDS + d.l;
-    const u64 pv = f3_probe_issue(st + d.stat_index, dead, d.ty, lane);
-    if (f3_probe_decide(pv, dead, d.ty, d.u2, d.u0, lane)) return;
-  }
+  const int f = f0;
+  const int Q = PK ? d.f : 1, wsh = PK ? (Q == 4 ? 4 : 5) : 6;
+  const int q = PK ? lane >> wsh : 0, lq = PK ? lane & ((1 << wsh) - 1) : lane;
+  const int nq = PK ? min(Q, n_frames - f0) : 1;
+  const bool on = !PK || q < nq;
   const int w = d.w, h = d.h, pitch = d.pitch, th = (int)(d.pad >> 16);
   const int y0 = (int)(d.pad & 0xffffu), y1 = min(y0 + th, h);
   const int thr = fp.threshold, narc_any = fp.n;
   const bool first = d.tx == 0, last = d.tx + 1 == d.u2;
   const int dw0 = d.tx * C::S;
-  const int x_lane = 4 * (dw0 + lane);
+  const int x_lane = 4 * (dw0 + lq);
   const int P0 = first ? 0 : 4 * (dw0 + C::HD), P1 = last ? 4 * (dw0 + 64) : 4 * (dw0 + 64 - C::HD);
-  const uint32_t scol = f4_colmask(x_lane, max(P0 - R, 3), min(P1 + R, w - 3));
-  const uint32_t pcol = f4_colmask(x_lane, max(P0, 3), min(P1, w - 3));
+  const uint32_t scol = on ? f4_colmask(x_lane, max(P0 - R, 3), min(P1 + R, w - 3)) : 0u;
+  const uint32_t pcol = on ? f4_colmask(x_lane, max(P0, 3), min(P1, w - 3)) : 0u;
   const int sy_lo = max(y0 - R, 3), sy_hi = min(y1 + R, h - 3);
 
   const __amdgpu_buffer_rsrc_t rsrc = __builtin_amdgcn_make_buffer_rsrc(
-      const_cast<uint8_t*>(pyr) + ((size_t)f * (size_t)frame_bytes + d.img_off), 0, pitch * h, 0x00020000);
-  const uint32_t voff = x_lane < pitch ? (uint32_t)x_lane : 0xffffffffu;
+      const_cast<uint8_t*>(pyr) + ((size_t)f * (size_t)frame_bytes + d.img_off), 0,
+      (int)((uint32_t)(nq - 1) * (uint32_t)frame_bytes + (uint32_t)(pitch * h)), 0x00020000);
+  const uint32_t voff = on && x_lane < pitch ? (uint32_t)x_lane + (uint32_t)q * (uint32_t)frame_bytes : 0xffffffffu;
   const int rbase = y0 - R - 3;
   auto issue = [&](int t, uint32_t& r) {
     const int ry = min(max(rbase + t, 0), h - 1);
@@ -274,7 +282,7 @@
     }
 
     wave_lds_sync();
-    {
+    if (!PK) {
       const int r = lane >> 2, wq = lane & 3;
       const int y = cy0 - R + r;
       if (lane < C::G * 4) {
@@ -285,51 +293,119 @@
           surv += __popc(m.x) + __popc(m.y);
         }
       }
+    } else {
+      const int wpf = 4 >> (6 - wsh);
+      for (int i = lane; i < C::G * 4 * Q; i += 64) {
+        const int wq = i & 3, qq = (i >> 2) & (Q - 1), r = i >> (8 - wsh);
+        const int y = cy0 - R + r;
+        uint2 m = make_uint2(0u, 0u);
+        if (wq < wpf) m = reinterpret_cast<const uint2*>(s_mask32)[r * 4 + qq * wpf + wq];
+        if (qq < nq && y >= y0 && y < y1) {
+          mask_base[(size_t)qq * (size_t)mask_words + (size_t)y * wpr + wq] = (u64)m.x | ((u64)m.y << 32);
+          surv += __popc(m.x) + __popc(m.y);
+        }
+      }
+      wave_lds_sync();
+      if (lane < C::G * 4) reinterpret_cast<uint2*>(s_mask32)[lane] = make_uint2(0u, 0u);
     }
     wave_lds_sync();
     sm0 += C::G;
     sm0 = sm0 >= C::NS ? sm0 - C::NS : sm0;
   }
   if (row_stat) {
-    const int ws = wave_sum(surv);
-    if (lane == 0)
-      __hip_atomic_fetch_add(row_stat + (size_t)f * ORBX_FAST_STAT_WORDS + d.stat_index + d.ty,
-                             (1ull << 32) | (u64)(uint32_t)ws, __ATOMIC_RELAXED, __HIP_MEMORY_SCOPE_AGENT);
-  }
+    if (!PK) {
+      const int ws = wave_sum(surv);
+      if (lane == 0)
+        __hip_atomic_fetch_add(row_stat + (size_t)f * ORBX_FAST_STAT_WORDS + d.stat_index + d.ty,
+                               (1ull << 32) | (u64)(uint32_t)ws, __ATOMIC_RELAXED, __HIP_MEMORY_SCOPE_AGENT);
+    } else {
+      const int qs = (lane >> 2) & (Q - 1);
+      for (int qq = 0; qq < nq; qq++) {
+        const int ws = wave_sum(qs == qq ? surv : 0);
+        if (lane == 0)
+          __hip_atomic_fetch_add(row_stat + (size_t)(f + qq) * ORBX_FAST_STAT_WORDS + d.stat_index + d.ty,
+                                 (1ull << 32) | (u64)(uint32_t)ws, __ATOMIC_RELAXED, __HIP_MEMORY_SCOPE_AGENT);
+      }
+    }
+  }
+}
+
+template <int R, bool ZT>
+__global__ __launch_bounds__(64) void k_fast4(const OrbxTileDesc* __restrict__ tiles, int n_tiles, int n_frames,
+                                              const uint8_t* __restrict__ pyr, int frame_bytes, int mask_words,
+                                              OrbxFastParams fp, u64* __restrict__ mask, u64* __restrict__ row_stat,
+                                              OrbxPackGrid pg) {
+  typedef F4<R> C;
+  __shared__ __attribute__((aligned(16))) uint32_t s_img32[C::IMG_SLOTS * 64];
+  __shared__ __attribute__((aligned(16))) uint16_t s_sc[C::NS * C::SC_PITCH];
+  __shared__ __attribute__((aligned(16))) uint16_t s_queue[C::QCAP];
+  __shared__ __attribute__((aligned(16))) uint32_t s_cflag[64];
+  __shared__ __attribute__((aligned(16))) uint32_t s_mask32[C::G * 8];
+  __shared__ __attribute__((aligned(16))) uint32_t s_lut32[128];
+  __shared__ int s_qn;
+  const F4Lds<R> S{s_img32, s_sc, s_queue, s_cflag, s_mask32, s_lut32, &s_qn};
+
+  const int lane = threadIdx.x;
+  int lin = blockIdx.x;
+  if (lin < pg.blocks) {
+    int u = 0, base = 0;
+#pragma unroll
+    for (int i = 1; i < ORBX_MAX_LEVELS; i++) {
+      const bool here = i < pg.n_units && lin >= pg.start[i];
+      u = here ? i : u;
+      base = here ? pg.start[i] : base;
+    }
+    const OrbxTileDesc d = f3_tile(tiles, u);
+    f4_unit<R, ZT, true>(S, d, (lin - base) * d.f, n_frames, pyr, frame_bytes, mask_words, fp, mask, row_stat);
+    return;
+  }
+  lin -= pg.blocks;
+  const int tile = lin / n_frames, f = lin - tile * n_frames;
+  const OrbxTileDesc d = f3_tile(tiles, pg.n_units + tile);
+  if (row_stat && d.ty > 0) {
+    u64* st = row_stat + (size_t)f * ORBX_FAST_STAT_WORDS;
+    u64* dead = st + ORBX_MAX_LEVELS * ORBX_MAX_BANDS + d.l;
+    const u64 pv = f3_probe_issue(st + d.stat_index, dead, d.ty, lane);
+    if (f3_probe_decide(pv, dead, d.ty, d.u2, d.u0, lane)) return;
+  }
+  f4_unit<R, ZT, false>(S, d, f, n_frames, pyr, frame_bytes, mask_words, fp, mask, row_stat);
 }
 
 template <int R>
 void launch_fast4(unsigned wgs, hipStream_t s, const OrbxTileDesc* d_tiles, int n_tiles, int n_frames, const uint8_t* d_pyr,
                   int frame_bytes, int mask_words, OrbxFastParams fp, unsigned long long* d_mask,
-                  unsigned long long* d_row_stat) {
+                  unsigned long long* d_row_stat, const OrbxPackGrid& pg) {
   if (fp.threshold == 0)
     hipLaunchKernelGGL((k_fast4<R, true>), dim3(wgs), dim3(64), 0, s, d_tiles, n_tiles, n_frames, d_pyr, frame_bytes,
-                       mask_words, fp, d_mask, d_row_stat);
+                       mask_words, fp, d_mask, d_row_stat, pg);
   else
     hipLaunchKernelGGL((k_fast4<R, false>), dim3(wgs), dim3(64), 0, s, d_tiles, n_tiles, n_frames, d_pyr, frame_bytes,
-                       mask_words, fp, d_mask, d_row_stat);
+                       mask_words, fp, d_mask, d_row_stat, pg);
 }
 
 }
 
 hipError_t orbx_launch_fast4(hipStream_t s, const OrbxTileDesc* d_tiles, int n_tiles, int n_frames, const uint8_t* d_pyr,
                              int frame_bytes, int mask_words, OrbxFastParams fp, unsigned long long* d_mask,
-                             unsigned long long* d_row_stat) {
+                             unsigned long long* d_row_stat, const OrbxPackGrid* pack) {
   if (n_tiles <= 0 || n_frames <= 0) return hipSuccess;
-  const long long total = (long long)n_tiles * n_frames;
+  const OrbxPackGrid pg = pack ? *pack : OrbxPackGrid{};
+  if (pg.n_units < 0 || pg.n_units > n_tiles || pg.n_units > ORBX_MAX_LEVELS || pg.blocks < 0) return hipErrorInvalidValue;
+  const long long total = (long long)(n_tiles - pg.n_units) * n_frames + pg.blocks;
   if (total > 0x7fffffffll) return hipErrorInvalidValue;
+  if (total == 0) return hipSuccess;
   switch (fp.nms_radius) {
     case 0:
-      launch_fast4<0>((unsigned)total, s, d_tiles, n_tiles, n_frames, d_pyr, frame_bytes, mask_words, fp, d_mask, d_row_stat);
+      launch_fast4<0>((unsigned)total, s, d_tiles, n_tiles, n_frames, d_pyr, frame_bytes, mask_words, fp, d_mask, d_row_stat, pg);
       break;
     case 1:
-      launch_fast4<1>((unsigned)total, s, d_tiles, n_tiles, n_frames, d_pyr, frame_bytes, mask_words, fp, d_mask, d_row_stat);
+      launch_fast4<1>((unsigned)total, s, d_tiles, n_tiles, n_frames, d_pyr, frame_bytes, mask_words, fp, d_mask, d_row_stat, pg);
       break;
     case 2:
-      launch_fast4<2>((unsigned)total, s, d_tiles, n_tiles, n_frames, d_pyr, frame_bytes, mask_words, fp, d_mask, d_row_stat);
+      launch_fast4<2>((unsigned)total, s, d_tiles, n_tiles, n_frames, d_pyr, frame_bytes, mask_words, fp, d_mask, d_row_stat, pg);
       break;
     default:
-      launch_fast4<3>((unsigned)total, s, d_tiles, n_tiles, n_frames, d_pyr, frame_bytes, mask_words, fp, d_mask, d_row_stat);
+      launch_fast4<3>((unsigned)total, s, d_tiles, n_tiles, n_frames, d_pyr, frame_bytes, mask_words, fp, d_mask, d_row_stat, pg);
       break;
   }
   return hipGetLastError();
diff --git a/visual-odometry-gpu_amd/csrc/orbx_host.h b/visual-odometry-gpu_amd/csrc/orbx_host.h
--- a/visual-odometry-gpu_amd/csrc/orbx_host.h
+++ b/visual-odometry-gpu_amd/csrc/orbx_host.h
@@ -68,6 +68,8 @@
 };
 
 int fail(orbx_ctx* c, int status, const std::string& msg);
+
+extern "C" int orbx_debug_tail_packs(orbx_ctx* ctx, int* units, int* waves);
 
 #define HIPCHK(c, expr)                                                                              \
   do {                                                                                               \
@@ -289,6 +291,9 @@
   OrbxTileMap tm_blur{};
   OrbxBandMap bm_fast{};
   orbx_host::TileTable tiles[kTileTables];
+  orbx_host::TileTable fast_pack;
+  int fast_pack_units = 0;
+  OrbxTileDesc fast_pack_head[ORBX_MAX_LEVELS] = {};
   OrbxTopLevels top_levels{};
   std::vector<OrbxResizeTap> h_taps;
   OrbxPlanTables scratch;
@@ -312,6 +317,7 @@
   orbx_host::Lane lanes[2];
   int lane = 0;
   bool pipelined = false;
+  int last_pack_units = 0, last_pack_waves = 0;
   bool last_two_pass = false;
   hipStream_t last_stream = nullptr;
 
diff --git a/visual-odometry-gpu_amd/csrc/orbx_internal.h b/visual-odometry-gpu_amd/csrc/orbx_internal.h
--- a/visual-odometry-gpu_amd/csrc/orbx_internal.h
+++ b/visual-odometry-gpu_amd/csrc/orbx_internal.h
@@ -5,6 +5,7 @@
 #include "../../include/orbx.h"
 
 #include "orbx_plan.h"
+#include "orbx_pack.h"
 
 __host__ __device__ inline int orbx_mask_x(const OrbxLevel& L, int xw, int b) {
   return L.mask_strip_px ? (xw >> 2) * L.mask_strip_px + (xw & 3) * 64 + b : xw * 64 + b;
@@ -72,7 +73,7 @@
                                 unsigned long long* d_row_stat, int chunk_scale = 1);
 hipError_t orbx_launch_fast4(hipStream_t s, const OrbxTileDesc* d_tiles, int n_tiles, int n_frames, const uint8_t* d_pyr,
                              int frame_bytes, int mask_words, OrbxFastParams fp, unsigned long long* d_mask,
-                             unsigned long long* d_row_stat);
+                             unsigned long long* d_row_stat, const OrbxPackGrid* pack = nullptr);
 hipError_t orbx_launch_compact(hipStream_t s, const OrbxPlan& plan, int n_frames,
                                const unsigned long long* d_mask, orbx_keypoint* d_cand, int32_t* d_cand_count,
                                int32_t* d_cand_total, int need_total);
diff --git a/visual-odometry-gpu_amd/csrc/orbx_pack.h b/visual-odometry-gpu_amd/csrc/orbx_pack.h
--- /dev/null
+++ b/visual-odometry-gpu_amd/csrc/orbx_pack.h
@@ -0,0 +1,83 @@
+#pragma once
+#include "orbx_plan.h"
+
+struct OrbxTailPack {
+  int32_t q, w;
+};
+
+struct OrbxPackGrid {
+  int32_t n_units, blocks;
+  int32_t start[ORBX_MAX_LEVELS];
+};
+
+namespace orbx_pack {
+
+using namespace orbx_geom;
+
+inline int fast4_tail_lanes(int w, int nms_radius) {
+  const int dw0 = (orbx_fast4_strips(w, nms_radius) - 1) * orbx_fast4_strip_lanes(nms_radius);
+  return (w + 3) / 4 - dw0;
+}
+
+inline OrbxTailPack fast4_tail_pack(const OrbxPlan& plan, int l, int nms_radius) {
+  const OrbxLevel& L = plan.L[l];
+  const int lanes = fast4_tail_lanes(L.w, nms_radius), W = (lanes + 15) / 16 * 16;
+  if (W > 32) return OrbxTailPack{1, 64};
+  const int Q = 64 / W;
+  const uint64_t extent = (uint64_t)(Q - 1) * (uint64_t)plan.frame_bytes + (uint64_t)L.pitch * (uint64_t)L.h;
+  if (extent >= (1ull << 32)) return OrbxTailPack{1, 64};
+  return OrbxTailPack{Q, W};
+}
+
+inline void fast4_unit_cols(const OrbxTileDesc& d, int nms_radius, int* x0, int* x1) {
+  const int HD = orbx_fast4_halo(nms_radius), dw0 = d.tx * orbx_fast4_strip_lanes(nms_radius);
+  const int P0 = d.tx == 0 ? 0 : 4 * (dw0 + HD), P1 = d.tx + 1 == d.u2 ? 4 * (dw0 + 64) : 4 * (dw0 + 64 - HD);
+  *x0 = std::max(P0, 3);
+  *x1 = std::max(*x0, std::min(P1, d.w - 3));
+}
+
+inline size_t build_fast_pack_tiles(const OrbxPlan& plan, const OrbxBandMap& bm, int nms_radius, int bands, bool on,
+                                    std::vector<OrbxTileDesc>* out, int* n_units) {
+  std::vector<OrbxTileDesc> all;
+  build_fast_tiles(plan, bm, 0, 1, &all);
+  const size_t first = (size_t)bm.band_begin[std::min(std::max(bands, 0), bm.nbands)];
+  std::vector<OrbxTileDesc> packed, rest;
+  for (size_t i = 0; i < first && i < all.size(); i++) {
+    OrbxTileDesc d = all[i];
+    const OrbxTailPack tp = on && d.ty == 0 && d.tx + 1 == d.u2 ? fast4_tail_pack(plan, d.l, nms_radius) : OrbxTailPack{1, 64};
+    if (tp.q > 1) {
+      d.f = tp.q;
+      packed.push_back(d);
+    } else {
+      rest.push_back(d);
+    }
+  }
+  if (n_units) *n_units = (int)packed.size();
+  if (out) {
+    out->clear();
+    out->insert(out->end(), packed.begin(), packed.end());
+    out->insert(out->end(), rest.begin(), rest.end());
+  }
+  return packed.size() + rest.size();
+}
+
+inline bool fast4_pack_grid(const OrbxTileDesc* tiles, int n_units, int n_frames, OrbxPackGrid* g) {
+  *g = OrbxPackGrid{};
+  if (n_units < 0 || n_units > ORBX_MAX_LEVELS) return false;
+  for (int i = 0; i < n_units; i++) {
+    const int q = tiles[i].f;
+    if ((q != 2 && q != 4) || n_frames < q) return false;
+    g->start[i] = g->blocks;
+    g->blocks += (n_frames + q - 1) / q;
+  }
+  g->n_units = n_units;
+  return true;
+}
+
+inline int fast4_row0_share_milli(const OrbxPlan& plan, int l, int nms_radius, bool on) {
+  const int strips = orbx_fast4_strips(plan.L[l].w, nms_radius);
+  const OrbxTailPack tp = on ? fast4_tail_pack(plan, l, nms_radius) : OrbxTailPack{1, 64};
+  return (1000 * (strips - 1) + 1000 / tp.q) / strips;
+}
+
+}
diff --git a/visual-odometry-gpu_amd/csrc/orbx_plan.h b/visual-odometry-gpu_amd/csrc/orbx_plan.h
--- a/visual-odometry-gpu_amd/csrc/orbx_plan.h
+++ b/visual-odometry-gpu_amd/csrc/orbx_plan.h
@@ -574,24 +574,26 @@
   return uc.setup_milli + 1000 * ((rows + 2 * nms_radius + 6) / 7);
 }
 inline int first_pass_cost_milli(const uint32_t* hist, int depth, int cut, int nms_radius,
-                                 const OrbxUnitCost& uc = OrbxUnitCost{ORBX_FAST4_UNIT_SETUP_MILLI, ORBX_FAST4_UNIT_EXIT_MILLI}) {
+                                 const OrbxUnitCost& uc = OrbxUnitCost{ORBX_FAST4_UNIT_SETUP_MILLI, ORBX_FAST4_UNIT_EXIT_MILLI},
+                                 int row0_milli = 1000) {
   uint64_t total = 0;
   for (int b = 0; b < ORBX_FILL_BUCKETS; b++) total += hist[b];
   const uint64_t out = total ? fill_exits(hist, cut) : 0, on = total ? total - out : 1;
   const uint64_t second = (on * (uint64_t)fast4_unit_cost_milli(depth - cut, nms_radius, uc) + out * (uint64_t)uc.exit_milli) /
                           (total ? total : 1);
-  return fast4_unit_cost_milli(cut, nms_radius, uc) + (int)second;
+  return (int)((int64_t)fast4_unit_cost_milli(cut, nms_radius, uc) * row0_milli / 1000) + (int)second;
 }
 inline int choose_first_cut(const uint32_t* hist, int depth, int nms_radius, int unit_max, int* cost_milli,
-                            const OrbxUnitCost& uc = OrbxUnitCost{ORBX_FAST4_UNIT_SETUP_MILLI, ORBX_FAST4_UNIT_EXIT_MILLI}) {
+                            const OrbxUnitCost& uc = OrbxUnitCost{ORBX_FAST4_UNIT_SETUP_MILLI, ORBX_FAST4_UNIT_EXIT_MILLI},
+                            int row0_milli = 1000) {
   uint64_t total = 0;
   for (int b = 0; b < ORBX_FILL_BUCKETS; b++) total += hist[b];
-  int best = 0, best_cost = first_pass_cost_milli(hist, depth, depth / 2, nms_radius, uc);
+  int best = 0, best_cost = first_pass_cost_milli(hist, depth, depth / 2, nms_radius, uc, row0_milli);
   if (total)
     for (int cut = 7 - (2 * nms_radius) % 7; cut < depth; cut += 7) {
       if (cut > unit_max || depth - cut > unit_max || cut == depth / 2) continue;
       if (fill_exits(hist, cut) == 0) continue;
-      const int c = first_pass_cost_milli(hist, depth, cut, nms_radius, uc);
+      const int c = first_pass_cost_milli(hist, depth, cut, nms_radius, uc, row0_milli);
       if (c < best_cost) {
         best = cut;
         best_cost = c;
diff --git a/visual-odometry-gpu_amd/csrc/orbx_tables.h b/visual-odometry-gpu_amd/csrc/orbx_tables.h
--- a/visual-odometry-gpu_amd/csrc/orbx_tables.h
+++ b/visual-odometry-gpu_amd/csrc/orbx_tables.h
@@ -4,6 +4,7 @@
 #include <vector>
 
 #include "orbx_adapt.h"
+#include "orbx_pack.h"
 
 enum {
   T_FAST,
@@ -21,6 +22,7 @@
   int top_rows;
   bool grouped;
   bool prefs_apply;
+  bool tail_pack = false;
 };
 
 struct OrbxPlanTables {
@@ -28,6 +30,8 @@
   OrbxBandMap bm_fast{};
   std::vector<OrbxTileDesc> tiles[kTileTables];
   OrbxTopLevels top_levels{};
+  std::vector<OrbxTileDesc> fast_pack;
+  int fast_pack_units = 0;
 };
 
 namespace orbx_tables {
@@ -92,6 +96,12 @@
   if (too_large(T_PYR2, "pyramid tile table exceeds pool")) return ORBX_ERR_UNSUPPORTED;
   build_fast_tiles(plan, bm, 0, 1, &out->tiles[T_FAST]);
   if (too_large(T_FAST, "FAST tile table exceeds pool")) return ORBX_ERR_UNSUPPORTED;
+  out->fast_pack.clear();
+  out->fast_pack_units = 0;
+  if (sw.tail_pack && sw.fast_impl == 4 && top > 0 && bm.nbands > top) {
+    orbx_pack::build_fast_pack_tiles(plan, bm, nms_radius, top, true, &out->fast_pack, &out->fast_pack_units);
+    if (out->fast_pack_units == 0) out->fast_pack.clear();
+  }
   return ORBX_OK;
 }
 
```

After: 696,100 frames/s. No clear change (-0.4%).
